# FriedFeid/Video-Depth-Anything

Measured on AMD Instinct MI355X. Metric: depth frames/sec at 32x518x518, ViT-L fp16, 1/2/4/8 MI355X, higher is better.
Workload: dtype fp16; 1 GPU; VideoDepthAnything.forward vitl 1x32x3x518x518 per GPU; encoder=vitl, frames_per_clip=32, H=518, W=518, clips_per_gpu=1, parallelism=clip-parallel dp1, ranks=1, depth_gather_to_rank0=False, hip_graph=False, clips_in_flight=2

## Files before the change

include/vda.h:

```cpp
#ifndef VDA_H
#define VDA_H

#include <stdint.h>

#ifdef __cplusplus
extern "C" {
#endif

enum {
  VDA_ACT_NONE = 0,
  VDA_ACT_GELU = 1,
  VDA_ACT_GEGLU = 2,
  VDA_ACT_RELU = 3
};

enum {
  VDA_STORE_ROWS = 0,
  VDA_STORE_PIXEL_SHUFFLE = 1
};

typedef struct vda_epilogue {
  const float* bias;
  const float* rowbias;
  int32_t rdiv, rmod;
  const float* gamma;
  const void* res;
  int64_t ldres;
  const void* res2;
  int64_t ldres2;
  int32_t act;
  int32_t store;
  int32_t ps_k, ps_cout, ps_hin, ps_win;
  const float* ln_stats;
  const float* ln_colsum;
  int32_t ln_parts;
  float ln_eps;
  float* stats_out;
  int32_t res2_h, res2_w;
  int32_t* sched;
  int32_t drop_period;
} vda_epilogue;

const char* vda_version(void);
int64_t vda_epilogue_size(void);
const char* vda_last_error(void);

int vda_gemm(const void* x, int64_t ldx, const void* w, void* y, int64_t ldy,
             int32_t M, int32_t N, int32_t K, const vda_epilogue* epi, void* stream);
int vda_gemm_check(int64_t ldx, int64_t ldy, int32_t M, int32_t N, int32_t K, const vda_epilogue* epi);

int vda_conv2d(const void* x, const void* w, void* y, int32_t BT, int32_t H, int32_t W,
               int32_t Cin, int32_t Cout, int32_t ks, int32_t stride, int32_t pad,
               int32_t pre_relu, int32_t up_h, int32_t up_w, const vda_epilogue* epi,
               void* ws, int64_t ws_bytes, void* stream);
int64_t vda_conv2d_workspace(int32_t BT, int32_t H, int32_t W, int32_t Cin, int32_t Cout, int32_t ks,
                             int32_t stride, int32_t pad);
int vda_conv2d_res2_upsample_ok(int32_t BT, int32_t H, int32_t W, int32_t Cin, int32_t Cout, int32_t ks,
                                int32_t stride, int32_t pad);

int vda_layernorm(const void* x, int64_t ldx, void* y, const float* gamma, const float* beta,
                  int32_t rows, int32_t C, float eps, int32_t skip_period, void* stream);

int vda_row_stats(const void* x, int64_t ldx, float* stats, int32_t rows, int32_t C, float eps,
                  void* stream);

int vda_groupnorm(const void* x, void* y, const float* gamma, const float* beta, int32_t F,
                  int32_t S, int32_t C, int32_t groups, float eps, float* ws, void* stream);
int64_t vda_groupnorm_workspace(int32_t F, int32_t S, int32_t C, int32_t groups);

int vda_groupnorm_linear(const void* x, const float* gamma, const float* beta, int32_t F, int32_t S,
                         int32_t C, int32_t groups, float eps, const void* w, const float* bias, void* y,
                         int32_t N, float* stats_out, void* ws, int64_t ws_bytes, void* stream);
int64_t vda_groupnorm_linear_workspace(int32_t F, int32_t S, int32_t C, int32_t groups, int32_t N);
int vda_groupnorm_linear_fused(int32_t C, int32_t groups, int32_t N);

int vda_spatial_attention(const void* qkv, void* out, int32_t B, int32_t N, int32_t H,
                          int32_t D, float scale, void* stream);

int vda_temporal_attention(const void* qkv, void* out, int32_t B, int32_t T, int32_t S,
                           int32_t H, int32_t D, float scale, float rope_theta, void* stream);

int vda_upsample_bilinear(const void* x, void* y, int32_t BT, int32_t H, int32_t W, int32_t C,
                          int32_t Ho, int32_t Wo, void* stream);

int vda_patch_im2col(const float* img, void* a, int32_t BT, int32_t H, int32_t W, int32_t Kp,
                     void* stream);

int vda_depth_head(const void* x, const void* w1, const float* b1, const float* w2,
                   const float* b2, float* depth, void* ws, int32_t BT, int32_t Hin, int32_t Win,
                   int32_t C, int32_t Ho, int32_t Wo, void* stream);
int64_t vda_depth_head_workspace(int32_t BT, int32_t Hin, int32_t Win, int32_t C, int32_t Ho, int32_t Wo);

int vda_preprocess_frames(const void* frames, float* out, int32_t N, int32_t h, int32_t w, int32_t H,
                          int32_t W, const float* mean, const float* std, void* stream);

int vda_depth_resize(const float* depth, float* out, int32_t N, int32_t H, int32_t W, int32_t ho,
                     int32_t wo, void* stream);

int64_t vda_scale_shift_workspace(int64_t n);
int vda_scale_shift(const float* pred, const float* target, const uint8_t* mask, int64_t n, double* sums,
                    float* ss, void* ws, int64_t ws_bytes, void* stream);

int vda_depth_align(const float* src, int32_t F, int32_t H, int32_t W, int32_t ho, int32_t wo, const float* ss,
                    int32_t clip, const float* pre, const float* w_pre, const float* w_post, float* out,
                    void* stream);

int64_t vda_depth_eval_workspace(int32_t F, int64_t S);
int vda_depth_eval_fit(const float* pred, const float* gt, const uint8_t* valid, int32_t F, int64_t S,
                       int32_t per_frame, double* sums, float* ss, void* ws, int64_t ws_bytes, void* stream);
int vda_depth_eval_metrics(const float* pred, const float* gt, const uint8_t* valid, int32_t F, int64_t S,
                           const float* ss, int32_t ss_per_frame, float max_depth, float* aligned,
                           double* frame_sums, double* total, void* ws, int64_t ws_bytes, void* stream);

enum {
  VDA_VIS_INDEX = 0,
  VDA_VIS_HWC = 1,
  VDA_VIS_PLANAR444 = 2,
  VDA_VIS_PLANAR420 = 3
};
int64_t vda_depth_range_workspace(int64_t n);
int vda_depth_range(const float* depth, int64_t n, float* range, void* ws, int64_t ws_bytes, void* stream);
int64_t vda_depth_colorize_bytes(int32_t F, int32_t H, int32_t W, int32_t layout);
int vda_depth_colorize(const float* depth, int32_t F, int32_t H, int32_t W, const float* range,
                       const uint8_t* lut, int32_t layout, uint8_t* out, void* stream);

enum {
  VDA_YUV_420 = 0,
  VDA_YUV_422 = 1,
  VDA_YUV_444 = 2,
  VDA_YUV_MONO = 3
};
int vda_yuv_to_rgb(const uint8_t* src, int32_t N, int32_t h, int32_t w, int64_t frame_stride, int32_t chroma,
                   uint8_t* out, void* stream);
int64_t vda_preprocess_yuv_workspace(int32_t N, int32_t h, int32_t w, int32_t H, int32_t W);
int vda_preprocess_yuv(const uint8_t* src, int32_t N, int32_t h, int32_t w, int64_t frame_stride, int32_t chroma,
                       float* out, int32_t H, int32_t W, const float* mean, const float* stdv, void* ws,
                       int64_t ws_bytes, void* stream);
int32_t vda_resample_taps(int32_t in, int32_t out);
int vda_resample_tables(int32_t in, int32_t out, int32_t* k, int32_t* bounds);
int vda_yuv_downscale_ok(int32_t h, int32_t w, int32_t h2, int32_t w2);
int64_t vda_yuv_downscale_workspace(int32_t N, int32_t h, int32_t w, int32_t h2, int32_t w2);
// ... 31 lines not shown
```

video-depth-anything_amd/_lib.py:

```python
from __future__ import annotations

import ctypes
import os
from ctypes import c_float, c_int32, c_int64, c_void_p, POINTER

_HERE = os.path.dirname(os.path.abspath(__file__))
LIB_PATH = os.environ.get("VDA_LIB_OVERRIDE") or os.path.join(_HERE, "libvda.so")
TORCH_LIB_PATH = os.path.join(_HERE, "libvda_torch.so")
if os.environ.get("VDA_LIB_OVERRIDE"):
    _ov = os.path.join(os.path.dirname(os.path.abspath(os.environ["VDA_LIB_OVERRIDE"])), "libvda_torch.so")
    if os.path.exists(_ov):
        TORCH_LIB_PATH = _ov

EXPORTED = (
    "vda_version", "vda_epilogue_size", "vda_last_error", "vda_gemm", "vda_gemm_check", "vda_conv2d", "vda_conv2d_workspace",
    "vda_layernorm",
    "vda_conv2d_res2_upsample_ok",
    "vda_row_stats", "vda_groupnorm", "vda_groupnorm_workspace",
    "vda_groupnorm_linear", "vda_groupnorm_linear_workspace", "vda_groupnorm_linear_fused",
    "vda_spatial_attention", "vda_temporal_attention", "vda_upsample_bilinear", "vda_patch_im2col",
    "vda_depth_head", "vda_depth_head_workspace", "vda_preprocess_frames", "vda_depth_resize",
    "vda_scale_shift", "vda_scale_shift_workspace", "vda_depth_align",
    "vda_depth_eval_workspace", "vda_depth_eval_fit", "vda_depth_eval_metrics",
    "vda_depth_range_workspace", "vda_depth_range", "vda_depth_colorize_bytes", "vda_depth_colorize",
    "vda_yuv_to_rgb", "vda_preprocess_yuv_workspace", "vda_preprocess_yuv",
    "vda_resample_taps", "vda_resample_tables", "vda_yuv_downscale_ok", "vda_yuv_downscale_workspace",
    "vda_yuv_downscale",
    "vda_gemm_f32", "vda_conv2d_f32", "vda_layernorm_f32", "vda_groupnorm_f32", "vda_spatial_attention_f32",
    "vda_temporal_attention_f32", "vda_upsample_bilinear_f32", "vda_patch_im2col_f32", "vda_depth_head_f32",
)
TUNE_EXPORTED = ("vda_debug_force_tile", "vda_debug_gemm_sched", "vda_debug_strip_split", "vda_debug_hconv",
                 "vda_debug_dconv", "vda_debug_attn")
TUNE_LIB_PATH = os.path.join(os.path.dirname(_HERE), "build", "tune", "libvda.so")

ACT_NONE, ACT_GELU, ACT_GEGLU, ACT_RELU = 0, 1, 2, 3
STORE_ROWS, STORE_PIXEL_SHUFFLE = 0, 1
VIS_INDEX, VIS_HWC, VIS_PLANAR444, VIS_PLANAR420 = 0, 1, 2, 3
YUV_420, YUV_422, YUV_444, YUV_MONO = 0, 1, 2, 3


class VDAUnavailable(RuntimeError):
    pass


class VDAError(RuntimeError):
    pass


class Epilogue(ctypes.Structure):
    _fields_ = [
        ("bias", c_void_p), ("rowbias", c_void_p), ("rdiv", c_int32), ("rmod", c_int32),
        ("gamma", c_void_p), ("res", c_void_p), ("ldres", c_int64), ("res2", c_void_p),
        ("ldres2", c_int64), ("act", c_int32), ("store", c_int32), ("ps_k", c_int32),
        ("ps_cout", c_int32), ("ps_hin", c_int32), ("ps_win", c_int32),
        ("ln_stats", c_void_p), ("ln_colsum", c_void_p), ("ln_parts", c_int32), ("ln_eps", c_float),
        ("stats_out", c_void_p), ("res2_h", c_int32), ("res2_w", c_int32), ("sched", c_void_p),
        ("drop_period", c_int32),
    ]


_lib = None
_load_error = None


def _declare(lib):
    P, I, L, F = c_void_p, c_int32, c_int64, c_float
    EP = POINTER(Epilogue)
    sig = {
        "vda_version": ([], ctypes.c_char_p),
        "vda_epilogue_size": ([], L),
        "vda_last_error": ([], ctypes.c_char_p),
        "vda_gemm": ([P, L, P, P, L, I, I, I, EP, P], I),
        "vda_gemm_check": ([L, L, I, I, I, EP], I),
        "vda_conv2d": ([P, P, P, I, I, I, I, I, I, I, I, I, I, I, EP, P, L, P], I),
        "vda_conv2d_workspace": ([I, I, I, I, I, I, I, I], L),
        "vda_conv2d_res2_upsample_ok": ([I, I, I, I, I, I, I, I], I),
        "vda_layernorm": ([P, L, P, P, P, I, I, F, I, P], I),
        "vda_row_stats": ([P, L, P, I, I, F, P], I),
        "vda_groupnorm": ([P, P, P, P, I, I, I, I, F, P, P], I),
        "vda_groupnorm_workspace": ([I, I, I, I], L),
        "vda_groupnorm_linear": ([P, P, P, I, I, I, I, F, P, P, P, I, P, P, L, P], I),
        "vda_groupnorm_linear_workspace": ([I, I, I, I, I], L),
        "vda_groupnorm_linear_fused": ([I, I, I], I),
        "vda_spatial_attention": ([P, P, I, I, I, I, F, P], I),
        "vda_temporal_attention": ([P, P, I, I, I, I, I, F, F, P], I),
        "vda_upsample_bilinear": ([P, P, I, I, I, I, I, I, P], I),
        "vda_patch_im2col": ([P, P, I, I, I, I, P], I),
        "vda_depth_head": ([P, P, P, P, P, P, P, I, I, I, I, I, I, P], I),
        "vda_depth_head_workspace": ([I, I, I, I, I, I], L),
        "vda_preprocess_frames": ([P, P, I, I, I, I, I, POINTER(F), POINTER(F), P], I),
        "vda_depth_resize": ([P, P, I, I, I, I, I, P], I),
        "vda_scale_shift_workspace": ([L], L),
        "vda_scale_shift": ([P, P, P, L, P, P, P, L, P], I),
        "vda_depth_align": ([P, I, I, I, I, I, P, I, P, POINTER(F), POINTER(F), P, P], I),
        "vda_depth_eval_workspace": ([I, L], L),
        "vda_depth_eval_fit": ([P, P, P, I, L, I, P, P, P, L, P], I),
        "vda_depth_eval_metrics": ([P, P, P, I, L, P, I, F, P, P, P, P, L, P], I),
        "vda_depth_range_workspace": ([L], L),
        "vda_depth_range": ([P, L, P, P, L, P], I),
        "vda_depth_colorize_bytes": ([I, I, I, I], L),
        "vda_depth_colorize": ([P, I, I, I, P, P, I, P, P], I),
        "vda_yuv_to_rgb": ([P, I, I, I, L, I, P, P], I),
        "vda_preprocess_yuv_workspace": ([I, I, I, I, I], L),
        "vda_preprocess_yuv": ([P, I, I, I, L, I, P, I, I, POINTER(F), POINTER(F), P, L, P], I),
        "vda_resample_taps": ([I, I], I),
        "vda_resample_tables": ([I, I, P, P], I),
        "vda_yuv_downscale_ok": ([I, I, I, I], I),
        "vda_yuv_downscale_workspace": ([I, I, I, I, I], L),
        "vda_yuv_downscale": ([P, I, I, I, L, I, P, P, P, P, P, I, I, P, L, P], I),
        "vda_gemm_f32": ([P, L, P, P, L, I, I, I, EP, P], I),
        "vda_conv2d_f32": ([P, P, P, I, I, I, I, I, I, I, I, I, EP, P], I),
        "vda_layernorm_f32": ([P, L, P, P, P, I, I, F, I, P], I),
        "vda_groupnorm_f32": ([P, P, P, P, I, I, I, I, F, P], I),
        "vda_spatial_attention_f32": ([P, P, I, I, I, I, F, P], I),
        "vda_temporal_attention_f32": ([P, P, I, I, I, I, I, F, F, P], I),
        "vda_upsample_bilinear_f32": ([P, P, I, I, I, I, I, I, P], I),
        "vda_patch_im2col_f32": ([P, P, I, I, I, I, P], I),
        "vda_depth_head_f32": ([P, P, P, P, P, P, P, P, I, I, I, I, I, I, P], I),
        "vda_debug_force_tile": ([I], I),
        "vda_debug_gemm_sched": ([I], I),
        "vda_debug_strip_split": ([I], I),
        "vda_debug_hconv": ([I], I),
        "vda_debug_dconv": ([I], I),
        "vda_debug_attn": ([I], I),
    }
    for name, (args, res) in sig.items():
        if name.startswith("vda_debug_") and not hasattr(lib, name):
            continue
        fn = getattr(lib, name)
        fn.argtypes = args
        fn.restype = res


def lib():
    global _lib, _load_error
    if _lib is not None:
        return _lib
    if _load_error is not None:
        raise VDAUnavailable(_load_error)
    if not os.path.exists(LIB_PATH):
        _load_error = f"libvda.so not found at {LIB_PATH}; run `make` (or __graft_entry__.build())"
        raise VDAUnavailable(_load_error)
    try:
        l = ctypes.CDLL(LIB_PATH)
        _declare(l)
        if l.vda_epilogue_size() != ctypes.sizeof(Epilogue):
            raise OSError(f"vda_epilogue is {l.vda_epilogue_size()} bytes in the library, {ctypes.sizeof(Epilogue)} "
                          f"in _lib.Epilogue: rebuild libvda.so or update the mirror")
    except OSError as e:
        _load_error = f"failed to load {LIB_PATH}: {e}"
        raise VDAUnavailable(_load_error) from e
    _lib = l
    return _lib


_torch_ops = None


def torch_ops():
# ... 20 lines not shown
```

video-depth-anything_amd/csrc/vda_conv2d.hip:

```cpp
#include "vda_internal.h"

static bool conv_takes_strip(int BT, int H, int W, int Cin, int Cout, int ks, int stride, int pad, int up_h) {
  if (up_h > 0 || ks != 3 || stride != 1 || pad != 1 || !vda_conv_strip_serves(W, Cin, Cout)) return false;
  const long strip_tiles = (long)BT * ((H * W + 255) / 256);
  return g_force_tile == -3 || (g_force_tile == -1 && (Cin >= 512 || strip_tiles * 2 <= vda_cu_count()));
}

static long conv_im2col_bytes(int BT, int H, int W, int Cin, int ks, int stride, int pad) {
  const long Ho = (H + 2L * pad - ks) / stride + 1, Wo = (W + 2L * pad - ks) / stride + 1;
  return (long)BT * Ho * Wo * ks * ks * Cin * 2;
}
static bool conv_takes_im2col(int BT, int H, int W, int Cin, int Cout, int ks, int stride, int pad, int up_h) {
  if (up_h > 0 || ks != 3 || stride != 2 || Cout % 256 != 0 || g_force_tile != -1) return false;
  const long Ho = (H + 2L * pad - ks) / stride + 1, Wo = (W + 2L * pad - ks) / stride + 1;
  return Ho > 0 && Wo > 0 && vda_gemm_phased256_serves((long)BT * Ho * Wo, Cout, 9L * Cin, 9L * Cin);
}

static bool conv_takes_hconv(int BT, int H, int W, int Cin, int Cout, int ks, int stride, int pad) {
  return ks == 3 && stride == 1 && pad == 1 && g_force_tile == -1 && vda_conv_hconv_serves(BT, H, W, Cin, Cout);
}

extern "C" int64_t vda_conv2d_workspace(int32_t BT, int32_t H, int32_t W, int32_t Cin, int32_t Cout, int32_t ks,
                                        int32_t stride, int32_t pad) {
  if (BT <= 0 || H <= 0 || W <= 0 || Cin <= 0 || Cout <= 0) return 0;
  if (conv_takes_hconv(BT, H, W, Cin, Cout, ks, stride, pad)) return 0;
  if (conv_takes_im2col(BT, H, W, Cin, Cout, ks, stride, pad, 0)) return conv_im2col_bytes(BT, H, W, Cin, ks, stride, pad);
  if (!conv_takes_strip(BT, H, W, Cin, Cout, ks, stride, pad, 0)) return 0;
  return vda_conv_strip_ws_bytes(BT, H, W, Cin, Cout);
}

extern "C" int vda_conv2d_res2_upsample_ok(int32_t BT, int32_t H, int32_t W, int32_t Cin, int32_t Cout, int32_t ks,
                                           int32_t stride, int32_t pad) {
  if (BT <= 0 || H <= 0 || W <= 0 || Cin <= 0 || Cout <= 0) return 0;
  return conv_takes_hconv(BT, H, W, Cin, Cout, ks, stride, pad) ? 1 : 0;
}

extern "C" int vda_conv2d(const void* x, const void* w, void* y, int32_t BT, int32_t H, int32_t W,
                          int32_t Cin, int32_t Cout, int32_t ks, int32_t stride, int32_t pad,
                          int32_t pre_relu, int32_t up_h, int32_t up_w, const vda_epilogue* epi,
                          void* ws, int64_t ws_bytes, void* stream) {
  VDA_CHECK_ARG(x && w && y, "null pointer");
  VDA_CHECK_ARG(BT > 0 && H > 0 && W > 0 && Cin > 0 && Cout > 0 && ks > 0 && stride > 0 && pad >= 0,
                "bad conv geometry");
  VDA_CHECK_ARG(Cin % 8 == 0 && Cout % 4 == 0, "Cin % 8 and Cout % 4 required");
  const int Hi = up_h > 0 ? up_h : H, Wi = up_w > 0 ? up_w : W;
  GemmParams p{};
  p.x = (const h16*)x; p.w = (const h16*)w; p.y = (h16*)y;
  p.H = H; p.W = W; p.Cin = Cin; p.ks = ks; p.stride = stride; p.pad = pad; p.pre_relu = pre_relu;
  p.up_h = up_h > 0 ? up_h : 0; p.up_w = up_w > 0 ? up_w : 0;
  p.Ho = (Hi + 2 * pad - ks) / stride + 1;
  p.Wo = (Wi + 2 * pad - ks) / stride + 1;
  VDA_CHECK_ARG(p.Ho > 0 && p.Wo > 0, "empty conv output");
  p.M = BT * p.Ho * p.Wo; p.N = Cout; p.K = ks * ks * Cin;
  p.ldy = Cout; p.ldx = 0;
  p.epi = epi ? *epi : vda_default_epi();
  if (p.epi.rdiv <= 0) p.epi.rdiv = 1;
  if (p.epi.rmod <= 0) p.epi.rmod = 1;
  VDA_CHECK_ARG(p.epi.store == VDA_STORE_ROWS && (p.epi.act == VDA_ACT_NONE || p.epi.act == VDA_ACT_RELU),
                "conv: row store, activation none/relu");
  VDA_CHECK_ARG(!p.epi.stats_out && !p.epi.ln_stats, "conv: no LayerNorm fold / row statistics");
  int rc = vda_check_epi(p.epi, p.M, Cout);
  if (rc) return rc;
  const bool res2_up = p.epi.res2_h > 0 || p.epi.res2_w > 0;
  if (res2_up) {
    VDA_CHECK_ARG(p.epi.res2 && p.epi.res2_h > 0 && p.epi.res2_w > 0 && p.epi.ldres2 == Cout && p.up_h == 0 &&
                      !p.epi.gamma && !p.epi.rowbias && (!p.epi.res || p.epi.ldres == Cout) &&
                      p.epi.res2_h <= p.Ho && p.epi.res2_w <= p.Wo &&
                      (long)p.epi.res2_h * p.epi.res2_w * Cout * 2 < (1L << 31) &&
                      conv_takes_hconv(BT, H, W, Cin, Cout, ks, stride, pad),
                  "upsampled res2 needs the halo conv route (vda_conv2d_res2_upsample_ok), a [BT, h <= Ho, w <= Wo, "
                  "Cout] source, no gamma / rowbias / input upsample");
    return vda_conv_hconv(x, w, y, p.epi.bias, p.epi.act == VDA_ACT_RELU, pre_relu, p.epi.res, p.epi.res2,
                          p.epi.res2_h, p.epi.res2_w, BT, H, W, Cin, Cout, (hipStream_t)stream);
  }
  if (p.up_h > 0) {
    if (g_force_tile < 0 && ks == 3 && stride == 1 && pad == 1 && !pre_relu && !p.epi.res && !p.epi.res2 &&
        !p.epi.gamma && !p.epi.rowbias) {
      rc = vda_conv_halo_fused(x, w, y, p.epi.bias, p.epi.act == VDA_ACT_RELU, BT, H, W, p.up_h, p.up_w, Cin, Cout,
                               (hipStream_t)stream);
      if (rc != 1) return rc;
    }
    return vda_launch_conv_reg(p, (hipStream_t)stream);
  }
  if (!p.epi.gamma && !p.epi.rowbias && (!p.epi.res || p.epi.ldres == Cout) && (!p.epi.res2 || p.epi.ldres2 == Cout) &&
      conv_takes_hconv(BT, H, W, Cin, Cout, ks, stride, pad)) {
    rc = vda_conv_hconv(x, w, y, p.epi.bias, p.epi.act == VDA_ACT_RELU, pre_relu, p.epi.res, p.epi.res2, 0, 0, BT, H,
                        W, Cin, Cout, (hipStream_t)stream);
    if (rc != 1) return rc;
  }
  if (conv_takes_strip(BT, H, W, Cin, Cout, ks, stride, pad, 0) && !p.epi.gamma && !p.epi.rowbias &&
      (!p.epi.res || p.epi.ldres == Cout) && (!p.epi.res2 || p.epi.ldres2 == Cout)) {
    rc = vda_conv_strip(x, w, y, p.epi.bias, p.epi.act == VDA_ACT_RELU, pre_relu, p.epi.res, p.epi.res2, BT, H, W,
                        Cin, Cout, ws, ws ? ws_bytes : 0, (hipStream_t)stream);
    if (rc != 1) return rc;
  }
  if (g_force_tile < 0 && ks == 3 && stride == 1 && pad == 1 && !pre_relu && !p.epi.res && !p.epi.res2 &&
      !p.epi.gamma && !p.epi.rowbias && (long)H * W >= 128L * 128L) {
    rc = vda_conv_halo(x, w, y, p.epi.bias, p.epi.act == VDA_ACT_RELU, BT, H, W, Cin, Cout, (hipStream_t)stream);
    if (rc != 1) return rc;
  }
  if (conv_takes_im2col(BT, H, W, Cin, Cout, ks, stride, pad, 0) && !pre_relu && ws &&
      ws_bytes >= conv_im2col_bytes(BT, H, W, Cin, ks, stride, pad) && (uintptr_t)ws % 16 == 0 &&
      (uintptr_t)x % 16 == 0) {
    rc = vda_conv_im2col(x, ws, BT, H, W, Cin, p.Ho, p.Wo, ks, stride, pad, (hipStream_t)stream);
    if (rc) return rc;
    p.x = (const h16*)ws;
    p.ldx = p.K;
    return vda_launch_gemm(p, (hipStream_t)stream);
  }
  return vda_launch_conv_gemm(p, (hipStream_t)stream);
}
```

video-depth-anything_amd/csrc/vda_f32.hip:

```cpp
#include "vda_common.h"
#include "../../include/vda.h"
#include <cmath>

namespace {

struct F32Params {
  const float* x; long ldx;
  const float* w;
  float* y; long ldy;
  int M, N, K;
  int H, W, Cin, Ho, Wo, ks, stride, pad, pre_relu;
  vda_epilogue epi;
};

constexpr int FBK = 16;
constexpr int FLD = 20;

__device__ __forceinline__ f4 mfma_f32(float a, float b, f4 c) {
  return __builtin_amdgcn_mfma_f32_16x16x4f32(a, b, c, 0, 0, 0);
}

__device__ __forceinline__ float gelu_exact(float v) { return 0.5f * v * (1.0f + erff(v * 0.70710678118654752f)); }

template <bool CONV>
// ... 389 lines not shown
    const f4 d = *reinterpret_cast<const f4*>(bp + ((long)y1 * W + x1) * C);
    f4 o;
#pragma unroll
    for (int j = 0; j < 4; ++j) o[j] = hy * (hx * a[j] + lx * bq[j]) + ly * (hx * cq[j] + lx * d[j]);
    *reinterpret_cast<f4*>(y + i * 4) = o;
  }
}

__global__ __launch_bounds__(256) void im2col_f32_kernel(const float* __restrict__ img, float* __restrict__ a, int BT,
                                                         int H, int W, int Kp) {
  const int ph = H / 14, pw = W / 14, np = ph * pw;
  const long total = (long)BT * (1 + np) * Kp;
  for (long i = (long)blockIdx.x * 256 + threadIdx.x; i < total; i += (long)gridDim.x * 256) {
    const int k = (int)(i % Kp);
    const long row = i / Kp;
    const int tok = (int)(row % (1 + np));
    const int bt = (int)(row / (1 + np));
    float v = 0.f;
    if (tok > 0 && k < 588) {
      const int pidx = tok - 1, py = pidx / pw, px = pidx - py * pw;
      const int ci = k / 196, r = k - ci * 196, ky = r / 14, kx = r - ky * 14;
      v = img[(((long)bt * 3 + ci) * H + py * 14 + ky) * W + px * 14 + kx];
    }
    a[i] = v;
  }
}

__global__ __launch_bounds__(256) void pointwise_relu_f32_kernel(const float* __restrict__ mid, const float* __restrict__ w2,
                                                                 const float* __restrict__ b2, float* __restrict__ out, long M) {
  const long m = (long)blockIdx.x * 256 + threadIdx.x;
  if (m >= M) return;
  const float* r = mid + m * 32;
  float a = 0.f;
#pragma unroll
  for (int c = 0; c < 32; c += 4) {
    const f4 v = *reinterpret_cast<const f4*>(r + c);
    a += v[0] * w2[c] + v[1] * w2[c + 1] + v[2] * w2[c + 2] + v[3] * w2[c + 3];
  }
  out[m] = fmaxf(a + b2[0], 0.f);
}

template <bool CONV>
int launch_f32(const F32Params& p, hipStream_t st) {
  const int tiles_n = (p.N + 127) / 128, tiles_m = (p.M + 127) / 128;
  const long blocks = (long)tiles_n * tiles_m;
  if (blocks > 0x7fffffffL) return vda_set_error(-22, "fp32 GEMM grid too large");
  const dim3 g((unsigned)blocks), bl(256);
  switch (p.epi.act) {
    case VDA_ACT_NONE: hipLaunchKernelGGL((gemm_f32_kernel<CONV, VDA_ACT_NONE>), g, bl, 0, st, p, tiles_n); break;
    case VDA_ACT_GELU: hipLaunchKernelGGL((gemm_f32_kernel<CONV, VDA_ACT_GELU>), g, bl, 0, st, p, tiles_n); break;
    case VDA_ACT_RELU: hipLaunchKernelGGL((gemm_f32_kernel<CONV, VDA_ACT_RELU>), g, bl, 0, st, p, tiles_n); break;
    case VDA_ACT_GEGLU:
      if (CONV) return vda_set_error(-22, "GEGLU epilogue is dense-only");
      hipLaunchKernelGGL((gemm_f32_kernel<CONV, VDA_ACT_GEGLU>), g, bl, 0, st, p, tiles_n);
      break;
    default: return vda_set_error(-22, "unknown activation");
  }
  VDA_LAUNCH_CHECK();
  return 0;
}

}

extern "C" int vda_gemm_f32(const float* x, int64_t ldx, const float* w, float* y, int64_t ldy, int32_t M, int32_t N,
                            int32_t K, const vda_epilogue* epi, void* stream) {
  VDA_CHECK_ARG(x && w && y && epi, "null pointer");
  VDA_CHECK_ARG(M > 0 && N > 0 && K > 0, "empty GEMM");
  VDA_CHECK_ARG(K % 4 == 0 && ldx % 4 == 0 && N % 4 == 0, "fp32 GEMM needs K, ldx, N multiples of 4");
  VDA_CHECK_ARG(ldx >= K, "fp32 GEMM needs ldx >= K");
  VDA_CHECK_ARG(ldy % 4 == 0, "fp32 GEMM needs ldy a multiple of 4");
  VDA_CHECK_ARG(!epi->res || epi->ldres % 4 == 0, "fp32 GEMM needs ldres a multiple of 4");
  VDA_CHECK_ARG(!epi->res2 || epi->ldres2 % 4 == 0, "fp32 GEMM needs ldres2 a multiple of 4");
  VDA_CHECK_ARG(epi->drop_period == 0, "fp32 GEMM: no drop_period (vda_gemm only)");
  VDA_CHECK_ARG(epi->act != VDA_ACT_GEGLU || (N % 32 == 0 && !epi->rowbias && !epi->res2 &&
                                              epi->store == VDA_STORE_ROWS),
                "GEGLU needs N % 32 == 0, no rowbias/res2, row store");
  VDA_CHECK_ARG(epi->store != VDA_STORE_PIXEL_SHUFFLE || (epi->ps_k > 0 && epi->ps_cout % 4 == 0 &&
                                                         epi->ps_hin > 0 && epi->ps_win > 0),
                "bad pixel-shuffle geometry");
  VDA_CHECK_ARG(!epi->rowbias || (epi->rdiv > 0 && epi->rmod > 0), "rowbias needs rdiv, rmod > 0");
  VDA_CHECK_ARG(!epi->ln_stats, "fp32 GEMM: no LayerNorm fold (the fp32 mode runs vda_layernorm_f32)");
  VDA_CHECK_ARG(!epi->stats_out, "fp32 GEMM: no row statistics output");
  VDA_CHECK_ARG(epi->res2_h == 0 && epi->res2_w == 0, "fp32 GEMM: no upsampled res2");
  F32Params p{};
  p.x = x; p.ldx = ldx; p.w = w; p.y = y; p.ldy = ldy; p.M = M; p.N = N; p.K = K; p.epi = *epi;
  return launch_f32<false>(p, (hipStream_t)stream);
}

extern "C" int vda_conv2d_f32(const float* x, const float* w, float* y, int32_t BT, int32_t H, int32_t W, int32_t Cin,
                              int32_t Cout, int32_t ks, int32_t stride, int32_t pad, int32_t pre_relu,
                              const vda_epilogue* epi, void* stream) {
  VDA_CHECK_ARG(x && w && y && epi, "null pointer");
  VDA_CHECK_ARG(BT > 0 && H > 0 && W > 0 && ks > 0 && stride > 0 && pad >= 0, "bad conv geometry");
  VDA_CHECK_ARG(Cin % 4 == 0 && Cout % 4 == 0, "fp32 conv needs Cin, Cout multiples of 4");
  VDA_CHECK_ARG(epi->act != VDA_ACT_GEGLU && epi->store == VDA_STORE_ROWS, "conv epilogue: no GEGLU / pixel shuffle");
  VDA_CHECK_ARG(epi->res2_h == 0 && epi->res2_w == 0, "fp32 conv: no upsampled res2 (materialise it)");
  VDA_CHECK_ARG(!epi->rowbias || (epi->rdiv > 0 && epi->rmod > 0), "rowbias needs rdiv, rmod > 0");
  VDA_CHECK_ARG(epi->drop_period == 0, "fp32 conv: no drop_period (vda_gemm only)");
  VDA_CHECK_ARG(!epi->res || epi->ldres % 4 == 0, "fp32 conv needs ldres a multiple of 4");
  VDA_CHECK_ARG(!epi->res2 || epi->ldres2 % 4 == 0, "fp32 conv needs ldres2 a multiple of 4");
  VDA_CHECK_ARG(!epi->ln_stats && !epi->stats_out, "fp32 conv: no LayerNorm fold / row statistics");
  F32Params p{};
  p.x = x; p.w = w; p.y = y; p.ldy = Cout;
  p.H = H; p.W = W; p.Cin = Cin; p.ks = ks; p.stride = stride; p.pad = pad; p.pre_relu = pre_relu;
  p.Ho = (H + 2 * pad - ks) / stride + 1;
  p.Wo = (W + 2 * pad - ks) / stride + 1;
  VDA_CHECK_ARG(p.Ho > 0 && p.Wo > 0, "empty conv output");
  const long M = (long)BT * p.Ho * p.Wo;
  VDA_CHECK_ARG(M < 0x7fffffffL, "conv output too large");
  p.M = (int)M; p.N = Cout; p.K = ks * ks * Cin; p.epi = *epi;
  return launch_f32<true>(p, (hipStream_t)stream);
}

extern "C" int vda_spatial_attention_f32(const float* qkv, float* out, int32_t B, int32_t N, int32_t H, int32_t D,
                                         float scale, void* stream) {
  VDA_CHECK_ARG(qkv && out, "null pointer");
  VDA_CHECK_ARG(B > 0 && N > 0 && H > 0, "empty attention");
  VDA_CHECK_ARG(D == 64, "fp32 spatial attention: head dim must be 64");
  VDA_CHECK_ARG(B <= 65535 && H <= 65535, "grid too large");
  hipLaunchKernelGGL(spatial_attn_f32_kernel, dim3((N + 63) / 64, H, B), dim3(256), 0, (hipStream_t)stream, qkv, out, N,
                     H, scale);
  VDA_LAUNCH_CHECK();
  return 0;
}

extern "C" int vda_temporal_attention_f32(const float* qkv, float* out, int32_t B, int32_t T, int32_t S, int32_t H,
                                          int32_t D, float scale, float rope_theta, void* stream) {
  VDA_CHECK_ARG(qkv && out, "null pointer");
  VDA_CHECK_ARG(B > 0 && T > 0 && S > 0 && H > 0 && D > 0, "empty attention");
  VDA_CHECK_ARG(T <= 32 && D <= 128 && D % 2 == 0, "temporal attention: T <= 32, even D <= 128");
  const long blocks = (long)B * S * H;
  VDA_CHECK_ARG(blocks < 0x7fffffffL, "grid too large");
  hipLaunchKernelGGL(temporal_attn_f32_kernel, dim3((unsigned)blocks), dim3(64), 0, (hipStream_t)stream, qkv, out, T, S,
                     H, D, scale, rope_theta);
  VDA_LAUNCH_CHECK();
  return 0;
}

extern "C" int vda_layernorm_f32(const float* x, int64_t ldx, float* y, const float* gamma, const float* beta,
                                 int32_t rows, int32_t C, float eps, int32_t skip_period, void* stream) {
  VDA_CHECK_ARG(x && y && gamma && beta, "null pointer");
  VDA_CHECK_ARG(rows > 0 && C > 0 && C <= 2048, "LayerNorm: 0 < C <= 2048");
  hipLaunchKernelGGL(layernorm_f32_kernel, dim3((rows + 3) / 4), dim3(256), 0, (hipStream_t)stream, x, (long)ldx, y,
                     gamma, beta, rows, C, eps, skip_period);
  VDA_LAUNCH_CHECK();
  return 0;
}

extern "C" int vda_groupnorm_f32(const float* x, float* y, const float* gamma, const float* beta, int32_t F, int32_t S,
                                 int32_t C, int32_t groups, float eps, void* stream) {
  VDA_CHECK_ARG(x && y && gamma && beta, "null pointer");
  VDA_CHECK_ARG(F > 0 && S > 0 && groups > 0 && C % groups == 0, "bad GroupNorm geometry");
  hipLaunchKernelGGL(groupnorm_f32_kernel, dim3(F * groups), dim3(256), 0, (hipStream_t)stream, x, y, gamma, beta, S, C,
                     groups, eps);
  VDA_LAUNCH_CHECK();
  return 0;
}

extern "C" int vda_upsample_bilinear_f32(const float* x, float* y, int32_t BT, int32_t H, int32_t W, int32_t C,
                                         int32_t Ho, int32_t Wo, void* stream) {
  VDA_CHECK_ARG(x && y, "null pointer");
  VDA_CHECK_ARG(BT > 0 && H > 0 && W > 0 && Ho > 0 && Wo > 0 && C > 0 && C % 4 == 0, "bad resize geometry");
  const long total = (long)BT * Ho * Wo * (C / 4);
  const int grid = (int)std::min<long>((total + 255) / 256, 65536);
  hipLaunchKernelGGL(upsample_f32_kernel, dim3(grid), dim3(256), 0, (hipStream_t)stream, x, y, BT, H, W, C, Ho, Wo);
  VDA_LAUNCH_CHECK();
  return 0;
}

extern "C" int vda_patch_im2col_f32(const float* img, float* a, int32_t BT, int32_t H, int32_t W, int32_t Kp,
                                    void* stream) {
  VDA_CHECK_ARG(img && a, "null pointer");
  VDA_CHECK_ARG(BT > 0 && H >= 14 && W >= 14 && H % 14 == 0 && W % 14 == 0, "bad image geometry");
  VDA_CHECK_ARG(Kp >= 588 && Kp % 4 == 0, "Kp must be >= 588 and a multiple of 4");
  const long total = (long)BT * (1 + (H / 14) * (W / 14)) * Kp;
  const int grid = (int)std::min<long>((total + 255) / 256, 65536);
  hipLaunchKernelGGL(im2col_f32_kernel, dim3(grid), dim3(256), 0, (hipStream_t)stream, img, a, BT, H, W, Kp);
  VDA_LAUNCH_CHECK();
  return 0;
// ... 21 lines not shown
```

video-depth-anything_amd/csrc/vda_gemm.hip:

```cpp
#include "vda_gemm_tile.h"
#include "vda_gemm_phased.h"
#include <algorithm>

VDA_KNOB_DEF(int, g_force_tile, -1);

static bool phased_dense_ok(long M, long N, long K, long ldx) {
  return K % 64 == 0 && M * ldx * 2 < (1L << 31) && N * K * 2 < (1L << 31);
}

bool vda_gemm_phased256_serves(long M, long N, long K, long ldx) {
  return N >= 256 && M >= 4096 && phased_dense_ok(M, N, K, ldx);
}

namespace {

VDA_KNOB(int, g_persist, -1);

enum Phased {
  PH_STAGED,
  PH_ROWB,
  PH_REG,
  PH_LNF,
  PH_LNF_REG,
  PH_LNF_ROWB,
// ... 57 lines not shown
  const int tiles_m = (p.M + BM - 1) / BM, tiles_n = (p.N + BN - 1) / BN;
  hipLaunchKernelGGL((gemm_kernel<BM, BN, NWM, NWN, KB, NS, CONV, ACT>), dim3(tiles_m * tiles_n), dim3(NWM * NWN * 64),
                     0, st, p, tiles_m, tiles_n);
}

template <int XR, int WR, bool CONV, int ACT>
void launch_phased(Phased v, const GemmParams& p, hipStream_t st) {
  const int BM = 128 * XR, BN = 128 * WR;
  const int tiles_m = (p.M + BM - 1) / BM, tiles_n = (p.N + BN - 1) / BN;
  const int grid = phased_sched(tiles_m * tiles_n, CONV);
  auto go = [&](void (*kernel)(GemmParams, int, int)) {
    hipLaunchKernelGGL(kernel, dim3(grid), dim3(512), 0, st, p, tiles_m, tiles_n);
  };
  constexpr bool PLAIN = ACT == VDA_ACT_NONE, GELU = ACT == VDA_ACT_GELU, GEGLU = ACT == VDA_ACT_GEGLU;
  constexpr bool D256 = !CONV && XR == 2;
  if constexpr (!CONV && PLAIN)
    if (v == PH_ROWB) return go(gemm256_kernel<XR, WR, CONV, ACT, true>);
  if constexpr (D256 && PLAIN)
    if (v == PH_LNF_ROWB) return go(gemm256_kernel<XR, WR, CONV, ACT, false, true, 3>);
  if constexpr (D256 && (PLAIN || GELU || GEGLU))
    if (v == PH_LNF) return go(gemm256_kernel<XR, WR, CONV, ACT, false, true>);
  if constexpr (D256 && (PLAIN || GELU)) {
    if (v == PH_LNF_REG) return go(gemm256_kernel<XR, WR, CONV, ACT, false, true, 1>);
    if (v == PH_REG) return go(gemm256_kernel<XR, WR, CONV, ACT, false, false, 1>);
  }
  go(gemm256_kernel<XR, WR, CONV, ACT, false>);
}

template <bool CONV, int ACT>
int launch_cfg(const GemmRoute& r, const GemmParams& p, hipStream_t st) {
  switch (r.cfg) {
    case 1: launch_tile<256, 128, 4, 2, 32, 4, CONV, ACT>(p, st); break;
    case 2: launch_tile<128, 64, 2, 2, 32, 4, CONV, ACT>(p, st); break;
    case 3: launch_tile<256, 256, 2, 4, 32, 4, CONV, ACT>(p, st); break;
    case 4: launch_phased<2, 2, CONV, ACT>(r.phased, p, st); break;
    case 5: launch_phased<4, 1, CONV, ACT>(r.phased, p, st); break;
    case 6:
    case 7:
      if constexpr (CONV) {
        return vda_set_error(-22, "conv: no 64-row tile configuration (6 / 7)");
      } else {
        if (r.cfg == 6) launch_tile<64, 64, 2, 2, 32, 4, CONV, ACT>(p, st);
        else launch_tile<64, 128, 2, 2, 32, 4, CONV, ACT>(p, st);
      }
      break;
    default: launch_tile<128, 128, 2, 2, 32, 4, CONV, ACT>(p, st); break;
  }
  return 0;
}

template <bool CONV>
int launch(const GemmParams& p, hipStream_t st) {
  const GemmRoute r = gemm_route(p, CONV);
  int rc = 0;
  switch (p.epi.act) {
    case VDA_ACT_GELU:
    case VDA_ACT_GEGLU:
      if constexpr (CONV) return vda_set_error(-22, "conv epilogue: activation none / relu");
      else rc = p.epi.act == VDA_ACT_GELU ? launch_cfg<CONV, VDA_ACT_GELU>(r, p, st) : launch_cfg<CONV, VDA_ACT_GEGLU>(r, p, st);
      break;
    case VDA_ACT_RELU: rc = launch_cfg<CONV, VDA_ACT_RELU>(r, p, st); break;
    default: rc = launch_cfg<CONV, VDA_ACT_NONE>(r, p, st); break;
  }
  if (rc) return rc;
  VDA_LAUNCH_CHECK();
  if (p.epi.stats_out && !r.writes_stats) return vda_row_partials_launch(p.y, p.ldy, p.epi.stats_out, p.M, p.N, st);
  return 0;
}

int gemm_check(const void* x, int64_t ldx, const void* w, void* y, int64_t ldy, int32_t M, int32_t N, int32_t K,
               const vda_epilogue* epi, GemmParams& p) {
  VDA_CHECK_ARG(x && w && y, "null pointer");
  VDA_CHECK_ARG(M > 0 && N > 0 && K > 0, "empty GEMM");
  VDA_CHECK_ARG(K % 8 == 0 && ldx % 8 == 0 && ldx >= K, "K and ldx must be multiples of 8, ldx >= K");
  VDA_CHECK_ARG(N % 4 == 0 && ldy % 4 == 0, "N and ldy must be multiples of 4");
  p = GemmParams{};
  p.x = (const h16*)x; p.ldx = ldx; p.w = (const h16*)w; p.y = (h16*)y; p.ldy = ldy;
  p.M = M; p.N = N; p.K = K;
  p.epi = epi ? *epi : vda_default_epi();
  if (p.epi.rdiv <= 0) p.epi.rdiv = 1;
  if (p.epi.rmod <= 0) p.epi.rmod = 1;
  const vda_epilogue& e = p.epi;
  VDA_CHECK_ARG(e.res2_h == 0 && e.res2_w == 0, "upsampled res2: vda_conv2d only");
  const GemmRoute r = gemm_route(p, false);
  const bool auto256 = g_force_tile < 0 && r.cfg == 4;
  if (e.drop_period != 0) {
    VDA_CHECK_ARG(auto256 && r.phased == PH_LNF_REG && e.act == VDA_ACT_NONE && e.ln_colsum && e.drop_period >= 256 &&
                      N % 256 == 0,
                  "drop_period: >= 256, with ln_stats + bias, no activation / gamma / res / rowbias / stats_out, "
                  "N % 256 == 0, M >= 4096, K % 64 == 0, 16-byte aligned rows");
  }
  int rc = vda_check_epi(e, M, N);
  if (rc) return rc;
  if (e.ln_stats && e.rowbias) {
    VDA_CHECK_ARG(auto256 && r.phased == PH_LNF_ROWB && N % 256 == 0 && (uintptr_t)x % 16 == 0,
                  "ln_stats with rowbias needs N % 256 == 0, M >= 4096, K % 64 == 0, 16-B aligned rows");
  }
  return 0;
}

}

int vda_launch_conv_reg(const GemmParams& p, hipStream_t st) {
  const int tiles_m = (p.M + 127) / 128;
  if (p.N >= 128) {
    const int tiles_n = (p.N + 127) / 128;
    if (p.epi.act == VDA_ACT_RELU)
      hipLaunchKernelGGL((gemm_reg_kernel<128, 128, ConvLoader, VDA_ACT_RELU>), dim3(tiles_m * tiles_n), dim3(256), 0, st, p, tiles_n);
    else
      hipLaunchKernelGGL((gemm_reg_kernel<128, 128, ConvLoader, VDA_ACT_NONE>), dim3(tiles_m * tiles_n), dim3(256), 0, st, p, tiles_n);
  } else {
    const int tiles_n = (p.N + 63) / 64;
    if (p.epi.act == VDA_ACT_RELU)
      hipLaunchKernelGGL((gemm_reg_kernel<128, 64, ConvLoader, VDA_ACT_RELU>), dim3(tiles_m * tiles_n), dim3(256), 0, st, p, tiles_n);
    else
      hipLaunchKernelGGL((gemm_reg_kernel<128, 64, ConvLoader, VDA_ACT_NONE>), dim3(tiles_m * tiles_n), dim3(256), 0, st, p, tiles_n);
  }
  VDA_LAUNCH_CHECK();
  return 0;
}

vda_epilogue vda_default_epi() {
  vda_epilogue e{};
  e.rdiv = 1; e.rmod = 1;
  return e;
}

int vda_check_epi(const vda_epilogue& e, int M, int N) {
  VDA_CHECK_ARG(!e.rowbias || (e.rdiv > 0 && e.rmod > 0), "rowbias needs rdiv, rmod > 0");
  VDA_CHECK_ARG(e.act >= 0 && e.act <= 3, "unknown activation");
  VDA_CHECK_ARG(e.act != VDA_ACT_GEGLU || (N % 32 == 0 && !e.rowbias && e.store == 0 && !e.res2),
                "GEGLU needs N % 32 == 0, no rowbias/res2, row store");
  VDA_CHECK_ARG(e.store == VDA_STORE_ROWS ||
                (e.store == VDA_STORE_PIXEL_SHUFFLE && e.ps_k > 0 && e.ps_cout > 0 && e.ps_cout % 4 == 0 &&
                 e.ps_hin > 0 && e.ps_win > 0 && N == e.ps_k * e.ps_k * e.ps_cout && !e.res && !e.res2),
                "bad pixel-shuffle store geometry");
  VDA_CHECK_ARG(!e.ln_stats || (e.ln_colsum && e.store == VDA_STORE_ROWS && !e.gamma &&
                                 (e.act == VDA_ACT_NONE || e.act == VDA_ACT_GELU || e.act == VDA_ACT_GEGLU)),
                "ln_stats needs ln_colsum, a row store, no gamma, activation none / gelu / geglu");
  VDA_CHECK_ARG(!e.ln_stats || !e.rowbias ||
                    (e.act == VDA_ACT_NONE && e.bias && !e.res && !e.res2 && !e.stats_out && e.rdiv >= 256),
                "ln_stats with rowbias needs a bias, no activation / residual / stats_out, rdiv >= 256");
  VDA_CHECK_ARG(!e.ln_stats || (e.ln_parts >= 0 && e.ln_parts <= 4), "ln_parts must be 0 .. 4");
  VDA_CHECK_ARG(!e.ln_stats || (long)M * (e.ln_parts > 0 ? e.ln_parts : 1) >= 2, "ln_stats needs M * max(ln_parts, 1) >= 2");
  VDA_CHECK_ARG(!e.stats_out || (e.store == VDA_STORE_ROWS && e.act != VDA_ACT_GEGLU),
                "stats_out needs a row store and no GEGLU");
  VDA_CHECK_ARG(!e.res || e.ldres % 4 == 0, "ldres % 4");
  VDA_CHECK_ARG(!e.res2 || e.ldres2 % 4 == 0, "ldres2 % 4");
  return 0;
}

int vda_launch_gemm(const GemmParams& p, hipStream_t st) { return launch<false>(p, st); }

extern "C" int vda_gemm_check(int64_t ldx, int64_t ldy, int32_t M, int32_t N, int32_t K, const vda_epilogue* epi) {
  GemmParams p;
  void* const aligned = (void*)16;
  return gemm_check(aligned, ldx, aligned, aligned, ldy, M, N, K, epi, p);
}

extern "C" int vda_gemm(const void* x, int64_t ldx, const void* w, void* y, int64_t ldy, int32_t M,
                        int32_t N, int32_t K, const vda_epilogue* epi, void* stream) {
  GemmParams p;
  const int rc = gemm_check(x, ldx, w, y, ldy, M, N, K, epi, p);
  return rc ? rc : vda_launch_gemm(p, (hipStream_t)stream);
}

int vda_launch_conv_gemm(const GemmParams& p, hipStream_t st) { return launch<true>(p, st); }

int vda_launch_depth_gemm(const GemmParams& p, hipStream_t st) {
  const int tiles_m = (p.M + 255) / 256;
  hipLaunchKernelGGL((gemm_kernel<256, 64, 8, 1, 64, 2, true, ACT_DEPTH>), dim3(tiles_m), dim3(512), 0, st, p, tiles_m, 1);
  VDA_LAUNCH_CHECK();
  return 0;
}

#ifdef VDA_TUNING
extern "C" int vda_debug_force_tile(int32_t cfg) {
  g_force_tile = cfg;
  return 0;
}

extern "C" int vda_debug_gemm_sched(int32_t persist_blocks) {
  g_persist = persist_blocks;
  return 0;
}
#endif
```

video-depth-anything_amd/csrc/vda_gemm_phased.h:

```cpp
#pragma once
#include "vda_common.h"
#include "phi_table.h"
#include <type_traits>
#ifdef VDA_TS
__device__ unsigned long long g_ts[4096][8];
#define TS(k) do { if (threadIdx.x == 0 && vb < 4096) g_ts[vb][k] = __builtin_amdgcn_s_memrealtime(); } while (0)
extern "C" int vda_debug_timestamps(void* host) {
  return (int)hipMemcpyFromSymbol(host, HIP_SYMBOL(g_ts), sizeof(g_ts), 0, hipMemcpyDeviceToHost);
}
__device__ unsigned long long g_tsc[1024][4];
#define TSC(k) do { if (threadIdx.x == 0 && blockIdx.x < 1024) { \
    g_tsc[blockIdx.x][2 * (k)] = __builtin_amdgcn_s_memtime(); \
    g_tsc[blockIdx.x][2 * (k) + 1] = __builtin_amdgcn_s_memrealtime(); } } while (0)
extern "C" int vda_debug_clock_stamps(void* host) {
  return (int)hipMemcpyFromSymbol(host, HIP_SYMBOL(g_tsc), sizeof(g_tsc), 0, hipMemcpyDeviceToHost);
}
#else
#define TS(k) do {} while (0)
#define TSC(k) do {} while (0)
#endif
#include "vda_gemm_tile.h"

constexpr int VDA_EPI_STORE_AUX = 2;

// ... 43 lines not shown
               : "v"((unsigned)(uintptr_t)(VDA_LDS const int*)ptr) : "memory");
  return v;
}

__device__ __forceinline__ void perm16_swap(float& a, float& b) {
  asm volatile("s_nop 1\n\tv_permlane16_swap_b32 %0, %1" : "+v"(a), "+v"(b));
}
template <int CTRL>
__device__ __forceinline__ float dpp_f(float v) {
  return __builtin_bit_cast(float, __builtin_amdgcn_mov_dpp(__builtin_bit_cast(int, v), CTRL, 0xF, 0xF, true));
}
__device__ __forceinline__ float halfwave_sum32(float (&v)[32], int lane) {
  float w[16];
#pragma unroll
  for (int k = 0; k < 16; ++k) {
    float a = v[k], b = v[16 + k];
    perm16_swap(a, b);
    w[k] = a + b;
  }
  const int i = lane & 15;
  float x[8], y[4], z[2];
  bool lo = i < 8;
#pragma unroll
  for (int k = 0; k < 8; ++k) x[k] = (lo ? w[k] : w[k + 8]) + dpp_f<0x140>(lo ? w[k + 8] : w[k]);
  lo = (i & 7) < 4;
#pragma unroll
  for (int k = 0; k < 4; ++k) y[k] = (lo ? x[k] : x[k + 4]) + dpp_f<0x141>(lo ? x[k + 4] : x[k]);
  lo = (i & 3) < 2;
#pragma unroll
  for (int k = 0; k < 2; ++k) z[k] = (lo ? y[k] : y[k + 2]) + dpp_f<0x1B>(lo ? y[k + 2] : y[k]);
  lo = (i & 1) == 0;
  return (lo ? z[0] : z[1]) + dpp_f<0xB1>(lo ? z[1] : z[0]);
}
template <class F>
__device__ __forceinline__ void pack_row_lines(F v, bool lo8, u32x4& A, u32x4& B) {
  u32x4 o[2];
#pragma unroll
  for (int pp = 0; pp < 2; ++pp) {
    float a[4], c[4];
#pragma unroll
    for (int r = 0; r < 4; ++r) {
      a[r] = v(2 * pp, r);
      c[r] = v(2 * pp + 1, r);
      perm16_swap(a[r], c[r]);
    }
    typedef float f2v __attribute__((ext_vector_type(2)));
    const h2 h0 = __builtin_convertvector(f2v{a[0], a[1]}, h2), h1 = __builtin_convertvector(f2v{a[2], a[3]}, h2);
    const h2 h2_ = __builtin_convertvector(f2v{c[0], c[1]}, h2), h3 = __builtin_convertvector(f2v{c[2], c[3]}, h2);
    o[pp] = u32x4{__builtin_bit_cast(unsigned, h0), __builtin_bit_cast(unsigned, h1),
                  __builtin_bit_cast(unsigned, h2_), __builtin_bit_cast(unsigned, h3)};
  }
#pragma unroll
  for (int k = 0; k < 4; ++k) {
    const unsigned snd = lo8 ? o[1][k] : o[0][k];
    const unsigned got = (unsigned)__builtin_amdgcn_mov_dpp((int)snd, 0x128, 0xF, 0xF, true);
    A[k] = lo8 ? o[0][k] : got;
    B[k] = lo8 ? got : o[1][k];
  }
}
__device__ __forceinline__ float2 ln_mean_rstd(float sm, float sq, float invK, float eps) {
  const float mean = sm * invK;
  return make_float2(mean, rsqrtf(fmaxf(fmaf(-mean, mean, sq * invK), 0.f) + eps));
}
__device__ __forceinline__ void stat_acc(h8 t, float& s, float& q) {
  const h2 one = h2{(h16)1.f, (h16)1.f};
  h2 tp[4];
#pragma unroll
  for (int k = 0; k < 4; ++k) tp[k] = h2{t[2 * k], t[2 * k + 1]};
  s = 0.f;
  q = 0.f;
#pragma unroll
  for (int k = 0; k < 4; ++k) {
    s = __builtin_amdgcn_fdot2(tp[k], one, s, false);
    q = __builtin_amdgcn_fdot2(tp[k], tp[k], q, false);
  }
}

template <int XR, int WR, int ACT>
constexpr int phased_nit() {
  constexpr int OW = (ACT == VDA_ACT_GEGLU) ? 64 * WR : 128 * WR;
  return (128 * XR) / (512 / (OW / 8));
}

template <int XR, int WR, bool CONV, int ACT, bool ROWB, bool LNF, int EK>
__device__ __forceinline__ int gemm256_tile(const GemmParams& p, int vb, int tiles_m, int tiles_n, h16* smem,
                                            bool pre, int vb_next, int wave_in, unsigned* tctr = nullptr,
                                            int tbase = 0, int* tslot = nullptr) {
  static_assert(!(LNF && (ROWB || CONV)), "LNF: dense, no row bias");
  static_assert(EK == 0 || (!CONV && !ROWB), "fixed epilogue kinds: dense, no row bias");
  static_assert(EK != 3 || (ACT == VDA_ACT_NONE && LNF), "EK 3: LN fold + per-frame row bias, no activation");
  const bool has_bias = EK ? true : p.epi.bias != nullptr;
  const bool has_gamma = EK ? false : p.epi.gamma != nullptr;
  const bool ps_rows = !EK && ACT != VDA_ACT_GEGLU && !ROWB && XR == 2 && WR == 2 &&
                       p.epi.store == VDA_STORE_PIXEL_SHUFFLE && p.epi.ps_cout % 256 == 0 && p.epi.ps_win >= 16 &&
                       (long)p.M * p.N * 2 < 0x7fffffffL && (uintptr_t)p.y % 16 == 0;
  const bool rows_store = EK ? true : (p.epi.store == VDA_STORE_ROWS || ps_rows);
  const bool has_res = EK ? false : p.epi.res != nullptr;
  const bool has_res2 = EK ? false : p.epi.res2 != nullptr;
  const bool has_stats = EK ? false : p.epi.stats_out != nullptr;
  static_assert(XR * WR == 4 && (XR == 2 || XR == 4), "8 waves as XR (m) x 8/XR (n), wave tile 128 x 64");
  constexpr int BM = 128 * XR, BN = 128 * WR;
  constexpr int HALF = 128 * BK;
  constexpr int BUF = (XR + WR) * HALF;
  constexpr bool TAB = XR == 2 && (ACT == VDA_ACT_GELU || ACT == VDA_ACT_GEGLU);
  const float* phi_lds = reinterpret_cast<const float*>(smem + 2 * BUF);
  const unsigned phib = phi_base(phi_lds);
  h16* lnst_lds = smem + 2 * BUF + (TAB ? PHI_LDS_HALVES : 0);
  auto lnst_shift_row = [&](int m0_) {
    const int P1 = p.epi.ln_parts > 0 ? p.epi.ln_parts : 1;
    return ((p.M * P1) & 1) && p.M - 1 - m0_ < 256 ? p.M - 1 - m0_ : -1;
  };

  int lane, wave;
  asm volatile("v_mbcnt_lo_u32_b32 %0, -1, 0\n\tv_mbcnt_hi_u32_b32 %0, -1, %0" : "=v"(lane));
  asm volatile("s_mov_b32 %0, %1" : "=s"(wave) : "s"(wave_in));
  const int tid = wave * 64 + lane;
  const int wm = wave % XR, wn = wave / XR;
  int tile_m, tile_n;
  tile_coords(vb, tiles_m * tiles_n, tiles_m, tiles_n, tile_m, tile_n);
  const int m0 = tile_m * BM, n0 = tile_n * BN;

  const h16* xrow[XR][2];
  const h16* wrow[WR][2];
  bool xok[XR][2], wok[WR][2];
  auto xr_of = [&](int i) { return i * 64 + wave * 8 + (lane >> 3); };
  auto wr_of = [&](int i) { return (wave >> 2) * 64 + i * 32 + (wave & 3) * 8 + (lane >> 3); };
  const int kch0 = ((lane & 7) ^ ((((wave & 1) << 3 | (lane >> 3)) >> 1) & 7)) * 8;
  int cyx[XR][2];
#pragma unroll
  for (int i = 0; i < 2; ++i) {
#pragma unroll
    for (int hh = 0; hh < XR; ++hh) {
      const int m = m0 + hh * 128 + xr_of(i);
      xok[hh][i] = m < p.M;
      const int mm = xok[hh][i] ? m : 0;
      if constexpr (CONV) {
        const int ox = mm % p.Wo;
        const int t = mm / p.Wo;
        const int oy = t % p.Ho, bt = t / p.Ho;
        const int iy0 = xok[hh][i] ? oy * p.stride - p.pad : -32768;
        const int ix0 = ox * p.stride - p.pad;
        cyx[hh][i] = (iy0 << 16) | (ix0 & 0xffff);
        xrow[hh][i] = p.x + (((long)bt * p.H + oy * p.stride - p.pad) * p.W + ix0) * p.Cin;
      } else {
        xrow[hh][i] = p.x + (long)mm * p.ldx;
      }
    }
#pragma unroll
    for (int hh = 0; hh < WR; ++hh) {
      const int n = n0 + hh * 128 + wr_of(i);
      wok[hh][i] = n < p.N;
      wrow[hh][i] = p.w + (long)(wok[hh][i] ? n : 0) * p.K;
    }
  }
  const void* zero = (const void*)g_zero_page;
  const bool tap_uniform = CONV && (p.Cin % BK == 0);
  int t_ci[2] = {0, 0}, t_kx[2] = {0, 0}, t_ky[2] = {0, 0};
  long t_off[2] = {0, 0};
  auto dma_x = [&](int kt, int buf, int i) {
    const int k0 = kt * BK;
    const int ky = t_ky[i], kx = t_kx[i];
    const long toff = t_off[i];
    if (tap_uniform) {
      t_off[i] += BK;
      t_ci[i] += BK;
      if (t_ci[i] == p.Cin) {
        t_ci[i] = 0;
        if (++t_kx[i] == p.ks) { t_kx[i] = 0; ++t_ky[i]; t_off[i] += (long)(p.W - p.ks) * p.Cin; }
      }
    }
#pragma unroll
    for (int hh = 0; hh < XR; ++hh) {
        const int k = k0 + kch0;
        const void* src = zero;
        if constexpr (CONV) {
          if (k < p.K) {
            if (tap_uniform) {
              if ((unsigned)((cyx[hh][i] >> 16) + ky) < (unsigned)p.H &&
                  (unsigned)((short)(cyx[hh][i] & 0xffff) + kx) < (unsigned)p.W)
// ... 336 lines not shown
      const unsigned rA = ya == 0x80000000u ? ya : ya + co;
      const unsigned rB = yb == 0x80000000u ? yb : yb + co;
      __builtin_amdgcn_raw_buffer_store_b128(A, ry, rA, 0, VDA_EPI_STORE_AUX);
      __builtin_amdgcn_raw_buffer_store_b128(B, ry, rB, 0, VDA_EPI_STORE_AUX);
    }
    TS(5);
    return succ;
  }
  if (rows_store) {
    constexpr int OW = (ACT == VDA_ACT_GEGLU) ? BN / 2 : BN;
    __syncthreads();
    const vda_epilogue& e = p.epi;
    bool nok[4];
    int ncl[4];
#pragma unroll
    for (int i = 0; i < 4; ++i) {
      const int n = n0 + wn * 64 + i * 16 + nq;
      nok[i] = n < p.N;
      ncl[i] = nok[i] ? n : 0;
    }
    if constexpr (LNF) {
      const float* st = reinterpret_cast<const float*>(lnst_lds);
      const f4* bv = pbv;
      const int P = e.ln_parts;
      const float invK = 1.f / (float)p.K;
      const int srow = lnst_shift_row(m0);
#pragma unroll
      for (int j = 0; j < 8; ++j) {
        const int rl = wm * 128 + j * 16 + mcol;
        const int sh = rl == srow ? 2 : 0;
        float2 mr;
        if (P <= 0) {
          mr = *reinterpret_cast<const float2*>(st + 2 * rl + sh);
        } else {
          float sm = 0.f, sq = 0.f;
          for (int t = 0; t < P; ++t) {
            const float2 pq = *reinterpret_cast<const float2*>(st + 2 * (rl * P + t) + (t == P - 1 ? sh : 0));
            sm += pq.x;
            sq += pq.y;
          }
          mr = ln_mean_rstd(sm, sq, invK, e.ln_eps);
        }
#pragma unroll
        for (int i = 0; i < 4; ++i)
#pragma unroll
          for (int r = 0; r < 4; ++r)
            acc[i][j][r] = fmaf(mr.y, fmaf(-mr.x, pgv[i][r], acc[i][j][r]), bv[i][r]);
      }
    } else if (has_bias) {
      f4 bv[4];
#pragma unroll
      for (int i = 0; i < 4; ++i)
        bv[i] = PREF ? pbv[i] : *reinterpret_cast<const f4*>(e.bias + (ACT == VDA_ACT_GEGLU ? ncl[i & ~1] + (i & 1) * 16 : ncl[i]));
#pragma unroll
      for (int i = 0; i < 4; ++i)
#pragma unroll
        for (int j = 0; j < 8; ++j) acc[i][j] += bv[i];
    }
    if constexpr (ACT != VDA_ACT_GEGLU && ROWB) {
      if (e.rowbias) {
        const float inv_div = 1.f / (float)e.rdiv, inv_mod = 1.f / (float)e.rmod;
        auto rb_load = [&](int j, f4 (&rb)[4]) {
          const int m = m0 + wm * 128 + j * 16 + mcol;
          int qd = (int)((float)m * inv_div);
          qd += (m - qd * e.rdiv >= e.rdiv) ? 1 : 0;
          qd -= (m < qd * e.rdiv) ? 1 : 0;
          int qm = (int)((float)qd * inv_mod);
          qm += (qd - qm * e.rmod >= e.rmod) ? 1 : 0;
          qm -= (qd < qm * e.rmod) ? 1 : 0;
          const long roff = m < p.M ? (long)(qd - qm * e.rmod) * p.N : 0;
#pragma unroll
          for (int i = 0; i < 4; ++i) rb[i] = *reinterpret_cast<const f4*>(e.rowbias + roff + ncl[i]);
        };
        constexpr int RBD = 2;
        f4 rb[RBD][4];
#pragma unroll
        for (int j = 0; j < RBD - 1; ++j) rb_load(j, rb[j]);
#pragma unroll
        for (int j = 0; j < 8; ++j) {
          if (j + RBD - 1 < 8) rb_load(j + RBD - 1, rb[(j + RBD - 1) % RBD]);
#pragma unroll
          for (int i = 0; i < 4; ++i) acc[i][j] += rb[j % RBD][i];
          __builtin_amdgcn_sched_barrier(0);
        }
      }
    }
    if constexpr (TAB) {
#pragma unroll
      for (int i = (ACT == VDA_ACT_GEGLU ? 1 : 0); i < 4; i += (ACT == VDA_ACT_GEGLU ? 2 : 1))
#pragma unroll
        for (int j = 0; j < 8; j += 4) {
          phi_f2 ab[16];
#pragma unroll
          for (int k = 0; k < 16; ++k) ab[k] = phi_line(acc[i][j + k / 4][k % 4], phib);
#pragma unroll
          for (int k = 0; k < 16; ++k) {
            const float a = acc[i][j + k / 4][k % 4];
            acc[i][j + k / 4][k % 4] = a * fmaf(a, ab[k].y, ab[k].x);
          }
        }
    }
    auto phase1 = [&](auto g_tag) {
      constexpr bool HG = decltype(g_tag)::value;
#pragma unroll
      for (int i = 0; i < 4; i += (ACT == VDA_ACT_GEGLU ? 2 : 1)) {
        const int nl = wn * 64 + i * 16 + nq;
        f4 gv = f4{1.f, 1.f, 1.f, 1.f};
        if constexpr (HG) {
          if constexpr (PREF) gv = pgv[i];
          else gv = *reinterpret_cast<const f4*>(e.gamma + (ACT == VDA_ACT_GEGLU ? (nok[i] ? (n0 >> 1) + ((wn * 64 + i * 16) >> 1) + nq : 0) : ncl[i]));
        }
#pragma unroll
        for (int j = 0; j < 8; ++j) {
          const int ml = wm * 128 + j * 16 + mcol;
          f4 v;
          int col;
          if constexpr (ACT == VDA_ACT_GEGLU) {
            const f4 vh = acc[i][j], vg = acc[i + 1][j];
#pragma unroll
            for (int r = 0; r < 4; ++r) v[r] = vh[r] * (TAB ? vg[r] : gelu_erf(vg[r]));
            col = ((wn * 64 + i * 16) >> 1) + nq;
          } else {
            v = acc[i][j];
            if constexpr (ACT == VDA_ACT_GELU && !TAB) {
#pragma unroll
              for (int r = 0; r < 4; ++r) v[r] = gelu_erf(v[r]);
            } else if constexpr (ACT == VDA_ACT_RELU) {
#pragma unroll
              for (int r = 0; r < 4; ++r) v[r] = fmaxf(v[r], 0.f);
            }
            col = nl;
          }
          if constexpr (HG) v *= gv;
          typedef float f2v __attribute__((ext_vector_type(2)));
          const h2 lo = __builtin_convertvector(f2v{v[0], v[1]}, h2);
          const h2 hi = __builtin_convertvector(f2v{v[2], v[3]}, h2);
          const int u = (col >> 2) ^ (ml & 15);
          *reinterpret_cast<uint2*>(&smem[ml * OW + u * 4]) = make_uint2(__builtin_bit_cast(unsigned, lo), __builtin_bit_cast(unsigned, hi));
        }
      }
    };
    const int nout = (ACT == VDA_ACT_GEGLU) ? (p.N >> 1) : p.N;
    const int cout0 = (ACT == VDA_ACT_GEGLU) ? (n0 >> 1) : n0;
    constexpr int CPR = OW / 8;
    constexpr int RPI = 512 / CPR;
    constexpr int NIT = BM / RPI;
    const int q = tid % CPR, row0 = tid / CPR;
    const int sw = row0 & 15;
    const h16* l0 = smem + row0 * OW + ((2 * q) ^ sw) * 4;
    const h16* l1 = smem + row0 * OW + ((2 * q + 1) ^ sw) * 4;
    const int c = cout0 + q * 8;
    const long mrows = p.M - m0;
    auto rsrc = [&](const h16* base, long ld) {
      return __builtin_amdgcn_make_buffer_rsrc((void*)(base + (long)m0 * ld), (short)0,
                                               (int)(mrows * ld * 2 < 0x7fffffffL ? mrows * ld * 2 : 0x7fffffffL), 0x00020000);
    };
    auto voff = [&](long ld) { return c < nout ? (unsigned)(((long)row0 * ld + c) * 2) : 0x80000000u; };
    const __amdgpu_buffer_rsrc_t ry = rsrc(p.y, p.ldy);
    const unsigned vy = voff(p.ldy), sy = (unsigned)(RPI * p.ldy * 2);
    const h16* r1p = (const h16*)(has_res ? e.res : e.res2);
    const long r1ld = has_res ? e.ldres : e.ldres2;
    const int nres = (has_res ? 1 : 0) + (has_res2 ? 1 : 0);
    constexpr bool RPF = XR == 2 && ACT == VDA_ACT_NONE && !CONV && !ROWB && !LNF;
    h8 rpre[RPF ? NIT : 1];
    if constexpr (RPF) {
      if (nres == 1) {
// ... 21 lines not shown
        __builtin_amdgcn_s_waitcnt(0xC07F);
        __builtin_amdgcn_s_barrier();
        int tmn, tnn;
        tile_coords(vb_next, tiles_m * tiles_n, tiles_m, tiles_n, tmn, tnn);
        unsigned xn[XR][2], wn2[WR][2];
        dense_offsets(tmn * BM, tnn * BN, xn, wn2);
        lnst_dma(tmn * BM, tnn * BN, vb_next);
        chain_dma(xn, wn2);
      }
    }
    auto phase2 = [&](auto nres_tag) {
      constexpr int NR = decltype(nres_tag)::value;
      __amdgpu_buffer_rsrc_t rr1, rr2;
      unsigned vr1 = 0, sr1 = 0, vr2 = 0, sr2 = 0;
      if constexpr (NR >= 1) { rr1 = rsrc(r1p, r1ld); vr1 = voff(r1ld); sr1 = (unsigned)(RPI * r1ld * 2); }
      if constexpr (NR >= 2) { rr2 = rsrc((const h16*)e.res2, e.ldres2); vr2 = voff(e.ldres2); sr2 = (unsigned)(RPI * e.ldres2 * 2); }
      constexpr int PD = 4;
      h8 q1[PD], q2[PD];
      auto ld1 = [&](int it) { return __builtin_bit_cast(h8, __builtin_amdgcn_raw_buffer_load_b128(rr1, vr1 + it * sr1, 0, 0)); };
      auto ld2 = [&](int it) { return __builtin_bit_cast(h8, __builtin_amdgcn_raw_buffer_load_b128(rr2, vr2 + it * sr2, 0, 0)); };
#pragma unroll
      for (int it = 0; it < PD && it < NIT; ++it) {
        if constexpr (NR >= 1) q1[it] = ld1(it);
        if constexpr (NR >= 2) q2[it] = ld2(it);
      }
#pragma unroll
      for (int it = 0; it < NIT; ++it) {
        h8 t = tv[it];
        if constexpr (NR >= 1) {
          t += q1[it % PD];
          if (it + PD < NIT) q1[it % PD] = ld1(it + PD);
        }
        if constexpr (NR >= 2) {
          t += q2[it % PD];
          if (it + PD < NIT) q2[it % PD] = ld2(it + PD);
        }
        __builtin_amdgcn_raw_buffer_store_b128(__builtin_bit_cast(u32x4, t), ry, vy + it * sy, 0, VDA_EPI_STORE_AUX);
      }
    };
    auto store_with_stats = [&](auto with_res) {
      constexpr bool WR1 = decltype(with_res)::value;
      static_assert(NIT == 16 && RPI == 16, "stats: a half-wave per row, 16 rows per lane");
      const bool cval = c < nout;
      float v[32];
#pragma unroll
      for (int it = 0; it < NIT; ++it) {
        h8 t = tv[it];
        if constexpr (WR1) t += rpre[it];
        __builtin_amdgcn_raw_buffer_store_b128(__builtin_bit_cast(u32x4, t), ry, vy + it * sy, 0, VDA_EPI_STORE_AUX);
        stat_acc(cval ? t : h8{0, 0, 0, 0, 0, 0, 0, 0}, v[it], v[16 + it]);
      }
      const float r = halfwave_sum32(v, lane);
      const int P = (p.N + 255) / 256;
      const int m = m0 + row0 + 16 * (lane & 15);
      const __amdgpu_buffer_rsrc_t rs =
          __builtin_amdgcn_make_buffer_rsrc((void*)e.stats_out, (short)0, (int)((long)p.M * P * 8), 0x00020000);
      const unsigned vo = m < p.M ? (unsigned)((((long)m * P + (n0 >> 8)) * 2 + ((lane >> 4) & 1)) * 4) : 0x80000000u;
      __builtin_amdgcn_raw_buffer_store_b32(__builtin_bit_cast(unsigned, r), rs, vo, 0, 0);
    };
    auto ps_store = [&]() {
      if constexpr (RPI == 16 && ACT != VDA_ACT_GEGLU && !ROWB && XR == 2) {
      const int k = e.ps_k, cout = e.ps_cout, win = e.ps_win, hin = e.ps_hin;
      const int ij = n0 / cout, co0 = n0 - ij * cout, ki = ij / k, kj = ij - ki * k;
      const __amdgpu_buffer_rsrc_t rz =
          __builtin_amdgcn_make_buffer_rsrc((void*)p.y, (short)0, (int)((long)p.M * p.N * 2), 0x00020000);
      int m = m0 + row0;
      int xw = m % win, tq = m / win;
      int yh = tq % hin, bt = tq / hin;
      const long rowlen = (long)win * k;
#pragma unroll
      for (int it = 0; it < NIT; ++it) {
        const long pix = ((long)(bt * hin + yh) * k + ki) * rowlen + (long)xw * k + kj;
        const unsigned off = m < p.M ? (unsigned)((pix * cout + co0 + q * 8) * 2) : 0x80000000u;
        __builtin_amdgcn_raw_buffer_store_b128(__builtin_bit_cast(u32x4, tv[it]), rz, off, 0, VDA_EPI_STORE_AUX);
        m += RPI;
        xw += RPI;
        if (xw >= win) {
          xw -= win;
          if (++yh == hin) { yh = 0; ++bt; }
        }
      }
      }
    };
    if (ps_rows) {
      ps_store();
    } else if (nres == 0) {
      if constexpr (RPF) {
        if (has_stats) store_with_stats(std::false_type{});
        else phase2(std::integral_constant<int, 0>{});
      } else {
        phase2(std::integral_constant<int, 0>{});
      }
    } else if (nres == 1) {
      if constexpr (RPF) {
        if (has_stats) {
          store_with_stats(std::true_type{});
        } else {
#pragma unroll
          for (int it = 0; it < NIT; ++it) {
            const h8 t = tv[it] + rpre[it];
            __builtin_amdgcn_raw_buffer_store_b128(__builtin_bit_cast(u32x4, t), ry, vy + it * sy, 0, VDA_EPI_STORE_AUX);
          }
        }
      } else {
        phase2(std::integral_constant<int, 1>{});
      }
    } else {
      phase2(std::integral_constant<int, 2>{});
    }
    TS(5);
    return succ;
  }
  if constexpr (PREF) {
#pragma unroll
    for (int i = 0; i < 4; ++i) asm volatile("" ::"v"(pbv[i]), "v"(pgv[i]));
  }
  if constexpr (EK != 0) {
    return succ;
  } else if constexpr (ACT == VDA_ACT_GEGLU) {
#pragma unroll
    for (int i = 0; i < 4; i += 2) {
      const int nbase = n0 + wn * 64 + i * 16;
      if (nbase >= p.N) continue;
      const int n_out = (nbase >> 1) + nq;
#pragma unroll
      for (int j = 0; j < 8; ++j) {
        const int m = m0 + wm * 128 + j * 16 + mcol;
        if (m < p.M) epi_geglu4(p, m, nbase + nq, nbase + 16 + nq, n_out, acc[i][j], acc[i + 1][j]);
      }
    }
  } else {
#pragma unroll
    for (int i = 0; i < 4; ++i) {
      const int n = n0 + wn * 64 + i * 16 + nq;
      if (n >= p.N) continue;
#pragma unroll
      for (int j = 0; j < 8; ++j) {
        const int m = m0 + wm * 128 + j * 16 + mcol;
        if (m < p.M) epi_store4<ACT>(p, m, n, acc[i][j]);
      }
    }
  }
  return succ;
}

template <int XR, int WR, bool CONV, int ACT, bool ROWB, bool LNF = false, int EK = 0>
__global__ __launch_bounds__(512) void gemm256_kernel(GemmParams p, int tiles_m, int tiles_n) {
  constexpr int BUF = (XR + WR) * 128 * BK;
  constexpr bool TAB = XR == 2 && (ACT == VDA_ACT_GELU || ACT == VDA_ACT_GEGLU);
  constexpr int SMEM_HALVES = 2 * BUF + (TAB ? PHI_LDS_HALVES : 0) + (LNF ? 4096 + 1024 : 0) +
                              (EK == 3 ? 2048 : 0) + (XR == 2 ? 64 : 0);
  __shared__ __attribute__((aligned(1024))) h16 smem[SMEM_HALVES];
  const int ntiles = tiles_m * tiles_n;
  const int wave = __builtin_amdgcn_readfirstlane((int)threadIdx.x >> 6);
  if constexpr (CONV) {
    const int vb = blockIdx.x;
    TS(0);
    gemm256_tile<XR, WR, CONV, ACT, ROWB, LNF, EK>(p, vb, tiles_m, tiles_n, smem, false, -1, wave);
    TS(7);
  } else {
    const bool chain = EK != 0;
    const bool dyn = XR == 2 && EK != 3 && p.epi.sched != nullptr && ntiles > (int)gridDim.x &&
                     (gridDim.x & 7) == 0;
    unsigned* tctr = dyn ? reinterpret_cast<unsigned*>(p.epi.sched) + (blockIdx.x & 7) : nullptr;
    const int tbase = (int)gridDim.x + (int)(blockIdx.x & 7);
    int* tslot = XR == 2 ? reinterpret_cast<int*>(smem + SMEM_HALVES - 64) : nullptr;
    bool pre = false;
    TSC(0);
    for (int vb = blockIdx.x; vb >= 0 && vb < ntiles;) {
      TS(0);
      const int nxt = vb + (int)gridDim.x;
      vb = gemm256_tile<XR, WR, CONV, ACT, ROWB, LNF, EK>(p, vb, tiles_m, tiles_n, smem, pre, nxt < ntiles ? nxt : -1,
                                                         wave, tctr, tbase, tslot);
      if (!chain) __syncthreads();
      pre = chain;
      TS(7);
    }
    TSC(1);
    if (dyn && wave == 0 && threadIdx.x == 0) {
      unsigned* sc = reinterpret_cast<unsigned*>(p.epi.sched);
      if (__hip_atomic_fetch_add(sc + 8, 1u, __ATOMIC_RELAXED, __HIP_MEMORY_SCOPE_AGENT) == gridDim.x - 1) {
#pragma unroll
        for (int i = 0; i < 9; ++i) __hip_atomic_store(sc + i, 0u, __ATOMIC_RELAXED, __HIP_MEMORY_SCOPE_AGENT);
      }
    }
  }
}

}
```

video-depth-anything_amd/csrc/vda_internal.h:

```cpp
#pragma once
#include "vda_common.h"
#include "../../include/vda.h"

struct GemmParams {
  const h16* x; long ldx;
  const h16* w;
  h16* y; long ldy;
  int M, N, K;
  int H, W, Cin, Ho, Wo, ks, stride, pad, pre_relu, up_h, up_w;
  vda_epilogue epi;
};
VDA_KNOB_DECL(int, g_force_tile, -1);
vda_epilogue vda_default_epi();
int vda_check_epi(const vda_epilogue& e, int M, int N);
int vda_launch_gemm(const GemmParams& p, hipStream_t st);
int vda_launch_conv_gemm(const GemmParams& p, hipStream_t st);
bool vda_gemm_phased256_serves(long M, long N, long K, long ldx);
int vda_launch_conv_reg(const GemmParams& p, hipStream_t st);
int vda_launch_depth_gemm(const GemmParams& p, hipStream_t st);

int vda_conv_halo(const void* x, const void* w, void* y, const float* bias, int relu, int BT, int H, int W, int Cin,
                  int Cout, hipStream_t st);
int vda_conv_halo_fused(const void* x, const void* w, void* y, const float* bias, int relu, int BT, int Hs, int Ws,
                        int H, int W, int Cin, int Cout, hipStream_t st);

bool vda_depth_conv_serves(int H, int W, int C);
int vda_depth_conv(const void* U, const void* w1, const float* b1, const float* w2, const float* b2, float* depth,
                   int BT, int H, int W, int C, hipStream_t st);
bool vda_depth_conv_fused_serves(int Hs, int Ws, int H, int W, int C);
int vda_depth_conv_fused(const void* x, const void* w1, const float* b1, const float* w2, const float* b2,
                         float* depth, int BT, int Hs, int Ws, int H, int W, int C, hipStream_t st);

bool vda_conv_strip_serves(int W, int Cin, int Cout);
long vda_conv_strip_ws_bytes(int BT, int H, int W, int Cin, int Cout);
int vda_conv_strip(const void* x, const void* w, void* y, const float* bias, int relu_out, int pre_relu,
                   const void* res, const void* res2, int BT, int H, int W, int Cin, int Cout, void* ws,
                   long ws_bytes, hipStream_t st);

bool vda_conv_hconv_serves(int BT, int H, int W, int Cin, int Cout);
int vda_conv_hconv(const void* x, const void* w, void* y, const float* bias, int relu_out, int pre_relu,
                   const void* res, const void* res2, int res2_h, int res2_w, int BT, int H, int W, int Cin, int Cout,
                   hipStream_t st);

int vda_row_partials_launch(const void* y, int64_t ldy, float* out, int32_t rows, int32_t N, hipStream_t st);

int vda_conv_im2col(const void* x, void* a, int BT, int H, int W, int Cin, int Ho, int Wo, int ks, int stride, int pad,
                    hipStream_t st);
```

video-depth-anything_amd/csrc/vda_oc1.hip:

```cpp
#include "vda_internal.h"
#include "vda_halo.h"

namespace {

__device__ __attribute__((aligned(64))) uint4 g_dz_page[4];
#ifdef VDA_TS
__device__ unsigned long long g_dts[1024][24];
#endif

constexpr int DT = 16;
constexpr int DP = DT + 2;
constexpr int DNPIX = DP * DP;
constexpr int CS = 64;
constexpr int CO = 128;
constexpr int NB = CO / 32;
constexpr int CPX = CS / 8;
constexpr int PSTR = 10;
constexpr int ND = CS / 32;
constexpr int SPU = 9;

typedef unsigned dh_u4 __attribute__((ext_vector_type(4)));

__device__ __forceinline__ int w_pos(int n, int cd) { return cd ^ ((n >> 1) & (CPX - 1)); }

template <bool UPS>
__global__ __launch_bounds__(UPS ? 768 : 512) void halo_conv_kernel(const h16* __restrict__ U, const h16* __restrict__ w1,
                                                                  const float* __restrict__ b1, h16* __restrict__ yout,
                                                                  int relu_out, int H, int W, int C, int tiles_x,
                                                                  int tiles_y, int ntiles, int Hs = 0, int Ws = 0) {
  constexpr int IW = UPS ? 4 : 0;
  constexpr int PSLOT = DNPIX * PSTR;
  constexpr int PP = (PSLOT + 63) / 64;
  constexpr int PBUF = (UPS ? PSLOT : PP * 64) * 8;
  constexpr int WSLOT = CO * CPX;
  constexpr int WBUF = WSLOT * 8;
  constexpr int WPCS = WSLOT / 64;
  constexpr int WPW = (WPCS + 7) / 8;
  constexpr int WRING = 2;
  constexpr int SPPW = (HALO_SRC_PIXELS * CPX + 511) / 512;
  constexpr int SSLOT = UPS ? SPPW * 8 * 64 : 0;
  static_assert(SPPW * 8 * 64 >= HALO_SRC_PIXELS * CPX, "source slot: HALO_SRC_PIXELS pixels x CPX chunks");
  __shared__ __attribute__((aligned(16))) h16 dsm[2 * PBUF + WRING * WBUF + SSLOT * 8];
  h16* patch = dsm;
  h16* wbuf = dsm + 2 * PBUF;
  h16* sbuf = dsm + 2 * PBUF + WRING * WBUF;

  const int tid = threadIdx.x, lane = tid & 63;
  const int wave = __builtin_amdgcn_readfirstlane(tid >> 6);
  const int mg = wave & 3, ng = wave >> 2;
  const bool iwave = IW > 0 && wave >= 8;
  const int nslab = C / CS;
  const int K = 9 * C;
  const int units_per_tile = nslab;
  const int my_tiles = blockIdx.x < ntiles ? (ntiles - 1 - blockIdx.x) / gridDim.x + 1 : 0;
  const int my_units = my_tiles * units_per_tile;
  if (my_units == 0) return;
  const int my_steps = my_units * SPU;
  const void* zero = (const void*)g_dz_page;

  struct Ud { int bt, y0, x0, slab, sy_lo, sx_lo, SR, SC; };
  auto tile_of_unit = [&](int u, int& bt, int& y0, int& x0) {
    halo_tile_of(blockIdx.x + (u / units_per_tile) * gridDim.x, tiles_x, tiles_y, DT, bt, y0, x0);
  };
  auto dma_patch = [&](int u, const Ud& ud, int q) {
    const int bt = ud.bt, y0 = ud.y0, x0 = ud.x0, slab = ud.slab;
    const int s = q * 64 + lane;
    const int p = s / PSTR, cd = s - p * PSTR;
    const int pr = p / DP;
    const int py = y0 - 1 + pr, px = x0 - 1 + (p - pr * DP);
    const void* src = zero;
    if (p < DNPIX && cd < CPX && (unsigned)py < (unsigned)H && (unsigned)px < (unsigned)W)
      src = U + (((long)bt * H + py) * W + px) * C + slab * CS + cd * 8;
    glds16(src, patch + (u & 1) * PBUF + q * 512);
  };
  constexpr int USL = DNPIX * CPX;
  constexpr int UCH = UPS ? (USL + 511) / 512 : 1;
  const float usy = UPS ? ac_scale(Hs, H) : 0.f, usx = UPS ? ac_scale(Ws, W) : 0.f;
  auto make_ud = [&](int u) {
    Ud ud;
    tile_of_unit(u, ud.bt, ud.y0, ud.x0);
    ud.slab = u % units_per_tile;
    ud.sy_lo = ud.sx_lo = ud.SR = ud.SC = 0;
    if constexpr (UPS) halo_src_region(usy, usx, ud.y0, ud.x0, DT, H, W, Hs, Ws, ud.sy_lo, ud.sx_lo, ud.SR, ud.SC);
    return ud;
  };
  auto dma_src = [&](const Ud& ud, int q) {
    const int bt = ud.bt, sy_lo = ud.sy_lo, sx_lo = ud.sx_lo, SR = ud.SR, SC = ud.SC, slab = ud.slab;
    const int s = q * 64 + lane;
    const int px = s / CPX, cd = s % CPX;
    const int r = px / SC, c = px - r * SC;
    const void* src = zero;
    if (r < SR) src = U + (((long)bt * Hs + sy_lo + r) * Ws + sx_lo + c) * C + slab * CS + cd * 8;
    glds16(src, sbuf + q * 512);
  };
  auto ups_interp = [&](int u, const Ud& ud, int t0, int tstride, auto nk_tag) {
    constexpr int NK = decltype(nk_tag)::value;
    const int y0 = ud.y0, x0 = ud.x0, sy_lo = ud.sy_lo, sx_lo = ud.sx_lo, SC = ud.SC;
#pragma unroll
    for (int k = 0; k < NK; ++k) {
      const int s = t0 + k * tstride;
      const int sc = min(s, USL - 1);
      const int p = sc / CPX, cd = sc - p * CPX;
      const int pr = p / DP;
      const int py = y0 - 1 + pr, px = x0 - 1 + (p - pr * DP);
      const bool ok = (unsigned)py < (unsigned)H && (unsigned)px < (unsigned)W;
      int sy0, sy1, sx0, sx1;
      float wy, wx;
      ac_coord(min(max(py, 0), H - 1), Hs, usy, sy0, sy1, wy);
      ac_coord(min(max(px, 0), W - 1), Ws, usx, sx0, sx1, wx);
      const int r0 = (sy0 - sy_lo) * SC, r1 = (sy1 - sy_lo) * SC, c0 = sx0 - sx_lo, c1 = sx1 - sx_lo;
      const h8 a = *reinterpret_cast<const h8*>(sbuf + ((r0 + c0) * CPX + cd) * 8);
      const h8 b = *reinterpret_cast<const h8*>(sbuf + ((r0 + c1) * CPX + cd) * 8);
// ... 13 lines not shown
  constexpr int ISEG = 3;
  constexpr int NITEM = (DP / ISEG) * DP * CPX;
  auto ups_interp_item = [&](int u, const Ud& ud, int it) {
    if (it >= NITEM) return;
    const int SC = ud.SC;
    const int cd = it % CPX, col = (it / CPX) % DP, seg = it / (CPX * DP);
    halo_blend_column<ISEG>(
        usy, usx, ud.y0, ud.x0, col, seg * ISEG, H, W, Hs, Ws, ud.sy_lo, ud.sx_lo,
        [&](int r, int c) { return *reinterpret_cast<const uint4*>(sbuf + ((r * SC + c) * CPX + cd) * 8); },
        [&](int pr, uint4 v) {
          const int slot = (pr * DP + col) * PSTR + cd;
          asm volatile("ds_write_b128 %0, %1" ::"v"((unsigned)(uintptr_t)(VDA_LDS h16*)(patch + (u & 1) * PBUF + slot * 8)),
                       "v"(__builtin_bit_cast(dh_u4, v))
                       : "memory");
        });
    lgkm0();
  };
  auto dma_w = [&](int st, int slab, int wslot) {
#pragma unroll
    for (int j = 0; j < WPW; ++j) {
      const int piece = (wave * WPW + j) % WPCS;
      const int s = piece * 64 + lane;
      const int n = s / CPX, pos = s - n * CPX;
      const int cd = w_pos(n, pos);
      glds16(w1 + (long)n * K + st * C + slab * CS + cd * 8, wbuf + wslot * WBUF + piece * 512);
    }
  };

  Ud ud_next = make_ud(0);
  if constexpr (UPS) {
    if (!iwave) {
      for (int j = 0; j < SPPW; ++j) dma_src(ud_next, wave + j * 8);
      dma_w(0, ud_next.slab, 0);
    }
    wait_vmcnt<0>();
    __builtin_amdgcn_s_barrier();
    if (!iwave) ups_interp(0, ud_next, tid, 512, std::integral_constant<int, UCH>{});
    __syncthreads();
  } else {
    for (int q = wave; q < PP; q += 8) dma_patch(0, ud_next, q);
    dma_w(0, ud_next.slab, 0);
    wait_vmcnt<0>();
  }
  __builtin_amdgcn_s_barrier();

  if constexpr (UPS) {
    if (iwave) {
      constexpr int SPI = SPPW * 8 / IW;
      constexpr int ISTEPS = (NITEM + 64 * IW - 1) / (64 * IW);
      static_assert(SPPW * 8 % IW == 0 && ISTEPS <= SPU - 3, "interpolation wave split");
      int iu = 0, ist = 0;
      for (int gs = 0; gs < my_steps; ++gs) {
        if (ist == 0 && iu + 1 < my_units) {
          ud_next = make_ud(iu + 1);
          for (int j = 0; j < SPI / 2; ++j) dma_src(ud_next, (wave - 8) + j * IW);
        }
        if (ist == 1 && iu + 1 < my_units)
          for (int j = SPI / 2; j < SPI; ++j) dma_src(ud_next, (wave - 8) + j * IW);
        if (ist >= 3 && ist < 3 + ISTEPS && iu + 1 < my_units)
          ups_interp_item(iu + 1, ud_next, (ist - 3) * 64 * IW + (tid - 512));
        if (ist == 2) wait_vmcnt<0>();
        __builtin_amdgcn_s_barrier();
        if (++ist == SPU) {
          ist = 0;
          ++iu;
        }
      }
      return;
    }
  }
  const int frow = lane & 15, g = lane >> 4;
  const unsigned lin_x = (unsigned)(((mg * 4) * DP + frow) * PSTR + g) * 16u;
  unsigned lin_w[ND];
#pragma unroll
  for (int d = 0; d < ND; ++d) {
    const int n0r = ng * NB * 16 + frow;
    lin_w[d] = (unsigned)(n0r * CPX + w_pos(n0r, d * 4 + g)) * 16u;
  }
  f4 acc[NB][4];
#pragma unroll
  for (int a = 0; a < NB; ++a)
#pragma unroll
    for (int i = 0; i < 4; ++i) acc[a][i] = f4{0.f, 0.f, 0.f, 0.f};
  f4 bias_r[NB];
#pragma unroll
  for (int a = 0; a < NB; ++a)
    bias_r[a] = b1 ? *reinterpret_cast<const f4*>(b1 + (ng * NB + a) * 16 + g * 4) : f4{0.f, 0.f, 0.f, 0.f};
  const int my_pp = (PP - 1 - wave) / 8 + 1;
  constexpr int PPMAX = (PP + 7) / 8;

  int u = 0, st = 0, slab = 0;
#ifdef VDA_TS
  unsigned long long tsa[10] = {0, 0, 0, 0, 0, 0, 0, 0, 0, 0};
  unsigned tsn[10] = {0, 0, 0, 0, 0, 0, 0, 0, 0, 0};
  const unsigned long long ts_rt0 = __builtin_amdgcn_s_memrealtime();
  const unsigned long long ts_c0 = __builtin_amdgcn_s_memtime();
  unsigned long long ts_prev = ts_c0, tsw = 0;
#endif
  for (int gs = 0; gs < my_steps; ++gs) {
    const bool issue_p = st == 0 && u + 1 < my_units;
    if (issue_p) ud_next = make_ud(u + 1);
    if (gs + 1 < my_steps) {
      if (st + 1 < SPU) dma_w(st + 1, slab, (gs + 1) & 1);
      else dma_w(0, slab + 1 == nslab ? 0 : slab + 1, (gs + 1) & 1);
    }
    if constexpr (!UPS) {
      if (issue_p)
        for (int j = 0; j < my_pp; ++j) dma_patch(u + 1, ud_next, wave + j * 8);
    }
    {
      const h16* pb = patch + (u & 1) * PBUF;
      const h16* wb = wbuf + (gs & 1) * WBUF;
      unsigned xs, ws;
      asm volatile("s_mov_b32 %0, %1" : "=s"(xs)
                   : "s"((unsigned)((pb - patch) * 2 + ((st / 3) * DP + (st % 3)) * PSTR * 16)));
      asm volatile("s_mov_b32 %0, %1" : "=s"(ws) : "s"((unsigned)((wb - wbuf) * 2)));
      const char* pxb = reinterpret_cast<const char*>(patch) + xs + lin_x;
      const char* wxb[ND];
#pragma unroll
      for (int d = 0; d < ND; ++d) wxb[d] = reinterpret_cast<const char*>(wbuf) + ws + lin_w[d];
#pragma unroll
      for (int d = 0; d < ND; ++d) {
        h8 wf[NB], xf[4];
#pragma unroll
        for (int a = 0; a < NB; ++a) wf[a] = *reinterpret_cast<const h8*>(wxb[d] + a * 16 * CPX * 16);
#pragma unroll
        for (int i = 0; i < 4; ++i) xf[i] = *reinterpret_cast<const h8*>(pxb + i * DP * PSTR * 16 + d * 64);
#pragma unroll
        for (int a = 0; a < NB; ++a)
#pragma unroll
          for (int i = 0; i < 4; ++i) acc[a][i] = mfma16(wf[a], xf[i], acc[a][i]);
      }
    }
    const bool tile_end = st == SPU - 1 && slab == units_per_tile - 1;
    if (tile_end) {
      int bt, y0, x0;
      tile_of_unit(u, bt, y0, x0);
      const __amdgpu_buffer_rsrc_t ys = __builtin_amdgcn_make_buffer_rsrc(
          (void*)(yout + (long)bt * H * W * CO), (short)0, (int)((long)H * W * CO * 2), 0x00020000);
      const bool godd = (g & 1) != 0;
#pragma unroll
      for (int a = 0; a < NB; a += 2) {
        const f4 bv0 = bias_r[a], bv1 = bias_r[a + 1];
#pragma unroll
        for (int i = 0; i < 4; ++i) {
          const int y = y0 + mg * 4 + i, x = x0 + frow;
          const f4 v0 = acc[a][i] + bv0, v1 = acc[a + 1][i] + bv1;
          h4 o0, o1;
#pragma unroll
          for (int r = 0; r < 4; ++r) {
            o0[r] = (h16)(relu_out ? fmaxf(v0[r], 0.f) : v0[r]);
            o1[r] = (h16)(relu_out ? fmaxf(v1[r], 0.f) : v1[r]);
          }
          const uint2 u0 = __builtin_bit_cast(uint2, o0), u1 = __builtin_bit_cast(uint2, o1);
          const uint2 snd = godd ? u0 : u1;
          float ax, bx, ay, by;
          swap16_pair(__builtin_bit_cast(float, snd.x), ax, bx);
          swap16_pair(__builtin_bit_cast(float, snd.y), ay, by);
          const uint2 rcv = make_uint2(__builtin_bit_cast(unsigned, godd ? ax : bx), __builtin_bit_cast(unsigned, godd ? ay : by));
          const u32x4 val = godd ? u32x4{rcv.x, rcv.y, u1.x, u1.y} : u32x4{u0.x, u0.y, rcv.x, rcv.y};
          const int n = (ng * NB + a + (godd ? 1 : 0)) * 16 + (g & 2) * 4;
          const unsigned vo = (y < H && x < W) ? (unsigned)(((y * W + x) * CO + n) * 2) : 0x80000000u;
          __builtin_amdgcn_raw_buffer_store_b128(val, ys, vo, 0, 0);
          acc[a][i] = f4{0.f, 0.f, 0.f, 0.f};
          acc[a + 1][i] = f4{0.f, 0.f, 0.f, 0.f};
        }
      }
    }
#ifdef VDA_TS
    const unsigned long long ts_pre = __builtin_amdgcn_s_memtime();
#endif
    if constexpr (UPS) {
      if (tile_end) wait_vmcnt<NB / 2 * 4>();
      else wait_vmcnt<0>();
    } else if (issue_p) {
      if (my_pp == PPMAX) wait_vmcnt<PPMAX>();
      else wait_vmcnt<PPMAX - 1>();
    } else {
      wait_vmcnt<0>();
    }
    __builtin_amdgcn_s_barrier();
#ifdef VDA_TS
    {
      const unsigned long long now = __builtin_amdgcn_s_memtime();
      const int cls = tile_end ? SPU : st;
#pragma unroll
      for (int c = 0; c <= SPU && c < 10; ++c)
        if (c == cls) { tsa[c] += now - ts_prev; ++tsn[c]; }
      tsw += now - ts_pre;
      ts_prev = now;
    }
#endif
    if (++st == SPU) {
      st = 0;
      ++u;
      if (++slab == nslab) slab = 0;
    }
  }
#ifdef VDA_TS
  if (UPS && tid == 0 && blockIdx.x < 1024) {
    const unsigned long long rt = __builtin_amdgcn_s_memrealtime() - ts_rt0, cy = __builtin_amdgcn_s_memtime() - ts_c0;
    for (int c = 0; c < 10; ++c) { g_dts[blockIdx.x][c] = tsa[c]; g_dts[blockIdx.x][10 + c] = tsn[c]; }
    g_dts[blockIdx.x][20] = rt;
    g_dts[blockIdx.x][21] = cy;
    g_dts[blockIdx.x][22] = tsw;
  }
#endif
}

}

#ifdef VDA_TS
extern "C" int vda_debug_oc1_timestamps(void* host) {
  return (int)hipMemcpyFromSymbol(host, HIP_SYMBOL(g_dts), sizeof(g_dts), 0, hipMemcpyDeviceToHost);
}
#endif

int vda_conv_halo_fused(const void* x, const void* w, void* y, const float* bias, int relu, int BT, int Hs, int Ws,
                        int H, int W, int Cin, int Cout, hipStream_t st) {
  if (Cout != CO || Cin % CS != 0 || Hs > H || Ws > W || Hs < 1 || Ws < 1) return 1;
  if ((long)H * W * Cout * 2 >= (1L << 31)) return 1;
  if (!halo_fused_fits(Hs, Ws, H, W)) return 1;
  HaloGrid g;
  if (!halo_tile_grid(BT, H, W, DT, 1, 0x7fffffffL, g)) return vda_set_error(-22, "conv: too many tiles");
  hipLaunchKernelGGL(halo_conv_kernel<true>, dim3(g.grid), dim3(768), 0, st, (const h16*)x, (const h16*)w, bias, (h16*)y,
                     relu, H, W, Cin, g.tiles_x, g.tiles_y, g.ntiles, Hs, Ws);
  VDA_LAUNCH_CHECK();
  return 0;
}

int vda_conv_halo(const void* x, const void* w, void* y, const float* bias, int relu, int BT, int H, int W, int Cin,
                  int Cout, hipStream_t st) {
  if (Cout != CO || Cin % CS != 0) return 1;
  if ((long)H * W * Cout * 2 >= (1L << 31)) return 1;
  HaloGrid g;
  if (!halo_tile_grid(BT, H, W, DT, 1, 0x7fffffffL, g)) return vda_set_error(-22, "conv: too many tiles");
  hipLaunchKernelGGL(halo_conv_kernel<false>, dim3(g.grid), dim3(512), 0, st, (const h16*)x, (const h16*)w, bias,
                     (h16*)y, relu, H, W, Cin, g.tiles_x, g.tiles_y, g.ntiles, 0, 0);
  VDA_LAUNCH_CHECK();
  return 0;
}
```

video-depth-anything_amd/csrc/vda_torch.cpp:

```cpp
#include <ATen/ATen.h>
#include <ATen/DeviceGuard.h>
#include <c10/hip/HIPStream.h>
#include <torch/library.h>

#include <array>
#include <cstring>

#include "vda.h"

namespace {

using at::Tensor;
using c10::optional;
using OptT = const optional<Tensor>&;

void* stream_of(const Tensor& t) {
  return (void*)c10::hip::getCurrentHIPStream(t.device().index()).stream();
}

void check_rc(int rc, const char* what) {
  TORCH_CHECK(rc == 0, what, " failed (rc=", rc, "): ", vda_last_error());
}

void need(const Tensor& t, at::ScalarType dt, const char* name, const Tensor& like) {
// ... 73 lines not shown
                 OptT res, OptT res2, int64_t act, OptT ln_stats, OptT ln_colsum, int64_t ln_parts, double ln_eps,
                 OptT stats_out, OptT sched, int64_t drop_period, Tensor out) {
  const auto dt = act_dtype(x);
  TORCH_CHECK(x.dim() == 2 && x.stride(1) == 1, "vda gemm: x must be a 2-D row-major (possibly row-strided) matrix");
  need_contig(w, dt, "w", x);
  TORCH_CHECK(w.dim() == 2 && w.size(1) == x.size(1), "vda gemm: K mismatch ", w.sizes(), " vs ", x.sizes());
  const int64_t M = x.size(0), K = x.size(1), N = w.size(0);
  const int64_t nout = act == VDA_ACT_GEGLU ? N / 2 : N;
  TORCH_CHECK(drop_period >= 0, "vda gemm: drop_period >= 0");
  const int64_t Mo = gemm_out_rows(M, drop_period);
  TORCH_CHECK(out.dim() == 2 && out.size(0) == Mo && out.size(1) == nout && out.stride(1) == 1 &&
                  out.scalar_type() == dt && out.device() == x.device(),
              "vda gemm: out must be [", Mo, ", ", nout, "] ", dt, " with unit column stride");
  if (stats_out)
    TORCH_CHECK(stats_out->dim() == 3 && stats_out->size(0) >= M && stats_out->size(1) == (nout + 255) / 256 &&
                    stats_out->size(2) == 2 && stats_out->scalar_type() == at::kFloat && stats_out->is_contiguous(),
                "vda gemm: stats_out must be a contiguous float [M, ceil(N / 256), 2]");
  if (x.is_meta()) return out;
  const at::OptionalDeviceGuard g(x.device());
  vda_epilogue e = make_epi(x, bias, rowbias, rdiv, rmod, gamma, res, res2, act, dt, ln_stats, ln_colsum, ln_parts,
                            ln_eps, stats_out);
  if (sched) {
    need_contig(*sched, at::kInt, "sched", x);
    TORCH_CHECK(sched->numel() >= 9, "vda gemm: sched must hold >= 9 int32 counters");
    e.sched = (int32_t*)sched->data_ptr();
  }
  e.drop_period = (int32_t)drop_period;
  const int rc = dt == at::kHalf
                     ? vda_gemm(x.data_ptr(), x.stride(0), w.data_ptr(), out.data_ptr(), out.stride(0), (int32_t)M,
                                (int32_t)N, (int32_t)K, &e, stream_of(x))
                     : vda_gemm_f32((const float*)x.data_ptr(), x.stride(0), (const float*)w.data_ptr(),
                                    (float*)out.data_ptr(), out.stride(0), (int32_t)M, (int32_t)N, (int32_t)K, &e,
                                    stream_of(x));
  check_rc(rc, "vda_gemm");
  return out;
}

Tensor gemm(const Tensor& x, const Tensor& w, OptT bias, OptT rowbias, int64_t rdiv, int64_t rmod, OptT gamma,
            OptT res, OptT res2, int64_t act, OptT ln_stats, OptT ln_colsum, int64_t ln_parts, double ln_eps,
            OptT stats_out, OptT sched, int64_t drop_period) {
  const auto dt = act_dtype(x);
  TORCH_CHECK(x.dim() == 2 && w.dim() == 2, "vda gemm: x and w must be 2-D");
  const int64_t nout = act == VDA_ACT_GEGLU ? w.size(0) / 2 : w.size(0);
  Tensor out = at::empty({gemm_out_rows(x.size(0), drop_period), nout}, x.options().dtype(dt));
  return gemm_into(x, w, bias, rowbias, rdiv, rmod, gamma, res, res2, act, ln_stats, ln_colsum, ln_parts, ln_eps,
                   stats_out, sched, drop_period, out);
}

Tensor& gemm_out(const Tensor& x, const Tensor& w, OptT bias, OptT rowbias, int64_t rdiv, int64_t rmod, OptT gamma,
                 OptT res, OptT res2, int64_t act, OptT ln_stats, OptT ln_colsum, int64_t ln_parts, double ln_eps,
                 OptT stats_out, OptT sched, int64_t drop_period, Tensor& out) {
  gemm_into(x, w, bias, rowbias, rdiv, rmod, gamma, res, res2, act, ln_stats, ln_colsum, ln_parts, ln_eps, stats_out,
            sched, drop_period, out);
  return out;
}

Tensor conv_transpose_ks(const Tensor& x, const Tensor& w, const Tensor& bias, int64_t BT, int64_t h, int64_t w_,
                         int64_t k) {
  const auto dt = act_dtype(x);
  TORCH_CHECK(x.dim() == 2 && x.is_contiguous(), "vda conv_transpose_ks: x must be a contiguous [BT*h*w, Cin] matrix");
  need_contig(w, dt, "w", x);
  need_contig(bias, at::kFloat, "bias", x);
  const int64_t M = x.size(0), K = x.size(1), N = w.size(0);
  TORCH_CHECK(k > 0 && N % (k * k) == 0 && w.size(1) == K && M == BT * h * w_, "vda conv_transpose_ks: bad geometry");
  const int64_t cout = N / (k * k);
  Tensor out = at::empty({BT, h * k, w_ * k, cout}, x.options());
  if (x.is_meta()) return out;
  const at::OptionalDeviceGuard g(x.device());
  vda_epilogue e;
  std::memset(&e, 0, sizeof(e));
  e.bias = (const float*)bias.data_ptr();
  e.rdiv = e.rmod = 1;
  e.store = VDA_STORE_PIXEL_SHUFFLE;
  e.ps_k = (int32_t)k; e.ps_cout = (int32_t)cout; e.ps_hin = (int32_t)h; e.ps_win = (int32_t)w_;
  const int rc = dt == at::kHalf
                     ? vda_gemm(x.data_ptr(), K, w.data_ptr(), out.data_ptr(), N, (int32_t)M, (int32_t)N, (int32_t)K,
                                &e, stream_of(x))
                     : vda_gemm_f32((const float*)x.data_ptr(), K, (const float*)w.data_ptr(), (float*)out.data_ptr(),
                                    N, (int32_t)M, (int32_t)N, (int32_t)K, &e, stream_of(x));
  check_rc(rc, "vda_gemm(pixel-shuffle)");
  return out;
}

Tensor upsample_bilinear(const Tensor& x, int64_t Ho, int64_t Wo);
Tensor conv2d(const Tensor& x, const Tensor& w, int64_t ks, int64_t stride, int64_t pad, OptT bias, bool pre_relu,
              int64_t act, OptT res, OptT res2, at::OptionalIntArrayRef up) {
  const auto dt = act_dtype(x);
  TORCH_CHECK(x.dim() == 4 && x.is_contiguous(), "vda conv2d: x must be a contiguous NHWC [BT, H, W, Cin] map");
  need_contig(w, dt, "w", x);
  const int64_t BT = x.size(0), H = x.size(1), W = x.size(2), Cin = x.size(3), Cout = w.size(0);
  TORCH_CHECK(w.dim() == 4 && w.size(1) == ks && w.size(2) == ks && w.size(3) == Cin, "vda conv2d: weight ",
              w.sizes(), " vs Cin=", Cin, " ks=", ks);
  int64_t uh = 0, uw = 0;
  if (up.has_value()) {
    TORCH_CHECK(up->size() == 2, "vda conv2d: up must be (Hu, Wu)");
    uh = (*up)[0];
    uw = (*up)[1];
  }
  const int64_t Hi = uh > 0 ? uh : H, Wi = uw > 0 ? uw : W;
  const int64_t Ho = (Hi + 2 * pad - ks) / stride + 1, Wo = (Wi + 2 * pad - ks) / stride + 1;
  Tensor out = at::empty({BT, Ho, Wo, Cout}, x.options());
  if (x.is_meta()) return out;
  const at::OptionalDeviceGuard g(x.device());
  optional<Tensor> r, r2;
  if (res) r = res->reshape({-1, Cout});
  int32_t r2h = 0, r2w = 0;
  if (res2) {
    Tensor s2 = *res2;
    if (s2.dim() == 4 && (s2.size(1) != Ho || s2.size(2) != Wo)) {
      TORCH_CHECK(s2.size(0) == BT && s2.size(3) == Cout && s2.size(1) <= Ho && s2.size(2) <= Wo && s2.is_contiguous(),
                  "vda conv2d: a res2 of another grid must be a contiguous [BT, h <= Ho, w <= Wo, Cout] map, got ",
                  s2.sizes());
      if (dt != at::kFloat && uh == 0 && vda_conv2d_res2_upsample_ok(BT, H, W, Cin, Cout, ks, stride, pad)) {
        r2h = (int32_t)s2.size(1);
        r2w = (int32_t)s2.size(2);
      } else {
        s2 = upsample_bilinear(s2, Ho, Wo);
      }
    }
    r2 = s2.reshape({-1, Cout});
  }
  vda_epilogue e = make_epi(x, bias, c10::nullopt, 1, 1, c10::nullopt, r, r2, act, dt);
  e.res2_h = r2h;
  e.res2_w = r2w;
  int rc;
  if (dt == at::kFloat) {
    TORCH_CHECK(uh == 0, "vda conv2d: the fused-upsample loader is fp16-only");
    rc = vda_conv2d_f32((const float*)x.data_ptr(), (const float*)w.data_ptr(), (float*)out.data_ptr(), BT, H, W,
                        Cin, Cout, ks, stride, pad, pre_relu ? 1 : 0, &e, stream_of(x));
  } else {
    const int64_t wsb = uh > 0 ? 0 : vda_conv2d_workspace(BT, H, W, Cin, Cout, ks, stride, pad);
    Tensor ws;
    if (wsb > 0) ws = at::empty({wsb}, x.options().dtype(at::kByte));
    rc = vda_conv2d(x.data_ptr(), w.data_ptr(), out.data_ptr(), BT, H, W, Cin, Cout, ks, stride, pad,
                    pre_relu ? 1 : 0, uh, uw, &e, wsb > 0 ? ws.data_ptr() : nullptr, wsb, stream_of(x));
  }
  check_rc(rc, "vda_conv2d");
  return out;
}

Tensor layernorm(const Tensor& x, const Tensor& gamma, const Tensor& beta, double eps, int64_t skip_period,
                 optional<int64_t> rows) {
  const auto dt = act_dtype(x);
  TORCH_CHECK(x.dim() == 2 && x.stride(1) == 1, "vda layernorm: x must be a 2-D row-major (possibly row-strided) matrix");
  const int64_t R = x.size(0), C = x.size(1);
  const int64_t nr = rows.has_value() ? *rows : (skip_period == 0 ? R : (R / (skip_period + 1)) * skip_period);
  Tensor out = at::empty({nr, C}, x.options());
  if (x.is_meta()) return out;
  const at::OptionalDeviceGuard g(x.device());
  need_contig(gamma, at::kFloat, "gamma", x);
  need_contig(beta, at::kFloat, "beta", x);
  const int rc = dt == at::kHalf
                     ? vda_layernorm(x.data_ptr(), x.stride(0), out.data_ptr(), (const float*)gamma.data_ptr(),
                                     (const float*)beta.data_ptr(), (int32_t)nr, (int32_t)C, (float)eps,
                                     (int32_t)skip_period, stream_of(x))
                     : vda_layernorm_f32((const float*)x.data_ptr(), x.stride(0), (float*)out.data_ptr(),
                                         (const float*)gamma.data_ptr(), (const float*)beta.data_ptr(), (int32_t)nr,
                                         (int32_t)C, (float)eps, (int32_t)skip_period, stream_of(x));
  check_rc(rc, "vda_layernorm");
  return out;
}

Tensor row_stats(const Tensor& x, double eps) {
  TORCH_CHECK(x.scalar_type() == at::kHalf && x.dim() == 2 && x.stride(1) == 1,
              "vda row_stats: x must be a 2-D row-major fp16 matrix");
  const int64_t R = x.size(0), C = x.size(1);
  Tensor out = at::empty({(R + 1) / 2 * 2, 2}, x.options().dtype(at::kFloat));
  if (x.is_meta()) return out;
  const at::OptionalDeviceGuard g(x.device());
  check_rc(vda_row_stats(x.data_ptr(), x.stride(0), (float*)out.data_ptr(), (int32_t)R, (int32_t)C, (float)eps,
                         stream_of(x)),
           "vda_row_stats");
  return out;
}

Tensor groupnorm(const Tensor& x, const Tensor& gamma, const Tensor& beta, int64_t frames, int64_t groups, double eps) {
  const auto dt = act_dtype(x);
  TORCH_CHECK(x.dim() == 2 && x.is_contiguous(), "vda groupnorm: x must be a contiguous [F*S, C] matrix");
  TORCH_CHECK(frames > 0 && x.size(0) % frames == 0, "vda groupnorm: rows must be a multiple of frames");
  Tensor out = at::empty_like(x);
  if (x.is_meta()) return out;
  const at::OptionalDeviceGuard g(x.device());
  need_contig(gamma, at::kFloat, "gamma", x);
  need_contig(beta, at::kFloat, "beta", x);
  const int64_t C = x.size(1), S = x.size(0) / frames;
  int rc;
  if (dt == at::kFloat) {
    rc = vda_groupnorm_f32((const float*)x.data_ptr(), (float*)out.data_ptr(), (const float*)gamma.data_ptr(),
                           (const float*)beta.data_ptr(), frames, S, C, groups, (float)eps, stream_of(x));
  } else {
    const int64_t nws = vda_groupnorm_workspace(frames, S, C, groups);
    Tensor ws = at::empty({std::max<int64_t>(nws, 1)}, x.options().dtype(at::kFloat));
    rc = vda_groupnorm(x.data_ptr(), out.data_ptr(), (const float*)gamma.data_ptr(), (const float*)beta.data_ptr(),
                       frames, S, C, groups, (float)eps, (float*)ws.data_ptr(), stream_of(x));
  }
  check_rc(rc, "vda_groupnorm");
  return out;
}

Tensor groupnorm_linear(const Tensor& x, const Tensor& gamma, const Tensor& beta, int64_t frames, int64_t groups,
                        double eps, const Tensor& w, OptT bias, OptT stats_out) {
  const auto dt = act_dtype(x);
  TORCH_CHECK(x.dim() == 2 && x.is_contiguous(), "vda groupnorm_linear: x must be a contiguous [F*S, C] matrix");
  TORCH_CHECK(frames > 0 && x.size(0) % frames == 0, "vda groupnorm_linear: rows must be a multiple of frames");
  TORCH_CHECK(w.dim() == 2 && w.size(1) == x.size(1), "vda groupnorm_linear: w must be [N, C], got ", w.sizes());
  const int64_t M = x.size(0), C = x.size(1), N = w.size(0), S = M / frames;
  if (stats_out)
// ... 351 lines not shown
  if (payload.is_meta() || N == 0) return out;
  const at::OptionalDeviceGuard g(payload.device());
  check_rc(vda_yuv_to_rgb((const uint8_t*)payload.data_ptr(), (int32_t)N, (int32_t)h, (int32_t)w, stride,
                          (int32_t)chroma, (uint8_t*)out.data_ptr(), stream_of(payload)),
           "vda_yuv_to_rgb");
  return out;
}

Tensor preprocess_yuv(const Tensor& payload, int64_t h, int64_t w, int64_t chroma, int64_t H, int64_t W,
                      at::ArrayRef<double> mean, at::ArrayRef<double> std) {
  const int64_t stride = yuv_frame_stride(payload, h, w, chroma, "vda preprocess_yuv");
  TORCH_CHECK(mean.size() == 3 && std.size() == 3, "vda preprocess_yuv: mean / std need 3 values");
  TORCH_CHECK(H >= 1 && W >= 1 && H <= INT32_MAX && W <= INT32_MAX, "vda preprocess_yuv: H and W must be positive");
  const int64_t N = payload.size(0);
  TORCH_CHECK(N <= 65535, "vda preprocess_yuv: N <= 65535 frames per call");
  Tensor out = at::empty({N, 3, H, W}, payload.options().dtype(at::kFloat));
  if (payload.is_meta() || N == 0) return out;
  const at::OptionalDeviceGuard g(payload.device());
  const float m3[3] = {(float)mean[0], (float)mean[1], (float)mean[2]};
  const float s3[3] = {(float)std[0], (float)std[1], (float)std[2]};
  const int64_t wsb = vda_preprocess_yuv_workspace((int32_t)N, (int32_t)h, (int32_t)w, (int32_t)H, (int32_t)W);
  Tensor ws;
  if (wsb > 0) ws = at::empty({wsb}, payload.options());
  check_rc(vda_preprocess_yuv((const uint8_t*)payload.data_ptr(), (int32_t)N, (int32_t)h, (int32_t)w, stride,
                              (int32_t)chroma, (float*)out.data_ptr(), (int32_t)H, (int32_t)W, m3, s3,
                              wsb > 0 ? ws.data_ptr() : nullptr, wsb, stream_of(payload)),
           "vda_preprocess_yuv");
  return out;
}

void need_tables(const Tensor& k, const Tensor& b, int64_t in, int64_t out, const char* axis, const Tensor& like) {
  need_contig(k, at::kInt, axis, like);
  need_contig(b, at::kInt, axis, like);
  const int64_t taps = vda_resample_taps((int32_t)in, (int32_t)out);
  TORCH_CHECK(k.dim() == 2 && k.size(0) == out && k.size(1) == taps, "vda yuv_downscale: the ", axis,
              " coefficients must be [", out, ", ", taps, "] for ", in, " -> ", out, ", got ", k.sizes());
  TORCH_CHECK(b.dim() == 2 && b.size(0) == out && b.size(1) == 2, "vda yuv_downscale: the ", axis,
              " bounds must be [", out, ", 2], got ", b.sizes());
}

Tensor yuv_downscale(const Tensor& payload, int64_t h, int64_t w, int64_t chroma, int64_t h2, int64_t w2,
                     const Tensor& kx, const Tensor& bx, const Tensor& ky, const Tensor& by) {
  const int64_t stride = yuv_frame_stride(payload, h, w, chroma, "vda yuv_downscale");
  TORCH_CHECK(h2 >= 1 && w2 >= 1 && w2 <= INT32_MAX, "vda yuv_downscale: h2 and w2 must be positive");
  const int64_t N = payload.size(0);
  TORCH_CHECK(N <= 65535 && h2 <= 65535, "vda yuv_downscale: N and h2 <= 65535 per call");
  need_tables(kx, bx, w, w2, "horizontal", payload);
  need_tables(ky, by, h, h2, "vertical", payload);
  TORCH_CHECK(vda_yuv_downscale_ok((int32_t)h, (int32_t)w, (int32_t)h2, (int32_t)w2) == 1, "vda yuv_downscale: ", h, "x", w,
              " -> ", h2, "x", w2, " is beyond the kernel's ratio (vda_yuv_downscale_ok)");
  Tensor out = at::empty({N, h2, w2, 3}, payload.options());
  if (payload.is_meta() || N == 0) return out;
  const at::OptionalDeviceGuard g(payload.device());
  const int64_t wsb = vda_yuv_downscale_workspace((int32_t)N, (int32_t)h, (int32_t)w, (int32_t)h2, (int32_t)w2);
  Tensor ws;
  if (wsb > 0) ws = at::empty({wsb}, payload.options());
  check_rc(vda_yuv_downscale((const uint8_t*)payload.data_ptr(), (int32_t)N, (int32_t)h, (int32_t)w, stride,
                             (int32_t)chroma, (const int32_t*)kx.data_ptr(), (const int32_t*)bx.data_ptr(),
                             (const int32_t*)ky.data_ptr(), (const int32_t*)by.data_ptr(), (uint8_t*)out.data_ptr(),
                             (int32_t)h2, (int32_t)w2, wsb > 0 ? ws.data_ptr() : nullptr, wsb, stream_of(payload)),
           "vda_yuv_downscale");
  return out;
}

}

TORCH_LIBRARY(vda, m) {
  m.def("yuv_to_rgb(Tensor payload, int h, int w, int chroma) -> Tensor");
  m.def("yuv_downscale(Tensor payload, int h, int w, int chroma, int h2, int w2, Tensor kx, Tensor bx, Tensor ky, "
        "Tensor by) -> Tensor");
  m.def("preprocess_yuv(Tensor payload, int h, int w, int chroma, int H, int W, float[] mean, float[] std) -> Tensor");
  m.def("depth_range(Tensor depth) -> Tensor");
  m.def("depth_colorize(Tensor depth, Tensor range, Tensor? lut, int layout) -> Tensor");
  m.def("gemm(Tensor x, Tensor w, Tensor? bias=None, Tensor? rowbias=None, int rdiv=1, int rmod=1, "
        "Tensor? gamma=None, Tensor? res=None, Tensor? res2=None, int act=0, Tensor? ln_stats=None, "
        "Tensor? ln_colsum=None, int ln_parts=0, float ln_eps=1e-6, Tensor(b!)? stats_out=None, "
        "Tensor(c!)? sched=None, int drop_period=0) -> Tensor");
  m.def("gemm.out(Tensor x, Tensor w, Tensor? bias=None, Tensor? rowbias=None, int rdiv=1, int rmod=1, "
        "Tensor? gamma=None, Tensor? res=None, Tensor? res2=None, int act=0, Tensor? ln_stats=None, "
        "Tensor? ln_colsum=None, int ln_parts=0, float ln_eps=1e-6, Tensor(b!)? stats_out=None, "
        "Tensor(c!)? sched=None, int drop_period=0, *, Tensor(a!) out) -> Tensor(a!)");
  m.def("row_stats(Tensor x, float eps) -> Tensor");
  m.def("conv_transpose_ks(Tensor x, Tensor w, Tensor bias, int BT, int h, int w_, int k) -> Tensor");
  m.def("conv2d(Tensor x, Tensor w, int ks=3, int stride=1, int pad=1, Tensor? bias=None, bool pre_relu=False, "
        "int act=0, Tensor? res=None, Tensor? res2=None, int[]? up=None) -> Tensor");
  m.def("layernorm(Tensor x, Tensor gamma, Tensor beta, float eps, int skip_period=0, int? rows=None) -> Tensor");
  m.def("groupnorm(Tensor x, Tensor gamma, Tensor beta, int frames, int groups, float eps) -> Tensor");
  m.def("groupnorm_linear(Tensor x, Tensor gamma, Tensor beta, int frames, int groups, float eps, Tensor w, "
        "Tensor? bias=None, Tensor(b!)? stats_out=None) -> Tensor");
  m.def("spatial_attention(Tensor qkv, int B, int N, int H, int D=64) -> Tensor");
  m.def("temporal_attention(Tensor qkv, int B, int T, int S, int H, int D, float rope_theta=0.) -> Tensor");
  m.def("upsample_bilinear(Tensor x, int Ho, int Wo) -> Tensor");
  m.def("patch_im2col(Tensor img, int Kp, ScalarType dtype=float16) -> Tensor");
  m.def("depth_head(Tensor x, Tensor w1, Tensor b1, Tensor w2, Tensor b2, int Ho, int Wo) -> Tensor");
  m.def("preprocess_frames(Tensor frames, int H, int W, float[] mean, float[] std) -> Tensor");
  m.def("depth_resize(Tensor depth, int ho, int wo) -> Tensor");
  m.def("scale_shift(Tensor pred, Tensor target, Tensor? mask=None) -> (Tensor ss, Tensor sums)");
  m.def("depth_align(Tensor src, int ho, int wo, Tensor? ss=None, bool clip=True, Tensor? pre=None, "
        "float[]? w_pre=None, float[]? w_post=None, Tensor(a!)? out=None) -> Tensor");
  m.def("depth_eval_fit(Tensor pred, Tensor gt, Tensor? valid=None, bool per_frame=False) -> (Tensor ss, Tensor sums)");
  m.def("depth_eval_metrics(Tensor pred, Tensor gt, Tensor? valid, Tensor ss, float max_depth=80., "
        "bool want_aligned=False) -> (Tensor frame_sums, Tensor total, Tensor? aligned)");
}

#define VDA_IMPL(KEY)                                         \
  TORCH_LIBRARY_IMPL(vda, KEY, m) {                           \
    m.impl("gemm", &gemm);                                    \
    m.impl("gemm.out", &gemm_out);                            \
    m.impl("conv_transpose_ks", &conv_transpose_ks);          \
    m.impl("conv2d", &conv2d);                                \
    m.impl("layernorm", &layernorm);                          \
    m.impl("row_stats", &row_stats);                          \
    m.impl("groupnorm", &groupnorm);                          \
    m.impl("groupnorm_linear", &groupnorm_linear);            \
    m.impl("spatial_attention", &spatial_attention);          \
    m.impl("temporal_attention", &temporal_attention);        \
    m.impl("upsample_bilinear", &upsample_bilinear);          \
    m.impl("patch_im2col", &patch_im2col);                    \
    m.impl("depth_head", &depth_head);                        \
    m.impl("preprocess_frames", &preprocess_frames);          \
    m.impl("depth_resize", &depth_resize);                    \
    m.impl("scale_shift", &scale_shift);                      \
    m.impl("depth_align", &depth_align);                      \
    m.impl("depth_eval_fit", &depth_eval_fit);                \
    m.impl("depth_eval_metrics", &depth_eval_metrics);        \
    m.impl("depth_range", &depth_range);                      \
    m.impl("depth_colorize", &depth_colorize);                \
    m.impl("yuv_to_rgb", &yuv_to_rgb);                        \
    m.impl("preprocess_yuv", &preprocess_yuv);                \
    m.impl("yuv_downscale", &yuv_downscale);                  \
  }

VDA_IMPL(CUDA)
VDA_IMPL(Meta)
```

video-depth-anything_amd/model.py:

```python
from __future__ import annotations

import math
from typing import Dict, List, Optional

import torch
import torch.nn as nn
import torch.nn.functional as F

from . import ops
from ._lib import ACT_GELU, ACT_GEGLU, ACT_RELU

PATCH = 14
ENCODER_CFG = {
    "vits": dict(embed_dim=384, depth=12, heads=6, taps=[2, 5, 8, 11]),
    "vitb": dict(embed_dim=768, depth=12, heads=12, taps=[2, 5, 8, 11]),
    "vitl": dict(embed_dim=1024, depth=24, heads=16, taps=[4, 11, 17, 23]),
}
MODEL_CONFIGS = {
    "vits": dict(encoder="vits", features=64, out_channels=[48, 96, 192, 384]),
    "vitb": dict(encoder="vitb", features=128, out_channels=[96, 192, 384, 768]),
    "vitl": dict(encoder="vitl", features=256, out_channels=[256, 512, 1024, 1024]),
}


# ... 107 lines not shown

class TemporalTransformerBlock(nn.Module):
    def __init__(self, dim, max_len, pe="ape"):
        super().__init__()
        self.attention_blocks = nn.ModuleList([TemporalAttention(dim, max_len, pe) for _ in range(2)])
        self.norms = nn.ModuleList([nn.LayerNorm(dim) for _ in range(2)])
        self.ff = FeedForward(dim)
        self.ff_norm = nn.LayerNorm(dim)


class TemporalTransformer3DModel(nn.Module):
    def __init__(self, C, max_len, pe="ape"):
        super().__init__()
        self.norm = nn.GroupNorm(32, C, eps=1e-6, affine=True)
        self.proj_in = nn.Linear(C, C)
        self.transformer_blocks = nn.ModuleList([TemporalTransformerBlock(C, max_len, pe)])
        self.proj_out = nn.Linear(C, C)


class TemporalModule(nn.Module):
    def __init__(self, C, max_len=32, pe="ape"):
        super().__init__()
        self.temporal_transformer = TemporalTransformer3DModel(C, max_len, pe)


class DPTHeadTemporal(nn.Module):
    def __init__(self, in_channels, features, out_channels, num_frames=32, pe="ape", use_bn=False,
                 use_clstoken=False):
        super().__init__()
        self.use_clstoken = use_clstoken
        self.projects = nn.ModuleList([nn.Conv2d(in_channels, oc, 1) for oc in out_channels])
        if use_clstoken:
            self.readout_projects = nn.ModuleList([
                nn.Sequential(nn.Linear(2 * in_channels, in_channels), nn.GELU()) for _ in out_channels])
        self.resize_layers = nn.ModuleList([
            nn.ConvTranspose2d(out_channels[0], out_channels[0], 4, 4, 0),
            nn.ConvTranspose2d(out_channels[1], out_channels[1], 2, 2, 0),
            nn.Identity(),
            nn.Conv2d(out_channels[3], out_channels[3], 3, 2, 1),
        ])
        s = nn.Module()
        s.layer1_rn = nn.Conv2d(out_channels[0], features, 3, 1, 1, bias=False)
        s.layer2_rn = nn.Conv2d(out_channels[1], features, 3, 1, 1, bias=False)
        s.layer3_rn = nn.Conv2d(out_channels[2], features, 3, 1, 1, bias=False)
        s.layer4_rn = nn.Conv2d(out_channels[3], features, 3, 1, 1, bias=False)
        s.refinenet1 = FeatureFusionBlock(features, use_bn)
        s.refinenet2 = FeatureFusionBlock(features, use_bn)
        s.refinenet3 = FeatureFusionBlock(features, use_bn)
        s.refinenet4 = FeatureFusionBlock(features, use_bn)
        s.output_conv1 = nn.Conv2d(features, features // 2, 3, 1, 1)
        s.output_conv2 = nn.Sequential(nn.Conv2d(features // 2, 32, 3, 1, 1), nn.ReLU(True),
                                       nn.Conv2d(32, 1, 1, 1, 0), nn.ReLU(True), nn.Identity())
        self.scratch = s
        self.motion_modules = nn.ModuleList([
            TemporalModule(out_channels[2], num_frames, pe), TemporalModule(out_channels[3], num_frames, pe),
            TemporalModule(features, num_frames, pe), TemporalModule(features, num_frames, pe)])


def _f(t):
    return t.detach().to(torch.float32).contiguous()


def _geglu_interleave(t):
    inner = t.shape[0] // 2
    hh, gg = t[:inner], t[inner:]
    blocks = []
    for p in range(0, inner, 16):
        blocks += [hh[p:p + 16], gg[p:p + 16]]
    return torch.cat(blocks, 0)


class _Packed:
    pass


class VideoDepthAnything(nn.Module):

    fold_layernorms: bool = True
    epilogue_stats: bool = True
    dynamic_tiles: bool = False
    fold_ff_norm: bool = False
    fuse_groupnorm_linear: bool = True
    fold_tap_norm: bool = True

    def __init__(self, encoder="vitl", features=256, out_channels=(256, 512, 1024, 1024), use_bn=False,
                 use_clstoken=False, num_frames=32, pe="ape"):
        super().__init__()
        if pe not in ("ape", "rope"):
            raise NotImplementedError(pe)
        self.pe = pe
        self.use_bn, self.use_clstoken = bool(use_bn), bool(use_clstoken)
        self.intermediate_layer_idx = {k: v["taps"] for k, v in ENCODER_CFG.items()}
        self.encoder = encoder
        self.num_frames = num_frames
        self.features = features
        self.out_channels = list(out_channels)
        self.pretrained = DinoVisionTransformer(encoder)
        self.head = DPTHeadTemporal(self.pretrained.embed_dim, features, self.out_channels, num_frames, pe,
                                    self.use_bn, self.use_clstoken)
        self._packed: Dict[str, _Packed] = {}
        self._pos_cache: Dict[tuple, torch.Tensor] = {}

    @classmethod
    def from_config(cls, encoder: str, device="meta", pe: str = "ape", use_bn: bool = False,
                    use_clstoken: bool = False):
        with torch.device(device):
            m = cls(**MODEL_CONFIGS[encoder], pe=pe, use_bn=use_bn, use_clstoken=use_clstoken)
        return m

    def load_state_dict(self, state_dict, strict: bool = True, assign: bool = False):
        self._packed.clear()
        self._pos_cache.clear()
        return super().load_state_dict(state_dict, strict=strict, assign=assign)

    @torch.no_grad()
    def _pack(self, device, fp32: bool = False) -> _Packed:
        key = f"{device}|{'f32' if fp32 else 'f16'}|{int(bool(self.fold_layernorms))}"
        if key in self._packed:
            return self._packed[key]
        dev = torch.device(device)
        wd = torch.float32 if fp32 else torch.float16
        _h = lambda t: t.detach().to(wd).contiguous()
        _conv_nhwc = lambda w: _h(w.detach().permute(0, 2, 3, 1))
        P = _Packed()
        P.fp32, P.dt = fp32, wd
        enc = self.pretrained
        C = enc.embed_dim
        P.C, P.heads = C, enc.num_heads
        P.Kp = 588 if fp32 else 640
        wpe = enc.patch_embed.proj.weight.reshape(C, -1)
        P.patch_w = _h(F.pad(wpe, (0, P.Kp - wpe.shape[1]))).to(dev)
        P.patch_b = _f(enc.patch_embed.proj.bias).to(dev)
        P.cls = _f(enc.cls_token.reshape(C)).to(dev)
        P.pos = _f(enc.pos_embed).to(dev)
        P.blocks = []
        P.lnfold = not fp32 and bool(self.fold_layernorms)

        def _ln_fold(weight, bias, ln):
            w = weight.detach().float()
            wg = (w * ln.weight.detach().float()[None, :]).to(wd).contiguous()
            c1 = wg.float().sum(1).contiguous()
            bb = (w @ ln.bias.detach().float() + bias.detach().float()).contiguous()
            return wg.to(dev), c1.to(dev), bb.to(dev)

        for b in enc.blocks:
            q = _Packed()
            q.n1w, q.n1b = _f(b.norm1.weight).to(dev), _f(b.norm1.bias).to(dev)
            if P.lnfold:
                q.qkv_w, q.qkv_c1, q.qkv_b = _ln_fold(b.attn.qkv.weight, b.attn.qkv.bias, b.norm1)
            else:
                q.qkv_w, q.qkv_b = _h(b.attn.qkv.weight).to(dev), _f(b.attn.qkv.bias).to(dev)
            g1 = b.ls1.gamma.detach().float()
            q.proj_w = _h(b.attn.proj.weight.detach().float() * g1[:, None]).to(dev)
            q.proj_b = _f(b.attn.proj.bias.detach().float() * g1).to(dev)
            q.n2w, q.n2b = _f(b.norm2.weight).to(dev), _f(b.norm2.bias).to(dev)
            if P.lnfold:
                q.fc1_w, q.fc1_c1, q.fc1_b = _ln_fold(b.mlp.fc1.weight, b.mlp.fc1.bias, b.norm2)
            else:
                q.fc1_w, q.fc1_b = _h(b.mlp.fc1.weight).to(dev), _f(b.mlp.fc1.bias).to(dev)
            g2 = b.ls2.gamma.detach().float()
            q.fc2_w = _h(b.mlp.fc2.weight.detach().float() * g2[:, None]).to(dev)
            q.fc2_b = _f(b.mlp.fc2.bias.detach().float() * g2).to(dev)
            P.blocks.append(q)
        P.nw, P.nb = _f(enc.norm.weight).to(dev), _f(enc.norm.bias).to(dev)

        hd = self.head
# ... 37 lines not shown
                    setattr(q, f"r{u}c{c}_b", _f(b).to(dev))
            P.ref[i] = q
        P.oc1_w, P.oc1_b = _conv_nhwc(s.output_conv1.weight).to(dev), _f(s.output_conv1.bias).to(dev)
        oc2 = s.output_conv2
        w1 = oc2[0].weight.detach().float().permute(0, 2, 3, 1)
        if fp32:
            P.oc2_w1 = w1.contiguous().to(dev)
        else:
            w1_hi = w1.half()
            w1_lo = (w1 - w1_hi.float()).half()
            P.oc2_w1 = torch.cat([w1_hi, w1_lo], 0).contiguous().to(dev)
        P.oc2_b1 = _f(oc2[0].bias).to(dev)
        P.oc2_w2 = _f(oc2[2].weight.reshape(-1)).to(dev)
        P.oc2_b2 = _f(oc2[2].bias).to(dev)

        P.mm = []
        for m in hd.motion_modules:
            tt = m.temporal_transformer
            q = _Packed()
            Cm = tt.proj_in.weight.shape[0]
            q.C = Cm
            q.gnw, q.gnb = _f(tt.norm.weight).to(dev), _f(tt.norm.bias).to(dev)
            q.pin_w, q.pin_b = _h(tt.proj_in.weight).to(dev), _f(tt.proj_in.bias).to(dev)
            q.pout_w, q.pout_b = _h(tt.proj_out.weight).to(dev), _f(tt.proj_out.bias).to(dev)
            blk = tt.transformer_blocks[0]
            q.attn = []
            for ab, nrm in zip(blk.attention_blocks, blk.norms):
                a = _Packed()
                a.nw, a.nb = _f(nrm.weight).to(dev), _f(nrm.bias).to(dev)
                wqkv = torch.cat([ab.to_q.weight, ab.to_k.weight, ab.to_v.weight], 0).float()
                a.qkv_w = _h(wqkv).to(dev)
                a.pe_bias = (_f(ab.pos_encoder.pe[0].float() @ wqkv.t()).to(dev)
                             if ab.pos_encoder is not None else None)
                a.fold = not fp32 and bool(self.fold_layernorms) and a.pe_bias is not None and (3 * Cm) % 256 == 0
                if a.fold:
                    a.qkv_wg = (wqkv * nrm.weight.detach().float()[None, :]).half().contiguous().to(dev)
                    a.qkv_cs = a.qkv_wg.float().sum(1).contiguous()
                    a.qkv_bb = (wqkv @ nrm.bias.detach().float()).contiguous().to(dev)
                a.out_w, a.out_b = _h(ab.to_out[0].weight).to(dev), _f(ab.to_out[0].bias).to(dev)
                q.attn.append(a)
            q.ffnw, q.ffnb = _f(blk.ff_norm.weight).to(dev), _f(blk.ff_norm.bias).to(dev)
            q.ff1_w = _h(_geglu_interleave(blk.ff.net[0].proj.weight)).to(dev)
            q.ff1_b = _f(_geglu_interleave(blk.ff.net[0].proj.bias)).to(dev)
            q.fffold = not fp32 and bool(self.fold_layernorms)
            if q.fffold:
                w1 = blk.ff.net[0].proj.weight.detach().float()
                q.ff1_wg = _geglu_interleave(w1 * blk.ff_norm.weight.detach().float()[None, :]).half().contiguous().to(dev)
                q.ff1_cs = q.ff1_wg.float().sum(1).contiguous()
                q.ff1_bb = _geglu_interleave(w1 @ blk.ff_norm.bias.detach().float()
                                             + blk.ff.net[0].proj.bias.detach().float()).contiguous().to(dev)
            q.ff2_w, q.ff2_b = _h(blk.ff.net[2].weight).to(dev), _f(blk.ff.net[2].bias).to(dev)
            P.mm.append(q)
        self._packed[key] = P
        return P

    def _token_bias(self, P: _Packed, H: int, W: int, device) -> torch.Tensor:
        key = (H, W, str(device))
        if key in self._pos_cache:
            return self._pos_cache[key]
        pos = P.pos
        N0 = pos.shape[1] - 1
        ph, pw = H // PATCH, W // PATCH
        if ph * pw == N0 and H == W:
            pe = pos[0]
        else:
            s0 = math.sqrt(N0)
            C = pos.shape[-1]
            pp = pos[:, 1:].reshape(1, int(s0), int(s0), C).permute(0, 3, 1, 2)
            pp = F.interpolate(pp, scale_factor=((ph + 0.1) / s0, (pw + 0.1) / s0), mode="bicubic",
                               antialias=False)
            assert pp.shape[-2:] == (ph, pw)
            pe = torch.cat([pos[0, :1], pp.permute(0, 2, 3, 1).reshape(ph * pw, C)], 0)
        tb = pe.clone()
        tb[0] += P.cls
        tb[1:] += P.patch_b
        tb = tb.contiguous()
        self._pos_cache[key] = tb
        return tb

    @torch.no_grad()
    def prepare(self, device, size, fp32: bool = False) -> None:
        P = self._pack(torch.device(device), fp32)
        self._token_bias(P, int(size[0]), int(size[1]), torch.device(device))

    def _qkv_fold(self, q: _Packed, M: int, S: int, T: int) -> List[bool]:
        ok = any(a.fold for a in q.attn) and ops.gemm_accepts(M, 3 * q.C, q.C, ln_fold=True, ln_parts=(q.C + 255) // 256,
                                                              rowbias=True, rdiv=S, rmod=T)
        return [bool(a.fold and ok) for a in q.attn]

    def _temporal(self, q: _Packed, x: torch.Tensor, B: int, T: int, S: int) -> torch.Tensor:
        C = q.C
        M = x.shape[0]
        fold = self._qkv_fold(q, M, S, T)
        fffold = q.fffold and bool(self.fold_ff_norm)
        st = torch.empty(M + 1, (C + 255) // 256, 2, device=x.device) if any(fold) or fffold else None
        if self.fuse_groupnorm_linear:
            h = ops.groupnorm_linear(x, q.gnw, q.gnb, B * T, 32, 1e-6, q.pin_w, bias=q.pin_b,
                                     stats_out=st if fold[0] else None)
        else:
            xn = ops.groupnorm(x, q.gnw, q.gnb, B * T, 32, 1e-6)
            h = ops.gemm(xn, q.pin_w, bias=q.pin_b, stats_out=st if fold[0] else None)
        for i, a in enumerate(q.attn):
            if fold[i]:
                qkv = ops.gemm(h, a.qkv_wg, bias=a.qkv_bb, rowbias=a.pe_bias, rdiv=S, rmod=T, ln_stats=st,
                               ln_parts=st.shape[1], ln_eps=1e-5, ln_colsum=a.qkv_cs)
                at = ops.temporal_attention(qkv, B, T, S, 8, C // 8)
            else:
                n = ops.layernorm(h, a.nw, a.nb, 1e-5)
                if a.pe_bias is not None:
                    qkv = ops.gemm(n, a.qkv_w, rowbias=a.pe_bias, rdiv=S, rmod=T)
                    at = ops.temporal_attention(qkv, B, T, S, 8, C // 8)
                else:
                    qkv = ops.gemm(n, a.qkv_w)
                    at = ops.temporal_attention(qkv, B, T, S, 8, C // 8, rope_theta=10000.0)
            nxt = fold[i + 1] if i + 1 < len(q.attn) else fffold
            h = ops.gemm(at, a.out_w, bias=a.out_b, res=h, out=h, stats_out=st if nxt else None)
        if fffold:
            g = ops.gemm(h, q.ff1_wg, bias=q.ff1_bb, act=ACT_GEGLU, ln_stats=st, ln_parts=st.shape[1], ln_eps=1e-5,
                         ln_colsum=q.ff1_cs)
        else:
            n = ops.layernorm(h, q.ffnw, q.ffnb, 1e-5)
            g = ops.gemm(n, q.ff1_w, bias=q.ff1_b, act=ACT_GEGLU)
        h = ops.gemm(g, q.ff2_w, bias=q.ff2_b, res=h, out=h)
        return ops.gemm(h, q.pout_w, bias=q.pout_b, res=x)

    def _fusion(self, q: _Packed, x0, x1, size):
        if x1 is not None:
            t = ops.conv2d(x1, q.r1c1_w, bias=q.r1c1_b, pre_relu=True, act=ACT_RELU)
            out = ops.conv2d(t, q.r1c2_w, bias=q.r1c2_b, res=x1, res2=x0)
        else:
            out = x0
        t = ops.conv2d(out, q.r2c1_w, bias=q.r2c1_b, pre_relu=True, act=ACT_RELU)
        out = ops.conv2d(t, q.r2c2_w, bias=q.r2c2_b, res=out)
        BT, h, w, Cf = out.shape
        y = ops.gemm(out.view(-1, Cf), q.out_w, bias=q.out_b).view(BT, h, w, Cf)
        return y, size

    def _check_input(self, x: torch.Tensor, T: int):
        if not x.is_cuda:
            raise RuntimeError("VideoDepthAnything (MI355X) runs on the GPU only; move the model input to cuda")
        Cc, H, W = x.shape[-3:]
        if Cc != 3:
            raise ValueError(f"expected 3 input channels, got {Cc}")
        if H % PATCH or W % PATCH:
            raise AssertionError(f"Input image size ({H}x{W}) is not a multiple of the patch size {PATCH}")
        if T > self.num_frames:
            raise ValueError(f"clip length {T} exceeds the temporal PE table ({self.num_frames})")

    def _encode(self, P: _Packed, img: torch.Tensor):
        BT, _, H, W = img.shape
        npt = (H // PATCH) * (W // PATCH)
        ntok = npt + 1
        a = ops.patch_im2col(img.float().contiguous(), P.Kp, dtype=P.dt)
        tok = ops.gemm(a, P.patch_w, rowbias=self._token_bias(P, H, W, img.device), rdiv=1, rmod=ntok)
        del a
        taps = self.intermediate_layer_idx[self.encoder]
        feats: List[torch.Tensor] = []
        cls: Optional[List[torch.Tensor]] = [] if self.use_clstoken else None
        C = P.C
        nparts = (C + 255) // 256
        epistats = P.lnfold and nparts <= 4 and bool(self.epilogue_stats)
        if epistats:
            st_a = torch.empty(tok.shape[0], nparts, 2, device=tok.device, dtype=torch.float32)
            st_b = torch.empty_like(st_a)
        stats, parts = None, 0
        sch = ops.sched_counters(tok.device) if self.dynamic_tiles and P.dt == torch.float16 else None
        tapfold = epistats and self._tap_fold(P, BT, ntok)
        for i, q in enumerate(P.blocks):
            if P.lnfold:
                if stats is None:
                    stats, parts = ops.row_stats(tok, 1e-6), 0
                qkv = ops.gemm(tok, q.qkv_w, bias=q.qkv_b, ln_stats=stats, ln_parts=parts, ln_eps=1e-6,
                               ln_colsum=q.qkv_c1, sched=sch)
            else:
                qkv = ops.gemm(ops.layernorm(tok, q.n1w, q.n1b, 1e-6), q.qkv_w, bias=q.qkv_b)
            at = ops.spatial_attention(qkv, BT, ntok, P.heads, 64)
            del qkv
            ops.gemm(at, q.proj_w, bias=q.proj_b, res=tok, out=tok, stats_out=st_a if epistats else None, sched=sch)
            if P.lnfold:
                if epistats:
                    stats, parts = st_a, nparts
                else:
                    stats, parts = ops.row_stats(tok, 1e-6), 0
                f = ops.gemm(tok, q.fc1_w, bias=q.fc1_b, act=ACT_GELU, ln_stats=stats, ln_parts=parts, ln_eps=1e-6,
                             ln_colsum=q.fc1_c1, sched=sch, tag="enc_fc1")
            else:
                f = ops.gemm(ops.layernorm(tok, q.n2w, q.n2b, 1e-6), q.fc1_w, bias=q.fc1_b, act=ACT_GELU,
                             tag="enc_fc1")
            last = i + 1 == len(P.blocks)
            ops.gemm(f, q.fc2_w, bias=q.fc2_b, res=tok, out=tok,
                     stats_out=st_b if epistats and (not last or (tapfold and i in taps)) else None, sched=sch)
            stats, parts = (st_b, nparts) if epistats else (None, 0)
            del f
            if i in taps and tapfold:
                w_, c1_, b_ = P.projf[len(feats)]
                feats.append(ops.gemm(tok, w_, bias=b_, ln_stats=st_b, ln_parts=nparts, ln_eps=1e-6, ln_colsum=c1_,
                                      drop_period=ntok))
            elif i in taps:
                feats.append(ops.layernorm(tok, P.nw, P.nb, 1e-6, skip_period=npt))
                if cls is not None:
                    cls.append(ops.layernorm(tok.view(BT, ntok, -1)[:, 0], P.nw, P.nb, 1e-6))
        return feats, cls, tapfold

    def _tap_fold(self, P: _Packed, BT: int, ntok: int) -> bool:
        if not (P.lnfold and bool(self.fold_tap_norm) and getattr(P, "projf", None) is not None):
            return False
        nparts = (P.C + 255) // 256
        return all(ops.gemm_accepts(BT * ntok, w.shape[0], P.C, ln_fold=True, ln_parts=nparts, drop_period=ntok)
                   for w, _, _ in P.projf)

    def _reassemble(self, P: _Packed, enc, BT: int, ph: int, pw: int) -> List[torch.Tensor]:
        feats, cls, projected = enc
        oc = self.out_channels
        lay = []
        for i, ft in enumerate(feats):
            if cls is not None:
                rb = ops.gemm(cls[i].float(), P.ro_wb[i], bias=P.ro_b[i])
                ft = ops.gemm(ft, P.ro_wa[i], rowbias=rb, rdiv=ph * pw, rmod=BT, act=ACT_GELU)
            p = ft if projected else ops.gemm(ft, P.proj_w[i], bias=P.proj_b[i])
            if i == 0:
                l = ops.conv_transpose_ks(p, P.rs_w[0], P.rs_b[0], BT, ph, pw, 4)
            elif i == 1:
                l = ops.conv_transpose_ks(p, P.rs_w[1], P.rs_b[1], BT, ph, pw, 2)
            elif i == 2:
                l = p.view(BT, ph, pw, oc[2])
            else:
                l = ops.conv2d(p.view(BT, ph, pw, oc[3]), P.rs_w[3], ks=3, stride=2, pad=1, bias=P.rs_b[3])
            lay.append(l)
        return lay

    def _head(self, P: _Packed, l1, l2, l3, l4, B: int, T: int, ph: int, pw: int, skip_tmp_block: bool,
              sel: Optional[List[int]] = None) -> torch.Tensor:
        oc = self.out_channels
        BT = B * T
        h3, w3 = l3.shape[1:3]
        h4, w4 = l4.shape[1:3]
        l3 = self._temporal(P.mm[0], l3.reshape(-1, oc[2]), B, T, h3 * w3).view(BT, h3, w3, oc[2])
        l4 = self._temporal(P.mm[1], l4.reshape(-1, oc[3]), B, T, h4 * w4).view(BT, h4, w4, oc[3])
        r1 = ops.conv2d(l1, P.rn[0])
        r2 = ops.conv2d(l2, P.rn[1])
        r3 = ops.conv2d(l3, P.rn[2])
        r4 = ops.conv2d(l4, P.rn[3])
        del l1, l2, l3, l4
        Fh = self.features
        y, _ = self._fusion(P.ref[4], r4, None, None)
        p4 = ops.upsample_bilinear(y, r3.shape[1], r3.shape[2])
        if not skip_tmp_block:
            p4 = self._temporal(P.mm[2], p4.view(-1, Fh), B, T, h3 * w3).view(p4.shape)
        y, _ = self._fusion(P.ref[3], p4, r3, None)
        p3 = ops.upsample_bilinear(y, r2.shape[1], r2.shape[2])
        p3 = self._temporal(P.mm[3], p3.view(-1, Fh), B, T, p3.shape[1] * p3.shape[2]).view(p3.shape)
        if sel is not None:
            p3 = p3.index_select(0, torch.tensor(sel, dtype=torch.long, device=p3.device))
        y, _ = self._fusion(P.ref[2], p3, r2, None)
        y, _ = self._fusion(P.ref[1], y, r1, None)
        H1, W1 = 2 * y.shape[1], 2 * y.shape[2]
        if P.fp32:
            o1 = ops.conv2d(ops.upsample_bilinear(y, H1, W1), P.oc1_w, bias=P.oc1_b)
        else:
            o1 = ops.conv2d(y, P.oc1_w, bias=P.oc1_b, up=(H1, W1))
        if P.fp32:
            return ops.depth_head_f32(o1, P.oc2_w1, P.oc2_b1, P.oc2_w2, P.oc2_b2, ph * PATCH, pw * PATCH)
        return ops.depth_head(o1, P.oc2_w1, P.oc2_b1, P.oc2_w2, P.oc2_b2, ph * PATCH, pw * PATCH)

    @torch.no_grad()
    def forward(self, x: torch.Tensor, skip_tmp_block: bool = False, *, fp32: bool = False) -> torch.Tensor:
        B, T, Cc, H, W = x.shape
        self._check_input(x, T)
        P = self._pack(x.device, fp32)
        BT = B * T
        ph, pw = H // PATCH, W // PATCH
        feats = self._encode(P, x.reshape(BT, 3, H, W))
        lay = self._reassemble(P, feats, BT, ph, pw)
        del feats
        depth = self._head(P, *lay, B, T, ph, pw, skip_tmp_block)
        return depth.view(B, T, H, W)

    @torch.no_grad()
    def get_motion_features(self, x: torch.Tensor, *, fp32: bool = False):
        if x.dim() == 5:
            x = x.flatten(0, 1)
        N, _, H, W = x.shape
        self._check_input(x, 1)
        P = self._pack(x.device, fp32)
        return tuple(self._reassemble(P, self._encode(P, x), N, H // PATCH, W // PATCH))

    @torch.no_grad()
    def forward_single_image(self, x: torch.Tensor, motion_features, pred_depth_idx=None, inference_length: int = 32,
                             skip_tmp_block: bool = False, *, fp32: bool = False):
        B, T1, Cc, H, W = x.shape
        T = int(inference_length)
        self._check_input(x, T)
        if B * T1 != 1:
            raise ValueError("forward_single_image takes one frame [1, 1, 3, H, W]")
        P = self._pack(x.device, fp32)
        ph, pw = H // PATCH, W // PATCH
        new = self._reassemble(P, self._encode(P, x.reshape(1, 3, H, W)), 1, ph, pw)
        o1, o2, o3, o4 = motion_features
        if o3.shape[0] + 1 != T or o4.shape[0] + 1 != T:
            raise ValueError(f"context must hold inference_length - 1 = {T - 1} frames, got {o3.shape[0]}")
        if pred_depth_idx is not None:
            pidx = [int(i) for i in pred_depth_idx]
            if pidx and not all(-o1.shape[0] <= i < o1.shape[0] for i in pidx):
                bad = next(i for i in pidx if not -o1.shape[0] <= i < o1.shape[0])
                raise IndexError(f"index {bad} is out of bounds for dimension 0 with size {o1.shape[0]}")
            it = torch.tensor([i if i >= 0 else i + o1.shape[0] for i in pidx], dtype=torch.long, device=x.device)
            l1 = torch.cat([o1.index_select(0, it), new[0]], 0)
            l2 = torch.cat([o2.index_select(0, it), new[1]], 0)
            sel = [i if i >= 0 else i + T for i in pidx] + [T - 1]
        else:
            l1, l2, sel = new[0], new[1], [T - 1]
        l3 = torch.cat([o3, new[2]], 0)
        l4 = torch.cat([o4, new[3]], 0)
        depth = self._head(P, l1, l2, l3, l4, 1, T, ph, pw, skip_tmp_block, sel=sel)
        return depth.view(1, len(sel), H, W), tuple(new)

    def infere_single_image(self, frames, target_fps, input_size=518, device="cuda", fp32=False, warmup=True,
                            inference_length=32, keyframe_list=(0, 12), align_each_new_frame=True,
                            skip_tmp_block=False, stitch="host"):
        from .stream import infere_single_image
        return infere_single_image(_StreamEngine(self, fp32), frames, target_fps, input_size=input_size, device=device,
                                   warmup=warmup, inference_length=inference_length, keyframe_list=keyframe_list,
                                   align_each_new_frame=align_each_new_frame, skip_tmp_block=skip_tmp_block,
                                   stitch=stitch)


class _StreamEngine:

    def __init__(self, m: VideoDepthAnything, fp32: bool = False):
        self.m = m
        self.fp32 = fp32

    def motion_features(self, x):
        return self.m.get_motion_features(x, fp32=self.fp32)

    def predict(self, x, old, pred_idx, T, skip_tmp_block=False):
        d, new = self.m.forward_single_image(x.unsqueeze(0), old, pred_idx, T, skip_tmp_block, fp32=self.fp32)
        return d[0], new


def _infer_video_depth(self, frames, target_fps, input_size=518, device="cuda", fp32=False, skip_tmp_block=False,
                       windows_per_batch=1, rank=0, world=1, group=None, streams=2, stitch="host",
                       return_device=False):
    from .video import infer_video_depth
    return infer_video_depth(lambda x: self.forward(x, skip_tmp_block, fp32=fp32), frames, target_fps, input_size=input_size,
                             device=device, windows_per_batch=windows_per_batch, rank=rank, world=world,
                             group=group, streams=streams, prepare=lambda hw: self.prepare(device, hw, fp32),
                             stitch=stitch, return_device=return_device)


VideoDepthAnything.infer_video_depth = _infer_video_depth


def _evaluate_video_depth(self, frames, target_fps, gt, valid=None, *, max_depth=80., align="all", **infer_kwargs):
    from .evaluate import evaluate_video_depth
    return evaluate_video_depth(self, frames, target_fps, gt, valid, max_depth=max_depth, align=align, **infer_kwargs)


# ... 13 lines not shown
```

video-depth-anything_amd/ops.py:

```python
from __future__ import annotations

import functools
from typing import Optional

import torch

from . import _lib
from ._lib import ACT_NONE, ACT_GELU, ACT_GEGLU, ACT_RELU, STORE_ROWS, STORE_PIXEL_SHUFFLE

Tensor = torch.Tensor


_PROBE: Optional[dict] = None


def enable_probe(tags):
    global _PROBE
    _PROBE = {t: [] for t in tags}


def take_probe():
    global _PROBE
    out = {}
    if _PROBE:
        torch.cuda.synchronize()
        out = {t: [(a.elapsed_time(b), fl) for a, b, fl in ev] for t, ev in _PROBE.items()}
    _PROBE = None
    return out


def _vda():
    return _lib.torch_ops()


def _need(t: Tensor, dtype, name: str):
    if not t.is_cuda:
        raise RuntimeError(f"vda op: {name} must be a GPU tensor (no CPU path in the product)")
    if t.dtype != dtype:
        raise RuntimeError(f"vda op: {name} must be {dtype}, got {t.dtype}")


def gemm(x: Tensor, w: Tensor, *, bias=None, rowbias=None, rdiv=1, rmod=1, gamma=None, res=None,
         res2=None, act=ACT_NONE, ln_stats=None, ln_colsum=None, ln_parts=0, ln_eps=1e-6, stats_out=None,
         sched=None, drop_period=0, out: Optional[Tensor] = None, tag: Optional[str] = None) -> Tensor:
    _need(x, x.dtype, "x")
    probe = _PROBE is not None and tag in _PROBE
    if probe:
        ev0, ev1 = torch.cuda.Event(enable_timing=True), torch.cuda.Event(enable_timing=True)
        ev0.record()
    v = _vda()
    if out is None:
        out = v.gemm(x, w, bias, rowbias, int(rdiv), int(rmod), gamma, res, res2, int(act), ln_stats, ln_colsum,
                     int(ln_parts), float(ln_eps), stats_out, sched, int(drop_period))
    else:
        v.gemm.out(x, w, bias, rowbias, int(rdiv), int(rmod), gamma, res, res2, int(act), ln_stats, ln_colsum,
                   int(ln_parts), float(ln_eps), stats_out, sched, int(drop_period), out=out)
    if probe:
        ev1.record()
        _PROBE[tag].append((ev0, ev1, 2.0 * x.shape[0] * w.shape[0] * x.shape[1]))
    return out


@functools.lru_cache(maxsize=None)
def gemm_accepts(M: int, N: int, K: int, *, bias=True, ln_fold=False, ln_parts=0, rowbias=False, rdiv=1, rmod=1,
                 drop_period=0, act=ACT_NONE, res=False, stats_out=False, ldx=None, ldy=None) -> bool:
    ptr = lambda on: 0x1000 if on else None
    ny = N // 2 if act == ACT_GEGLU else N
    e = _lib.Epilogue(bias=ptr(bias), rowbias=ptr(rowbias), rdiv=int(rdiv), rmod=int(rmod), res=ptr(res), ldres=ny,
                      act=int(act), ln_stats=ptr(ln_fold), ln_colsum=ptr(ln_fold), ln_parts=int(ln_parts),
                      stats_out=ptr(stats_out), drop_period=int(drop_period))
    return _lib.lib().vda_gemm_check(int(K if ldx is None else ldx), int(ny if ldy is None else ldy), int(M), int(N),
                                     int(K), e) == 0


_SCHED = {}


def sched_counters(device=None) -> Tensor:
    dev = torch.device("cuda", torch.cuda.current_device()) if device is None else torch.device(device)
    st = torch.cuda.current_stream(dev)
    key = (dev.index, st.cuda_stream)
    t = _SCHED.get(key)
    if t is None:
        t = torch.zeros(16, dtype=torch.int32, device=dev)
        _SCHED[key] = t
    return t


def conv_transpose_ks(x: Tensor, w: Tensor, bias: Tensor, BT: int, h: int, w_: int, k: int) -> Tensor:
    _need(x, x.dtype, "x")
    return _vda().conv_transpose_ks(x, w, bias, int(BT), int(h), int(w_), int(k))


def conv2d(x: Tensor, w: Tensor, *, ks=3, stride=1, pad=1, bias=None, pre_relu=False, act=ACT_NONE,
           res=None, res2=None, up=None) -> Tensor:
    _need(x, x.dtype, "x")
    return _vda().conv2d(x, w, int(ks), int(stride), int(pad), bias, bool(pre_relu), int(act), res, res2,
                         None if up is None else [int(up[0]), int(up[1])])


def layernorm(x: Tensor, gamma: Tensor, beta: Tensor, eps: float, *, skip_period: int = 0,
              rows: Optional[int] = None) -> Tensor:
    _need(x, x.dtype, "x")
    return _vda().layernorm(x, gamma, beta, float(eps), int(skip_period), rows)


def row_stats(x: Tensor, eps: float) -> Tensor:
    _need(x, torch.float16, "x")
    return _vda().row_stats(x, float(eps))


def groupnorm(x: Tensor, gamma: Tensor, beta: Tensor, frames: int, groups: int, eps: float) -> Tensor:
    _need(x, x.dtype, "x")
    return _vda().groupnorm(x, gamma, beta, int(frames), int(groups), float(eps))


def groupnorm_linear(x: Tensor, gamma: Tensor, beta: Tensor, frames: int, groups: int, eps: float, w: Tensor, *,
                     bias=None, stats_out=None) -> Tensor:
    _need(x, x.dtype, "x")
    return _vda().groupnorm_linear(x, gamma, beta, int(frames), int(groups), float(eps), w, bias, stats_out)


def spatial_attention(qkv: Tensor, B: int, N: int, H: int, D: int = 64) -> Tensor:
    _need(qkv, qkv.dtype, "qkv")
    return _vda().spatial_attention(qkv, int(B), int(N), int(H), int(D))


def temporal_attention(qkv: Tensor, B: int, T: int, S: int, H: int, D: int, rope_theta: float = 0.0) -> Tensor:
    _need(qkv, qkv.dtype, "qkv")
    return _vda().temporal_attention(qkv, int(B), int(T), int(S), int(H), int(D), float(rope_theta))


def upsample_bilinear(x: Tensor, Ho: int, Wo: int) -> Tensor:
    _need(x, x.dtype, "x")
    return _vda().upsample_bilinear(x, int(Ho), int(Wo))


def patch_im2col(img: Tensor, Kp: int, dtype=torch.float16) -> Tensor:
    _need(img, torch.float32, "img")
    return _vda().patch_im2col(img, int(Kp), dtype)


def depth_head(x: Tensor, w1_split: Tensor, b1: Tensor, w2: Tensor, b2: Tensor, Ho: int, Wo: int) -> Tensor:
    _need(x, torch.float16, "x")
    return _vda().depth_head(x, w1_split, b1, w2, b2, int(Ho), int(Wo))


def depth_head_f32(x: Tensor, w1: Tensor, b1: Tensor, w2: Tensor, b2: Tensor, Ho: int, Wo: int) -> Tensor:
    _need(x, torch.float32, "x")
    return _vda().depth_head(x, w1, b1, w2, b2, int(Ho), int(Wo))


def preprocess_frames(frames: Tensor, H: int, W: int, mean=(0.485, 0.456, 0.406), std=(0.229, 0.224, 0.225)) -> Tensor:
    _need(frames, torch.uint8, "frames")
    if frames.dim() != 4 or frames.shape[-1] != 3:
        raise ValueError(f"frames must be [N, h, w, 3] uint8, got {tuple(frames.shape)}")
    return _vda().preprocess_frames(frames, int(H), int(W), [float(v) for v in mean], [float(v) for v in std])


def depth_resize(depth: Tensor, ho: int, wo: int) -> Tensor:
    _need(depth, torch.float32, "depth")
    return _vda().depth_resize(depth, int(ho), int(wo))


def scale_shift(pred: Tensor, target: Tensor, *, mask: Optional[Tensor] = None):
    _need(pred, torch.float32, "pred")
    _need(target, torch.float32, "target")
    if pred.numel() != target.numel() or pred.numel() < 1:
        raise ValueError(f"pred and target need the same, non-zero number of elements, got {pred.numel()} and {target.numel()}")
    if mask is not None:
        _need(mask, torch.uint8, "mask")
        if mask.numel() != pred.numel():
            raise ValueError(f"mask has {mask.numel()} elements, pred {pred.numel()}")
    return _vda().scale_shift(pred, target, mask)


def depth_align(src: Tensor, ho: int, wo: int, *, ss: Optional[Tensor] = None, clip: bool = True,
                pre: Optional[Tensor] = None, w_pre=None, w_post=None, out: Optional[Tensor] = None) -> Tensor:
    _need(src, torch.float32, "src")
    if src.dim() != 3 or not 1 <= src.shape[0] <= 32:
        raise ValueError(f"src must be [F, H, W] with 1 <= F <= 32, got {tuple(src.shape)}")
# ... 129 lines not shown
```

video-depth-anything_amd/weights.py:

```python
from __future__ import annotations

import math
import zlib
from typing import Dict, Iterable, Tuple

import torch


def _pe_table(C: int, max_len: int) -> torch.Tensor:
    pos = torch.arange(max_len).unsqueeze(1)
    div = torch.exp(torch.arange(0, C, 2) * (-math.log(10000.0) / C))
    pe = torch.zeros(1, max_len, C)
    pe[0, :, 0::2] = torch.sin(pos * div)
    pe[0, :, 1::2] = torch.cos(pos * div)
    return pe


def synthetic_tensor(key: str, shape: Tuple[int, ...]) -> torch.Tensor:
    g = torch.Generator().manual_seed(zlib.crc32(key.encode()) & 0x7FFFFFFF)
    shape = tuple(int(s) for s in shape)
    if key.endswith("pos_encoder.pe"):
        return _pe_table(shape[-1], shape[-2])
    if key.endswith("mask_token"):
        return torch.zeros(shape)
    if key == "head.scratch.output_conv2.2.weight":
        return torch.randn(shape, generator=g).abs() / math.sqrt(32.0)
    if key == "head.scratch.output_conv2.2.bias":
        return torch.full(shape, 0.05)
    leaf = key.rsplit(".", 1)[-1]
    if leaf == "num_batches_tracked":
        return torch.zeros(shape, dtype=torch.long)
    if leaf == "running_var":
        return 0.5 + torch.rand(shape, generator=g)
    if leaf == "running_mean":
        return 0.1 * torch.randn(shape, generator=g)
    if leaf == "gamma":
        return 0.2 + 0.4 * torch.rand(shape, generator=g)
    if leaf == "weight" and len(shape) == 1:
        return 1.0 + 0.1 * torch.randn(shape, generator=g)
    if leaf in ("bias", "cls_token", "pos_embed") or len(shape) == 1:
        return 0.02 * torch.randn(shape, generator=g)
    if key in ("head.resize_layers.0.weight", "head.resize_layers.1.weight"):
        fan_in = shape[0]
    else:
        fan_in = int(math.prod(shape[1:]))
    return torch.randn(shape, generator=g) / math.sqrt(fan_in)


def synthetic_state_dict(key_shapes: Iterable[Tuple[str, Tuple[int, ...]]]) -> Dict[str, torch.Tensor]:
    return {k: synthetic_tensor(k, s) for k, s in key_shapes}


def load_checkpoint(path: str) -> Dict[str, torch.Tensor]:
    sd = torch.load(path, map_location="cpu", weights_only=True)
    if isinstance(sd, dict) and "model" in sd and isinstance(sd["model"], dict):
        sd = sd["model"]
    return sd
```

Measured before the change: 710.4 frames/s.

## Fold transposed-conv resize into following 3x3 conv via sub-pixel GEMM

Composes the head's ConvTranspose (stride 4 and 2) with the following 3x3 layer_rn conv into one sub-pixel GEMM. It uses per-phase composed weights and a 9-class border bias, and scatters outputs directly to the upsampled layout. It also folds the refinenet1 1x1 out_conv into output_conv1's 3x3 weights, using bias9 for border-dependent bias in the fused upsample conv. This removes intermediate full-resolution tensors and separate conv passes, at the cost of larger composed K, fp16 rounding of composed weights, and a new gated kernel path.

```diff
diff --git a/include/vda.h b/include/vda.h
--- a/include/vda.h
+++ b/include/vda.h
@@ -39,6 +39,7 @@
   int32_t res2_h, res2_w;
   int32_t* sched;
   int32_t drop_period;
+  const float* bias9;
 } vda_epilogue;
 
 const char* vda_version(void);
@@ -57,6 +58,12 @@
                              int32_t stride, int32_t pad);
 int vda_conv2d_res2_upsample_ok(int32_t BT, int32_t H, int32_t W, int32_t Cin, int32_t Cout, int32_t ks,
                                 int32_t stride, int32_t pad);
+int vda_conv2d_bias9_ok(int32_t BT, int32_t H, int32_t W, int32_t Cin, int32_t Cout, int32_t up_h, int32_t up_w);
+
+int vda_subpixel_conv(const void* x, const void* w, const float* bias9, void* y, int32_t BT, int32_t h, int32_t w_,
+                      int32_t Cin, int32_t Cout, int32_t s, void* ws, int64_t ws_bytes, void* stream);
+int64_t vda_subpixel_conv_workspace(int32_t BT, int32_t h, int32_t w_, int32_t Cin, int32_t s);
+int vda_subpixel_conv_check(int32_t BT, int32_t h, int32_t w_, int32_t Cin, int32_t Cout, int32_t s);
 
 int vda_layernorm(const void* x, int64_t ldx, void* y, const float* gamma, const float* beta,
                   int32_t rows, int32_t C, float eps, int32_t skip_period, void* stream);
diff --git a/video-depth-anything_amd/_lib.py b/video-depth-anything_amd/_lib.py
--- a/video-depth-anything_amd/_lib.py
+++ b/video-depth-anything_amd/_lib.py
@@ -15,7 +15,8 @@
 EXPORTED = (
     "vda_version", "vda_epilogue_size", "vda_last_error", "vda_gemm", "vda_gemm_check", "vda_conv2d", "vda_conv2d_workspace",
     "vda_layernorm",
-    "vda_conv2d_res2_upsample_ok",
+    "vda_conv2d_res2_upsample_ok", "vda_conv2d_bias9_ok",
+    "vda_subpixel_conv", "vda_subpixel_conv_workspace", "vda_subpixel_conv_check",
     "vda_row_stats", "vda_groupnorm", "vda_groupnorm_workspace",
     "vda_groupnorm_linear", "vda_groupnorm_linear_workspace", "vda_groupnorm_linear_fused",
     "vda_spatial_attention", "vda_temporal_attention", "vda_upsample_bilinear", "vda_patch_im2col",
@@ -55,7 +56,7 @@
         ("ps_cout", c_int32), ("ps_hin", c_int32), ("ps_win", c_int32),
         ("ln_stats", c_void_p), ("ln_colsum", c_void_p), ("ln_parts", c_int32), ("ln_eps", c_float),
         ("stats_out", c_void_p), ("res2_h", c_int32), ("res2_w", c_int32), ("sched", c_void_p),
-        ("drop_period", c_int32),
+        ("drop_period", c_int32), ("bias9", c_void_p),
     ]
 
 
@@ -75,6 +76,10 @@
         "vda_conv2d": ([P, P, P, I, I, I, I, I, I, I, I, I, I, I, EP, P, L, P], I),
         "vda_conv2d_workspace": ([I, I, I, I, I, I, I, I], L),
         "vda_conv2d_res2_upsample_ok": ([I, I, I, I, I, I, I, I], I),
+        "vda_conv2d_bias9_ok": ([I, I, I, I, I, I, I], I),
+        "vda_subpixel_conv": ([P, P, P, P, I, I, I, I, I, I, P, L, P], I),
+        "vda_subpixel_conv_workspace": ([I, I, I, I, I], L),
+        "vda_subpixel_conv_check": ([I, I, I, I, I, I], I),
         "vda_layernorm": ([P, L, P, P, P, I, I, F, I, P], I),
         "vda_row_stats": ([P, L, P, I, I, F, P], I),
         "vda_groupnorm": ([P, P, P, P, I, I, I, I, F, P, P], I),
diff --git a/video-depth-anything_amd/csrc/vda_conv2d.hip b/video-depth-anything_amd/csrc/vda_conv2d.hip
--- a/video-depth-anything_amd/csrc/vda_conv2d.hip
+++ b/video-depth-anything_amd/csrc/vda_conv2d.hip
@@ -33,6 +33,12 @@
                                            int32_t stride, int32_t pad) {
   if (BT <= 0 || H <= 0 || W <= 0 || Cin <= 0 || Cout <= 0) return 0;
   return conv_takes_hconv(BT, H, W, Cin, Cout, ks, stride, pad) ? 1 : 0;
+}
+
+extern "C" int vda_conv2d_bias9_ok(int32_t BT, int32_t H, int32_t W, int32_t Cin, int32_t Cout, int32_t up_h,
+                                   int32_t up_w) {
+  if (BT <= 0 || H <= 0 || W <= 0 || Cin <= 0 || Cout <= 0 || up_h <= 0 || up_w <= 0 || g_force_tile >= 0) return 0;
+  return vda_conv_halo_fused_serves(BT, H, W, up_h, up_w, Cin, Cout) ? 1 : 0;
 }
 
 extern "C" int vda_conv2d(const void* x, const void* w, void* y, int32_t BT, int32_t H, int32_t W,
@@ -73,11 +79,16 @@
     return vda_conv_hconv(x, w, y, p.epi.bias, p.epi.act == VDA_ACT_RELU, pre_relu, p.epi.res, p.epi.res2,
                           p.epi.res2_h, p.epi.res2_w, BT, H, W, Cin, Cout, (hipStream_t)stream);
   }
+  VDA_CHECK_ARG(!p.epi.bias9 || (!p.epi.bias && (uintptr_t)p.epi.bias9 % 16 == 0 && ks == 3 && stride == 1 && pad == 1 &&
+                                 !pre_relu && !p.epi.res && !p.epi.res2 && !p.epi.gamma && !p.epi.rowbias &&
+                                 vda_conv2d_bias9_ok(BT, H, W, Cin, Cout, p.up_h, p.up_w)),
+                "bias9: the 3x3 conv through a fused resize only (vda_conv2d_bias9_ok), 16-byte aligned, in place "
+                "of bias, no residual / gamma / rowbias / pre-ReLU");
   if (p.up_h > 0) {
     if (g_force_tile < 0 && ks == 3 && stride == 1 && pad == 1 && !pre_relu && !p.epi.res && !p.epi.res2 &&
         !p.epi.gamma && !p.epi.rowbias) {
       rc = vda_conv_halo_fused(x, w, y, p.epi.bias, p.epi.act == VDA_ACT_RELU, BT, H, W, p.up_h, p.up_w, Cin, Cout,
-                               (hipStream_t)stream);
+                               (hipStream_t)stream, p.epi.bias9);
       if (rc != 1) return rc;
     }
     return vda_launch_conv_reg(p, (hipStream_t)stream);
diff --git a/video-depth-anything_amd/csrc/vda_f32.hip b/video-depth-anything_amd/csrc/vda_f32.hip
--- a/video-depth-anything_amd/csrc/vda_f32.hip
+++ b/video-depth-anything_amd/csrc/vda_f32.hip
@@ -495,6 +495,7 @@
   VDA_CHECK_ARG(!epi->ln_stats, "fp32 GEMM: no LayerNorm fold (the fp32 mode runs vda_layernorm_f32)");
   VDA_CHECK_ARG(!epi->stats_out, "fp32 GEMM: no row statistics output");
   VDA_CHECK_ARG(epi->res2_h == 0 && epi->res2_w == 0, "fp32 GEMM: no upsampled res2");
+  VDA_CHECK_ARG(!epi->bias9, "fp32 GEMM: no bias9");
   F32Params p{};
   p.x = x; p.ldx = ldx; p.w = w; p.y = y; p.ldy = ldy; p.M = M; p.N = N; p.K = K; p.epi = *epi;
   return launch_f32<false>(p, (hipStream_t)stream);
@@ -508,6 +509,7 @@
   VDA_CHECK_ARG(Cin % 4 == 0 && Cout % 4 == 0, "fp32 conv needs Cin, Cout multiples of 4");
   VDA_CHECK_ARG(epi->act != VDA_ACT_GEGLU && epi->store == VDA_STORE_ROWS, "conv epilogue: no GEGLU / pixel shuffle");
   VDA_CHECK_ARG(epi->res2_h == 0 && epi->res2_w == 0, "fp32 conv: no upsampled res2 (materialise it)");
+  VDA_CHECK_ARG(!epi->bias9, "fp32 conv: no bias9");
   VDA_CHECK_ARG(!epi->rowbias || (epi->rdiv > 0 && epi->rmod > 0), "rowbias needs rdiv, rmod > 0");
   VDA_CHECK_ARG(epi->drop_period == 0, "fp32 conv: no drop_period (vda_gemm only)");
   VDA_CHECK_ARG(!epi->res || epi->ldres % 4 == 0, "fp32 conv needs ldres a multiple of 4");
diff --git a/video-depth-anything_amd/csrc/vda_gemm.hip b/video-depth-anything_amd/csrc/vda_gemm.hip
--- a/video-depth-anything_amd/csrc/vda_gemm.hip
+++ b/video-depth-anything_amd/csrc/vda_gemm.hip
@@ -163,6 +163,7 @@
   if (p.epi.rmod <= 0) p.epi.rmod = 1;
   const vda_epilogue& e = p.epi;
   VDA_CHECK_ARG(e.res2_h == 0 && e.res2_w == 0, "upsampled res2: vda_conv2d only");
+  VDA_CHECK_ARG(!e.bias9, "bias9: vda_conv2d only");
   const GemmRoute r = gemm_route(p, false);
   const bool auto256 = g_force_tile < 0 && r.cfg == 4;
   if (e.drop_period != 0) {
@@ -248,6 +249,17 @@
 
 int vda_launch_conv_gemm(const GemmParams& p, hipStream_t st) { return launch<true>(p, st); }
 
+int vda_launch_subpixel_gemm(const GemmParams& p, hipStream_t st) {
+  if (!phased_dense_ok(p.M, p.N, p.K, p.ldx) || p.N % 256 != 0 || p.N > 8 * 256)
+    return vda_set_error(-22, "sub-pixel conv: K % 64 == 0, N = 256 phases (<= 8), operands below 2 GiB");
+  const int tiles_m = (p.M + 255) / 256, tiles_n = p.N / 256;
+  const int grid = phased_sched(tiles_m * tiles_n, false);
+  hipLaunchKernelGGL((gemm256_kernel<2, 2, false, VDA_ACT_NONE, false, false, 0, true>), dim3(grid), dim3(512), 0, st, p,
+                     tiles_m, tiles_n);
+  VDA_LAUNCH_CHECK();
+  return 0;
+}
+
 int vda_launch_depth_gemm(const GemmParams& p, hipStream_t st) {
   const int tiles_m = (p.M + 255) / 256;
   hipLaunchKernelGGL((gemm_kernel<256, 64, 8, 1, 64, 2, true, ACT_DEPTH>), dim3(tiles_m), dim3(512), 0, st, p, tiles_m, 1);
diff --git a/video-depth-anything_amd/csrc/vda_gemm_phased.h b/video-depth-anything_amd/csrc/vda_gemm_phased.h
--- a/video-depth-anything_amd/csrc/vda_gemm_phased.h
+++ b/video-depth-anything_amd/csrc/vda_gemm_phased.h
@@ -149,19 +149,21 @@
   return (128 * XR) / (512 / (OW / 8));
 }
 
-template <int XR, int WR, bool CONV, int ACT, bool ROWB, bool LNF, int EK>
+template <int XR, int WR, bool CONV, int ACT, bool ROWB, bool LNF, int EK, bool SUBP = false>
 __device__ __forceinline__ int gemm256_tile(const GemmParams& p, int vb, int tiles_m, int tiles_n, h16* smem,
                                             bool pre, int vb_next, int wave_in, unsigned* tctr = nullptr,
                                             int tbase = 0, int* tslot = nullptr) {
   static_assert(!(LNF && (ROWB || CONV)), "LNF: dense, no row bias");
   static_assert(EK == 0 || (!CONV && !ROWB), "fixed epilogue kinds: dense, no row bias");
   static_assert(EK != 3 || (ACT == VDA_ACT_NONE && LNF), "EK 3: LN fold + per-frame row bias, no activation");
+  static_assert(!SUBP || (XR == 2 && WR == 2 && !CONV && ACT == VDA_ACT_NONE && !ROWB && !LNF && EK == 0),
+                "SUBP: dense 256x256, staged epilogue, no activation");
   const bool has_bias = EK ? true : p.epi.bias != nullptr;
   const bool has_gamma = EK ? false : p.epi.gamma != nullptr;
   const bool ps_rows = !EK && ACT != VDA_ACT_GEGLU && !ROWB && XR == 2 && WR == 2 &&
                        p.epi.store == VDA_STORE_PIXEL_SHUFFLE && p.epi.ps_cout % 256 == 0 && p.epi.ps_win >= 16 &&
                        (long)p.M * p.N * 2 < 0x7fffffffL && (uintptr_t)p.y % 16 == 0;
-  const bool rows_store = EK ? true : (p.epi.store == VDA_STORE_ROWS || ps_rows);
+  const bool rows_store = (EK || SUBP) ? true : (p.epi.store == VDA_STORE_ROWS || ps_rows);
   const bool has_res = EK ? false : p.epi.res != nullptr;
   const bool has_res2 = EK ? false : p.epi.res2 != nullptr;
   const bool has_stats = EK ? false : p.epi.stats_out != nullptr;
@@ -664,6 +666,36 @@
 #pragma unroll
           for (int i = 0; i < 4; ++i) acc[i][j] += rb[j % RBD][i];
           __builtin_amdgcn_sched_barrier(0);
+        }
+      }
+    }
+    if constexpr (SUBP) {
+      const int s = p.stride, hc = p.H + 1, wc = p.W + 1;
+      const int ph = (p.sp_phases >> (4 * tile_n)) & 15, pa = ph >> 2, pb = ph & 3;
+      const int m = m0 + wm * 128 + mcol;
+      int cj = m % wc, ci = (m / wc) % hc;
+      const float* bcol = p.sp_bias + wn * 64 + nq;
+      f4 bmid[4];
+#pragma unroll
+      for (int i = 0; i < 4; ++i) bmid[i] = *reinterpret_cast<const f4*>(bcol + 4 * 256 + i * 16);
+#pragma unroll
+      for (int j = 0; j < 8; ++j) {
+        const int si = ci - (pa == s - 1 ? 1 : 0), sj = cj - (pb == s - 1 ? 1 : 0);
+        const int yc = (pa == 0 && si == 0) ? 0 : (pa == s - 1 && si == p.H - 1) ? 2 : 1;
+        const int xc = (pb == 0 && sj == 0) ? 0 : (pb == s - 1 && sj == p.W - 1) ? 2 : 1;
+        const int cls = yc * 3 + xc;
+        if (cls == 4) {
+#pragma unroll
+          for (int i = 0; i < 4; ++i) acc[i][j] += bmid[i];
+        } else {
+#pragma unroll
+          for (int i = 0; i < 4; ++i) acc[i][j] += *reinterpret_cast<const f4*>(bcol + cls * 256 + i * 16);
+        }
+        __builtin_amdgcn_sched_barrier(0);
+        cj += 16;
+        while (cj >= wc) {
+          cj -= wc;
+          if (++ci == hc) ci = 0;
         }
       }
     }
@@ -851,7 +883,36 @@
       }
       }
     };
-    if (ps_rows) {
+    auto sp_store = [&]() {
+      if constexpr (SUBP) {
+        const int s = p.stride, hin = p.H, win = p.W, hc = hin + 1, wc = win + 1;
+        const int ph = (p.sp_phases >> (4 * tile_n)) & 15, pa = ph >> 2, pb = ph & 3;
+        const int ea = pa == s - 1 ? 1 : 0, eb = pb == s - 1 ? 1 : 0;
+        const __amdgpu_buffer_rsrc_t rz = __builtin_amdgcn_make_buffer_rsrc(
+            (void*)p.y, (short)0, (int)((long)p.sp_bt * hin * s * win * s * 256 * 2), 0x00020000);
+        int m = m0 + row0;
+        int cj = m % wc, tq = m / wc;
+        int ci = tq % hc, bt = tq / hc;
+        const long rowlen = (long)win * s;
+#pragma unroll
+        for (int it = 0; it < NIT; ++it) {
+          const int si = ci - ea, sj = cj - eb;
+          const bool ok = m < p.M && (unsigned)si < (unsigned)hin && (unsigned)sj < (unsigned)win;
+          const long pix = ((long)(bt * hin + si) * s + pa) * rowlen + (long)sj * s + pb;
+          const unsigned off = ok ? (unsigned)((pix * 256 + q * 8) * 2) : 0x80000000u;
+          __builtin_amdgcn_raw_buffer_store_b128(__builtin_bit_cast(u32x4, tv[it]), rz, off, 0, VDA_EPI_STORE_AUX);
+          m += RPI;
+          cj += RPI;
+          while (cj >= wc) {
+            cj -= wc;
+            if (++ci == hc) { ci = 0; ++bt; }
+          }
+        }
+      }
+    };
+    if constexpr (SUBP) {
+      sp_store();
+    } else if (ps_rows) {
       ps_store();
     } else if (nres == 0) {
       if constexpr (RPF) {
@@ -913,7 +974,7 @@
   return succ;
 }
 
-template <int XR, int WR, bool CONV, int ACT, bool ROWB, bool LNF = false, int EK = 0>
+template <int XR, int WR, bool CONV, int ACT, bool ROWB, bool LNF = false, int EK = 0, bool SUBP = false>
 __global__ __launch_bounds__(512) void gemm256_kernel(GemmParams p, int tiles_m, int tiles_n) {
   constexpr int BUF = (XR + WR) * 128 * BK;
   constexpr bool TAB = XR == 2 && (ACT == VDA_ACT_GELU || ACT == VDA_ACT_GEGLU);
@@ -939,8 +1000,8 @@
     for (int vb = blockIdx.x; vb >= 0 && vb < ntiles;) {
       TS(0);
       const int nxt = vb + (int)gridDim.x;
-      vb = gemm256_tile<XR, WR, CONV, ACT, ROWB, LNF, EK>(p, vb, tiles_m, tiles_n, smem, pre, nxt < ntiles ? nxt : -1,
-                                                         wave, tctr, tbase, tslot);
+      vb = gemm256_tile<XR, WR, CONV, ACT, ROWB, LNF, EK, SUBP>(p, vb, tiles_m, tiles_n, smem, pre,
+                                                               nxt < ntiles ? nxt : -1, wave, tctr, tbase, tslot);
       if (!chain) __syncthreads();
       pre = chain;
       TS(7);
diff --git a/video-depth-anything_amd/csrc/vda_internal.h b/video-depth-anything_amd/csrc/vda_internal.h
--- a/video-depth-anything_amd/csrc/vda_internal.h
+++ b/video-depth-anything_amd/csrc/vda_internal.h
@@ -9,6 +9,8 @@
   int M, N, K;
   int H, W, Cin, Ho, Wo, ks, stride, pad, pre_relu, up_h, up_w;
   vda_epilogue epi;
+  int sp_bt, sp_phases;
+  const float* sp_bias;
 };
 VDA_KNOB_DECL(int, g_force_tile, -1);
 vda_epilogue vda_default_epi();
@@ -16,13 +18,15 @@
 int vda_launch_gemm(const GemmParams& p, hipStream_t st);
 int vda_launch_conv_gemm(const GemmParams& p, hipStream_t st);
 bool vda_gemm_phased256_serves(long M, long N, long K, long ldx);
+int vda_launch_subpixel_gemm(const GemmParams& p, hipStream_t st);
 int vda_launch_conv_reg(const GemmParams& p, hipStream_t st);
 int vda_launch_depth_gemm(const GemmParams& p, hipStream_t st);
 
 int vda_conv_halo(const void* x, const void* w, void* y, const float* bias, int relu, int BT, int H, int W, int Cin,
                   int Cout, hipStream_t st);
 int vda_conv_halo_fused(const void* x, const void* w, void* y, const float* bias, int relu, int BT, int Hs, int Ws,
-                        int H, int W, int Cin, int Cout, hipStream_t st);
+                        int H, int W, int Cin, int Cout, hipStream_t st, const float* bias9 = nullptr);
+bool vda_conv_halo_fused_serves(int BT, int Hs, int Ws, int H, int W, int Cin, int Cout);
 
 bool vda_depth_conv_serves(int H, int W, int C);
 int vda_depth_conv(const void* U, const void* w1, const float* b1, const float* w2, const float* b2, float* depth,
diff --git a/video-depth-anything_amd/csrc/vda_oc1.hip b/video-depth-anything_amd/csrc/vda_oc1.hip
--- a/video-depth-anything_amd/csrc/vda_oc1.hip
+++ b/video-depth-anything_amd/csrc/vda_oc1.hip
@@ -27,7 +27,8 @@
 __global__ __launch_bounds__(UPS ? 768 : 512) void halo_conv_kernel(const h16* __restrict__ U, const h16* __restrict__ w1,
                                                                   const float* __restrict__ b1, h16* __restrict__ yout,
                                                                   int relu_out, int H, int W, int C, int tiles_x,
-                                                                  int tiles_y, int ntiles, int Hs = 0, int Ws = 0) {
+                                                                  int tiles_y, int ntiles, int Hs = 0, int Ws = 0,
+                                                                  const float* __restrict__ b9 = nullptr) {
   constexpr int IW = UPS ? 4 : 0;
   constexpr int PSLOT = DNPIX * PSTR;
   constexpr int PP = (PSLOT + 63) / 64;
@@ -207,10 +208,11 @@
   for (int a = 0; a < NB; ++a)
 #pragma unroll
     for (int i = 0; i < 4; ++i) acc[a][i] = f4{0.f, 0.f, 0.f, 0.f};
+  const float* bsrc = b9 ? b9 + 4 * CO : b1;
   f4 bias_r[NB];
 #pragma unroll
   for (int a = 0; a < NB; ++a)
-    bias_r[a] = b1 ? *reinterpret_cast<const f4*>(b1 + (ng * NB + a) * 16 + g * 4) : f4{0.f, 0.f, 0.f, 0.f};
+    bias_r[a] = bsrc ? *reinterpret_cast<const f4*>(bsrc + (ng * NB + a) * 16 + g * 4) : f4{0.f, 0.f, 0.f, 0.f};
   const int my_pp = (PP - 1 - wave) / 8 + 1;
   constexpr int PPMAX = (PP + 7) / 8;
 
@@ -264,12 +266,19 @@
       const __amdgpu_buffer_rsrc_t ys = __builtin_amdgcn_make_buffer_rsrc(
           (void*)(yout + (long)bt * H * W * CO), (short)0, (int)((long)H * W * CO * 2), 0x00020000);
       const bool godd = (g & 1) != 0;
+      const bool ring = b9 != nullptr && (y0 == 0 || y0 + DT >= H || x0 == 0 || x0 + DT >= W);
 #pragma unroll
       for (int a = 0; a < NB; a += 2) {
-        const f4 bv0 = bias_r[a], bv1 = bias_r[a + 1];
 #pragma unroll
         for (int i = 0; i < 4; ++i) {
           const int y = y0 + mg * 4 + i, x = x0 + frow;
+          f4 bv0 = bias_r[a], bv1 = bias_r[a + 1];
+          if (ring) {
+            const int cls = (y == 0 ? 0 : y >= H - 1 ? 2 : 1) * 3 + (x == 0 ? 0 : x >= W - 1 ? 2 : 1);
+            const float* bp = b9 + cls * CO + (ng * NB + a) * 16 + g * 4;
+            bv0 = *reinterpret_cast<const f4*>(bp);
+            bv1 = *reinterpret_cast<const f4*>(bp + 16);
+          }
           const f4 v0 = acc[a][i] + bv0, v1 = acc[a + 1][i] + bv1;
           h4 o0, o1;
 #pragma unroll
@@ -342,16 +351,23 @@
 #endif
 
 int vda_conv_halo_fused(const void* x, const void* w, void* y, const float* bias, int relu, int BT, int Hs, int Ws,
-                        int H, int W, int Cin, int Cout, hipStream_t st) {
+                        int H, int W, int Cin, int Cout, hipStream_t st, const float* bias9) {
   if (Cout != CO || Cin % CS != 0 || Hs > H || Ws > W || Hs < 1 || Ws < 1) return 1;
   if ((long)H * W * Cout * 2 >= (1L << 31)) return 1;
   if (!halo_fused_fits(Hs, Ws, H, W)) return 1;
   HaloGrid g;
   if (!halo_tile_grid(BT, H, W, DT, 1, 0x7fffffffL, g)) return vda_set_error(-22, "conv: too many tiles");
   hipLaunchKernelGGL(halo_conv_kernel<true>, dim3(g.grid), dim3(768), 0, st, (const h16*)x, (const h16*)w, bias, (h16*)y,
-                     relu, H, W, Cin, g.tiles_x, g.tiles_y, g.ntiles, Hs, Ws);
+                     relu, H, W, Cin, g.tiles_x, g.tiles_y, g.ntiles, Hs, Ws, bias9);
   VDA_LAUNCH_CHECK();
   return 0;
+}
+
+bool vda_conv_halo_fused_serves(int BT, int Hs, int Ws, int H, int W, int Cin, int Cout) {
+  if (Cout != CO || Cin % CS != 0 || Hs > H || Ws > W || Hs < 1 || Ws < 1 || BT < 1) return false;
+  if ((long)H * W * Cout * 2 >= (1L << 31) || !halo_fused_fits(Hs, Ws, H, W)) return false;
+  HaloGrid g;
+  return halo_tile_grid(BT, H, W, DT, 1, 0x7fffffffL, g);
 }
 
 int vda_conv_halo(const void* x, const void* w, void* y, const float* bias, int relu, int BT, int H, int W, int Cin,
diff --git a/video-depth-anything_amd/csrc/vda_subpixel.hip b/video-depth-anything_amd/csrc/vda_subpixel.hip
--- /dev/null
+++ b/video-depth-anything_amd/csrc/vda_subpixel.hip
@@ -0,0 +1,94 @@
+#include "vda_internal.h"
+#include <algorithm>
+
+namespace {
+
+__global__ __launch_bounds__(256) void corner_gather_kernel(const h16* __restrict__ x, h16* __restrict__ a, int M, int H,
+                                                            int W, int Cin) {
+  const int cpt = Cin >> 3;
+  const int c = blockIdx.x * 256 + threadIdx.x;
+  if (c >= 4 * cpt) return;
+  const int blk = c / cpt, cc = c - blk * cpt;
+  const int dy = (blk == 0 || blk == 3) ? -1 : 0, dx = blk < 2 ? -1 : 0;
+  const int hc = H + 1, wc = W + 1;
+  for (int m = blockIdx.y; m < M; m += gridDim.y) {
+    const int bt = m / (hc * wc), r = m - bt * (hc * wc), ci = r / wc, cj = r - ci * wc;
+    const int iy = ci + dy, ix = cj + dx;
+    uint4 v = make_uint4(0u, 0u, 0u, 0u);
+    if ((unsigned)iy < (unsigned)H && (unsigned)ix < (unsigned)W)
+      v = ldg16(x + (((long)bt * H + iy) * W + ix) * Cin + cc * 8);
+    stg16(a + ((long)m * 4 * cpt + c) * 8, v);
+  }
+}
+
+struct Group {
+  int koff, kblocks;
+  int phases;
+};
+constexpr int ph4(int a0, int b0, int a1, int b1, int a2, int b2, int a3, int b3) {
+  return (a0 << 2 | b0) | (a1 << 2 | b1) << 4 | (a2 << 2 | b2) << 8 | (a3 << 2 | b3) << 12;
+}
+const Group G2[] = {{0, 4, ph4(0, 0, 0, 1, 1, 0, 1, 1)}};
+const Group G4[] = {{0, 4, ph4(0, 0, 0, 3, 3, 0, 3, 3)},
+                    {1, 2, ph4(1, 0, 1, 3, 2, 0, 2, 3)},
+                    {2, 2, ph4(0, 1, 0, 2, 3, 1, 3, 2)},
+                    {2, 1, ph4(1, 1, 1, 2, 2, 1, 2, 2)}};
+
+int check(int BT, int h, int w, int Cin, int Cout, int s) {
+  VDA_CHECK_ARG(BT > 0 && h > 0 && w > 0 && Cin > 0, "sub-pixel conv: empty map");
+  VDA_CHECK_ARG(s == 2 || s == 4, "sub-pixel conv: s must be 2 or 4");
+  VDA_CHECK_ARG(Cout == 256 && Cin % 64 == 0, "sub-pixel conv: Cout == 256 and Cin % 64 == 0");
+  const long M = (long)BT * (h + 1) * (w + 1);
+  VDA_CHECK_ARG(M * 4 * Cin * 2 < (1L << 31) && (long)BT * h * s * w * s * Cout * 2 < (1L << 31) &&
+                    (long)BT * h * w * Cin * 2 < (1L << 31),
+                "sub-pixel conv: the corner matrix, the input and the output must each stay below 2 GiB");
+  return 0;
+}
+
+}
+
+extern "C" int vda_subpixel_conv_check(int32_t BT, int32_t h, int32_t w, int32_t Cin, int32_t Cout, int32_t s) {
+  return check(BT, h, w, Cin, Cout, s);
+}
+
+extern "C" int64_t vda_subpixel_conv_workspace(int32_t BT, int32_t h, int32_t w, int32_t Cin, int32_t s) {
+  if (check(BT, h, w, Cin, 256, s)) return 0;
+  return (int64_t)BT * (h + 1) * (w + 1) * 4 * Cin * 2;
+}
+
+extern "C" int vda_subpixel_conv(const void* x, const void* w, const float* bias9, void* y, int32_t BT, int32_t h,
+                                 int32_t w_, int32_t Cin, int32_t Cout, int32_t s, void* ws, int64_t ws_bytes,
+                                 void* stream) {
+  VDA_CHECK_ARG(x && w && bias9 && y && ws, "null pointer");
+  int rc = check(BT, h, w_, Cin, Cout, s);
+  if (rc) return rc;
+  VDA_CHECK_ARG((uintptr_t)x % 16 == 0 && (uintptr_t)w % 16 == 0 && (uintptr_t)y % 16 == 0 && (uintptr_t)ws % 16 == 0 &&
+                    (uintptr_t)bias9 % 16 == 0,
+                "sub-pixel conv: x, w, bias9, y and ws must be 16-byte aligned");
+  const int M = BT * (h + 1) * (w_ + 1);
+  VDA_CHECK_ARG(ws_bytes >= (int64_t)M * 4 * Cin * 2, "sub-pixel conv: workspace too small (vda_subpixel_conv_workspace)");
+  hipStream_t st = (hipStream_t)stream;
+  const int cpr = 4 * (Cin / 8);
+  hipLaunchKernelGGL(corner_gather_kernel, dim3((unsigned)((cpr + 255) / 256), (unsigned)std::min(M, 65535)), dim3(256), 0,
+                     st, (const h16*)x, (h16*)ws, M, h, w_, Cin);
+  VDA_LAUNCH_CHECK();
+  const Group* g = s == 2 ? G2 : G4;
+  const int ng = s == 2 ? 1 : 4;
+  const h16* wg = (const h16*)w;
+  for (int i = 0; i < ng; ++i) {
+    GemmParams p{};
+    p.x = (const h16*)ws + (long)g[i].koff * Cin;
+    p.ldx = 4L * Cin;
+    p.w = wg;
+    p.y = (h16*)y;
+    p.ldy = Cout;
+    p.M = M; p.N = 4 * Cout; p.K = g[i].kblocks * Cin;
+    p.H = h; p.W = w_; p.stride = s;
+    p.epi = vda_default_epi();
+    p.sp_bt = BT; p.sp_phases = g[i].phases; p.sp_bias = bias9;
+    rc = vda_launch_subpixel_gemm(p, st);
+    if (rc) return rc;
+    wg += (long)p.N * p.K;
+  }
+  return 0;
+}
diff --git a/video-depth-anything_amd/csrc/vda_torch.cpp b/video-depth-anything_amd/csrc/vda_torch.cpp
--- a/video-depth-anything_amd/csrc/vda_torch.cpp
+++ b/video-depth-anything_amd/csrc/vda_torch.cpp
@@ -179,9 +179,34 @@
   return out;
 }
 
+Tensor subpixel_conv(const Tensor& x, const Tensor& w, const Tensor& bias9, int64_t BT, int64_t h, int64_t w_,
+                     int64_t s) {
+  TORCH_CHECK(x.scalar_type() == at::kHalf, "vda subpixel_conv: fp16 only");
+  TORCH_CHECK(x.dim() == 2 && x.is_contiguous() && x.size(0) == BT * h * w_,
+              "vda subpixel_conv: x must be a contiguous [BT*h*w, Cin] matrix");
+  need_contig(w, at::kHalf, "w", x);
+  need_contig(bias9, at::kFloat, "bias9", x);
+  TORCH_CHECK(bias9.dim() == 2 && bias9.size(0) == 9, "vda subpixel_conv: bias9 must be [9, Cout]");
+  const int64_t Cin = x.size(1), Cout = bias9.size(1);
+  TORCH_CHECK((s == 2 || s == 4) && w.numel() == 4 * Cout * Cin * (s == 2 ? 4 : 9),
+              "vda subpixel_conv: w must hold the packed phase groups of s = ", s);
+  Tensor out = at::empty({BT, h * s, w_ * s, Cout}, x.options());
+  if (x.is_meta()) return out;
+  const at::OptionalDeviceGuard g(x.device());
+  check_rc(vda_subpixel_conv_check((int32_t)BT, (int32_t)h, (int32_t)w_, (int32_t)Cin, (int32_t)Cout, (int32_t)s),
+           "vda_subpixel_conv_check");
+  const int64_t wsb = vda_subpixel_conv_workspace((int32_t)BT, (int32_t)h, (int32_t)w_, (int32_t)Cin, (int32_t)s);
+  Tensor ws = at::empty({wsb}, x.options().dtype(at::kByte));
+  check_rc(vda_subpixel_conv(x.data_ptr(), w.data_ptr(), (const float*)bias9.data_ptr(), out.data_ptr(), (int32_t)BT,
+                             (int32_t)h, (int32_t)w_, (int32_t)Cin, (int32_t)Cout, (int32_t)s, ws.data_ptr(), wsb,
+                             stream_of(x)),
+           "vda_subpixel_conv");
+  return out;
+}
+
 Tensor upsample_bilinear(const Tensor& x, int64_t Ho, int64_t Wo);
 Tensor conv2d(const Tensor& x, const Tensor& w, int64_t ks, int64_t stride, int64_t pad, OptT bias, bool pre_relu,
-              int64_t act, OptT res, OptT res2, at::OptionalIntArrayRef up) {
+              int64_t act, OptT res, OptT res2, at::OptionalIntArrayRef up, OptT bias9) {
   const auto dt = act_dtype(x);
   TORCH_CHECK(x.dim() == 4 && x.is_contiguous(), "vda conv2d: x must be a contiguous NHWC [BT, H, W, Cin] map");
   need_contig(w, dt, "w", x);
@@ -220,6 +245,12 @@
   vda_epilogue e = make_epi(x, bias, c10::nullopt, 1, 1, c10::nullopt, r, r2, act, dt);
   e.res2_h = r2h;
   e.res2_w = r2w;
+  if (bias9) {
+    need_contig(*bias9, at::kFloat, "bias9", x);
+    TORCH_CHECK(!bias && bias9->dim() == 2 && bias9->size(0) == 9 && bias9->size(1) == Cout,
+                "vda conv2d: bias9 must be [9, Cout] and replaces bias");
+    e.bias9 = (const float*)bias9->data_ptr();
+  }
   int rc;
   if (dt == at::kFloat) {
     TORCH_CHECK(uh == 0, "vda conv2d: the fused-upsample loader is fp16-only");
@@ -737,8 +768,9 @@
         "Tensor(c!)? sched=None, int drop_period=0, *, Tensor(a!) out) -> Tensor(a!)");
   m.def("row_stats(Tensor x, float eps) -> Tensor");
   m.def("conv_transpose_ks(Tensor x, Tensor w, Tensor bias, int BT, int h, int w_, int k) -> Tensor");
+  m.def("subpixel_conv(Tensor x, Tensor w, Tensor bias9, int BT, int h, int w_, int s) -> Tensor");
   m.def("conv2d(Tensor x, Tensor w, int ks=3, int stride=1, int pad=1, Tensor? bias=None, bool pre_relu=False, "
-        "int act=0, Tensor? res=None, Tensor? res2=None, int[]? up=None) -> Tensor");
+        "int act=0, Tensor? res=None, Tensor? res2=None, int[]? up=None, Tensor? bias9=None) -> Tensor");
   m.def("layernorm(Tensor x, Tensor gamma, Tensor beta, float eps, int skip_period=0, int? rows=None) -> Tensor");
   m.def("groupnorm(Tensor x, Tensor gamma, Tensor beta, int frames, int groups, float eps) -> Tensor");
   m.def("groupnorm_linear(Tensor x, Tensor gamma, Tensor beta, int frames, int groups, float eps, Tensor w, "
@@ -763,6 +795,7 @@
     m.impl("gemm", &gemm);                                    \
     m.impl("gemm.out", &gemm_out);                            \
     m.impl("conv_transpose_ks", &conv_transpose_ks);          \
+    m.impl("subpixel_conv", &subpixel_conv);                  \
     m.impl("conv2d", &conv2d);                                \
     m.impl("layernorm", &layernorm);                          \
     m.impl("row_stats", &row_stats);                          \
diff --git a/video-depth-anything_amd/model.py b/video-depth-anything_amd/model.py
--- a/video-depth-anything_amd/model.py
+++ b/video-depth-anything_amd/model.py
@@ -213,6 +213,7 @@
     fold_ff_norm: bool = False
     fuse_groupnorm_linear: bool = True
     fold_tap_norm: bool = True
+    fold_head_linear: bool = True
 
     def __init__(self, encoder="vitl", features=256, out_channels=(256, 512, 1024, 1024), use_bn=False,
                  use_clstoken=False, num_frames=32, pe="ape"):
@@ -416,6 +417,10 @@
     def prepare(self, device, size, fp32: bool = False) -> None:
         P = self._pack(torch.device(device), fp32)
         self._token_bias(P, int(size[0]), int(size[1]), torch.device(device))
+        if self._head_fold(P, 1, int(size[0]) // PATCH, int(size[1]) // PATCH):
+            self._pack_subpixel(P)
+        if self._oc1_fold(P, 1, int(size[0]) // PATCH, int(size[1]) // PATCH):
+            self._pack_oc1(P)
 
     def _qkv_fold(self, q: _Packed, M: int, S: int, T: int) -> List[bool]:
         ok = any(a.fold for a in q.attn) and ops.gemm_accepts(M, 3 * q.C, q.C, ln_fold=True, ln_parts=(q.C + 255) // 256,
@@ -458,7 +463,7 @@
         h = ops.gemm(g, q.ff2_w, bias=q.ff2_b, res=h, out=h)
         return ops.gemm(h, q.pout_w, bias=q.pout_b, res=x)
 
-    def _fusion(self, q: _Packed, x0, x1, size):
+    def _fusion(self, q: _Packed, x0, x1, size, out_conv: bool = True):
         if x1 is not None:
             t = ops.conv2d(x1, q.r1c1_w, bias=q.r1c1_b, pre_relu=True, act=ACT_RELU)
             out = ops.conv2d(t, q.r1c2_w, bias=q.r1c2_b, res=x1, res2=x0)
@@ -466,6 +471,8 @@
             out = x0
         t = ops.conv2d(out, q.r2c1_w, bias=q.r2c1_b, pre_relu=True, act=ACT_RELU)
         out = ops.conv2d(t, q.r2c2_w, bias=q.r2c2_b, res=out)
+        if not out_conv:
+            return out, size
         BT, h, w, Cf = out.shape
         y = ops.gemm(out.view(-1, Cf), q.out_w, bias=q.out_b).view(BT, h, w, Cf)
         return y, size
@@ -543,16 +550,52 @@
         return all(ops.gemm_accepts(BT * ntok, w.shape[0], P.C, ln_fold=True, ln_parts=nparts, drop_period=ntok)
                    for w, _, _ in P.projf)
 
-    def _reassemble(self, P: _Packed, enc, BT: int, ph: int, pw: int) -> List[torch.Tensor]:
+    def _head_fold(self, P: _Packed, BT: int, ph: int, pw: int) -> bool:
+        if P.fp32 or not bool(self.fold_head_linear):
+            return False
+        oc, Fh = self.out_channels, self.features
+        return (ops.subpixel_conv_accepts(BT, ph, pw, oc[0], Fh, 4) and
+                ops.subpixel_conv_accepts(BT, ph, pw, oc[1], Fh, 2))
+
+    def _oc1_fold(self, P: _Packed, BT: int, ph: int, pw: int) -> bool:
+        if P.fp32 or not bool(self.fold_head_linear):
+            return False
+        Fh = self.features
+        return ops.conv2d_bias9_accepts(BT, 4 * ph, 4 * pw, Fh, Fh // 2, (8 * ph, 8 * pw))
+
+    def _pack_oc1(self, P: _Packed):
+        if getattr(P, "oc1c", None) is None:
+            from .weights import compose_pointwise_conv3
+            s, dev = self.head.scratch, P.patch_w.device
+            w, b9 = compose_pointwise_conv3(s.refinenet1.out_conv.weight, s.refinenet1.out_conv.bias,
+                                            s.output_conv1.weight, s.output_conv1.bias)
+            P.oc1c = (w.to(dev), b9.to(dev))
+        return P.oc1c
+
+    def _pack_subpixel(self, P: _Packed):
+        if getattr(P, "sp", None) is None:
+            from .weights import compose_subpixel
+            hd, dev = self.head, P.patch_w.device
+            P.sp = []
+            for i, s in ((0, 4), (1, 2)):
+                ct = hd.resize_layers[i]
+                w, b9 = compose_subpixel(ct.weight, ct.bias, getattr(hd.scratch, f"layer{i + 1}_rn").weight, s)
+                P.sp.append((w.to(dev), b9.to(dev)))
+        return P.sp
+
+    def _reassemble(self, P: _Packed, enc, BT: int, ph: int, pw: int, fold: bool = False) -> List[torch.Tensor]:
         feats, cls, projected = enc
         oc = self.out_channels
+        sp = self._pack_subpixel(P) if fold else None
         lay = []
         for i, ft in enumerate(feats):
             if cls is not None:
                 rb = ops.gemm(cls[i].float(), P.ro_wb[i], bias=P.ro_b[i])
                 ft = ops.gemm(ft, P.ro_wa[i], rowbias=rb, rdiv=ph * pw, rmod=BT, act=ACT_GELU)
             p = ft if projected else ops.gemm(ft, P.proj_w[i], bias=P.proj_b[i])
-            if i == 0:
+            if fold and i < 2:
+                l = ops.subpixel_conv(p, sp[i][0], sp[i][1], BT, ph, pw, 4 if i == 0 else 2)
+            elif i == 0:
                 l = ops.conv_transpose_ks(p, P.rs_w[0], P.rs_b[0], BT, ph, pw, 4)
             elif i == 1:
                 l = ops.conv_transpose_ks(p, P.rs_w[1], P.rs_b[1], BT, ph, pw, 2)
@@ -564,15 +607,15 @@
         return lay
 
     def _head(self, P: _Packed, l1, l2, l3, l4, B: int, T: int, ph: int, pw: int, skip_tmp_block: bool,
-              sel: Optional[List[int]] = None) -> torch.Tensor:
+              sel: Optional[List[int]] = None, folded: bool = False, fold_out: bool = False) -> torch.Tensor:
         oc = self.out_channels
         BT = B * T
         h3, w3 = l3.shape[1:3]
         h4, w4 = l4.shape[1:3]
         l3 = self._temporal(P.mm[0], l3.reshape(-1, oc[2]), B, T, h3 * w3).view(BT, h3, w3, oc[2])
         l4 = self._temporal(P.mm[1], l4.reshape(-1, oc[3]), B, T, h4 * w4).view(BT, h4, w4, oc[3])
-        r1 = ops.conv2d(l1, P.rn[0])
-        r2 = ops.conv2d(l2, P.rn[1])
+        r1 = l1 if folded else ops.conv2d(l1, P.rn[0])
+        r2 = l2 if folded else ops.conv2d(l2, P.rn[1])
         r3 = ops.conv2d(l3, P.rn[2])
         r4 = ops.conv2d(l4, P.rn[3])
         del l1, l2, l3, l4
@@ -587,10 +630,13 @@
         if sel is not None:
             p3 = p3.index_select(0, torch.tensor(sel, dtype=torch.long, device=p3.device))
         y, _ = self._fusion(P.ref[2], p3, r2, None)
-        y, _ = self._fusion(P.ref[1], y, r1, None)
+        y, _ = self._fusion(P.ref[1], y, r1, None, out_conv=not fold_out)
         H1, W1 = 2 * y.shape[1], 2 * y.shape[2]
         if P.fp32:
             o1 = ops.conv2d(ops.upsample_bilinear(y, H1, W1), P.oc1_w, bias=P.oc1_b)
+        elif fold_out:
+            wc, b9 = self._pack_oc1(P)
+            o1 = ops.conv2d(y, wc, bias9=b9, up=(H1, W1))
         else:
             o1 = ops.conv2d(y, P.oc1_w, bias=P.oc1_b, up=(H1, W1))
         if P.fp32:
@@ -605,9 +651,10 @@
         BT = B * T
         ph, pw = H // PATCH, W // PATCH
         feats = self._encode(P, x.reshape(BT, 3, H, W))
-        lay = self._reassemble(P, feats, BT, ph, pw)
+        fold = self._head_fold(P, BT, ph, pw)
+        lay = self._reassemble(P, feats, BT, ph, pw, fold=fold)
         del feats
-        depth = self._head(P, *lay, B, T, ph, pw, skip_tmp_block)
+        depth = self._head(P, *lay, B, T, ph, pw, skip_tmp_block, folded=fold, fold_out=self._oc1_fold(P, BT, ph, pw))
         return depth.view(B, T, H, W)
 
     @torch.no_grad()
diff --git a/video-depth-anything_amd/ops.py b/video-depth-anything_amd/ops.py
--- a/video-depth-anything_amd/ops.py
+++ b/video-depth-anything_amd/ops.py
@@ -92,11 +92,26 @@
     return _vda().conv_transpose_ks(x, w, bias, int(BT), int(h), int(w_), int(k))
 
 
+def subpixel_conv(x: Tensor, w: Tensor, bias9: Tensor, BT: int, h: int, w_: int, s: int) -> Tensor:
+    _need(x, torch.float16, "x")
+    return _vda().subpixel_conv(x, w, bias9, int(BT), int(h), int(w_), int(s))
+
+
+@functools.lru_cache(maxsize=None)
+def subpixel_conv_accepts(BT: int, h: int, w_: int, Cin: int, Cout: int, s: int) -> bool:
+    return _lib.lib().vda_subpixel_conv_check(int(BT), int(h), int(w_), int(Cin), int(Cout), int(s)) == 0
+
+
+@functools.lru_cache(maxsize=None)
+def conv2d_bias9_accepts(BT: int, H: int, W: int, Cin: int, Cout: int, up) -> bool:
+    return _lib.lib().vda_conv2d_bias9_ok(int(BT), int(H), int(W), int(Cin), int(Cout), int(up[0]), int(up[1])) == 1
+
+
 def conv2d(x: Tensor, w: Tensor, *, ks=3, stride=1, pad=1, bias=None, pre_relu=False, act=ACT_NONE,
-           res=None, res2=None, up=None) -> Tensor:
+           res=None, res2=None, up=None, bias9=None) -> Tensor:
     _need(x, x.dtype, "x")
     return _vda().conv2d(x, w, int(ks), int(stride), int(pad), bias, bool(pre_relu), int(act), res, res2,
-                         None if up is None else [int(up[0]), int(up[1])])
+                         None if up is None else [int(up[0]), int(up[1])], bias9)
 
 
 def layernorm(x: Tensor, gamma: Tensor, beta: Tensor, eps: float, *, skip_period: int = 0,
diff --git a/video-depth-anything_amd/weights.py b/video-depth-anything_amd/weights.py
--- a/video-depth-anything_amd/weights.py
+++ b/video-depth-anything_amd/weights.py
@@ -51,6 +51,65 @@
     return {k: synthetic_tensor(k, s) for k, s in key_shapes}
 
 
+_CORNER = ((-1, -1), (0, -1), (0, 0), (-1, 0))
+SUBPIXEL_GROUPS = {
+    2: [(((0, 0), (0, 1), (1, 0), (1, 1)), _CORNER)],
+    4: [(((0, 0), (0, 3), (3, 0), (3, 3)), _CORNER),
+        (((1, 0), (1, 3), (2, 0), (2, 3)), _CORNER[1:3]),
+        (((0, 1), (0, 2), (3, 1), (3, 2)), _CORNER[2:4]),
+        (((1, 1), (1, 2), (2, 1), (2, 2)), _CORNER[2:3])],
+}
+
+
+def subpixel_blocks(wt: torch.Tensor, wr: torch.Tensor, s: int) -> Dict[tuple, torch.Tensor]:
+    wt, wr = wt.detach().double().cpu(), wr.detach().double().cpu()
+    out: Dict[tuple, torch.Tensor] = {}
+    for a in range(s):
+        for b in range(s):
+            for dy in (-1, 0, 1):
+                for dx in (-1, 0, 1):
+                    di, a2 = divmod(a + dy, s)
+                    dj, b2 = divmod(b + dx, s)
+                    blk = wr[:, :, dy + 1, dx + 1] @ wt[:, :, a2, b2].t()
+                    key = (a, b, di, dj)
+                    out[key] = out[key] + blk if key in out else blk
+    return out
+
+
+def subpixel_bias9(bt: torch.Tensor, wr: torch.Tensor) -> torch.Tensor:
+    bt, wr = bt.detach().double().cpu(), wr.detach().double().cpu()
+    taps = ((0, 1), (-1, 0, 1), (-1, 0))
+    rows = []
+    for rc in range(3):
+        for cc in range(3):
+            rows.append(sum(wr[:, :, dy + 1, dx + 1] @ bt for dy in taps[rc] for dx in taps[cc]))
+    return torch.stack(rows, 0)
+
+
+def compose_subpixel(wt: torch.Tensor, bt: torch.Tensor, wr: torch.Tensor, s: int):
+    blocks = subpixel_blocks(wt, wr, s)
+    used = set()
+    parts = []
+    for phases, window in SUBPIXEL_GROUPS[s]:
+        rows = []
+        for a, b in phases:
+            ea, eb = int(a == s - 1), int(b == s - 1)
+            keys = [(a, b, r + ea, c + eb) for r, c in window]
+            used.update(keys)
+            rows.append(torch.cat([blocks[k] for k in keys], 1))
+        parts.append(torch.cat(rows, 0).reshape(-1))
+    assert used == set(blocks), "every non-zero block of the composition belongs to exactly one phase window"
+    return torch.cat(parts).half().contiguous(), subpixel_bias9(bt, wr).float().contiguous()
+
+
+def compose_pointwise_conv3(w0: torch.Tensor, b0: torch.Tensor, w1: torch.Tensor, b1: torch.Tensor):
+    w0d = w0.detach().double().cpu().reshape(w0.shape[0], -1)
+    w1d = w1.detach().double().cpu()
+    wc = torch.einsum("omyx,mi->oyxi", w1d, w0d)
+    b9 = subpixel_bias9(b0, w1) + b1.detach().double().cpu()[None, :]
+    return wc.half().contiguous(), b9.float().contiguous()
+
+
 def load_checkpoint(path: str) -> Dict[str, torch.Tensor]:
     sd = torch.load(path, map_location="cpu", weights_only=True)
     if isinstance(sd, dict) and "model" in sd and isinstance(sd["model"], dict):
```

Measured after the change: 724.1 frames/s, median of 6. 1.9% higher.
